# arjunchandra/paac

Measured on AMD Instinct MI355X. Metric: global env-steps/sec at 32 envs, t_max=5, Nature net; 1/2/4/8 MI355X, higher is better.
Workload: dtype f32; 1 GPU; breakout action set (A=4), NATURE net, 32 envs per GPU x 1 GPU, t_max=5, synthetic 84x84x4 u8 frames generated on device, sampler=numpy, hipGraph replay; envs_per_gpu=32, t_max=5, global_envs=32, parallelism=env-sharded dp1, no collective (one process)

## Files before the change

include/paac_hip.h:

```cpp
#ifndef PAAC_HIP_H
#define PAAC_HIP_H

#include <stdint.h>

#ifdef __cplusplus
extern "C" {
#endif

typedef struct paac_ctx paac_ctx;
typedef struct paac_graph paac_graph;
typedef void* paac_stream_t;

enum { PAAC_ARCH_NIPS = 0, PAAC_ARCH_NATURE = 1,
       PAAC_ARCH_USER = 2 };
enum { PAAC_CLIP_IGNORE = 0, PAAC_CLIP_GLOBAL = 1, PAAC_CLIP_LOCAL = 2 };

#define PAAC_MAX_TENSORS 12
#define PAAC_OBS_BYTES 28224
#define PAAC_RAW_H 210
#define PAAC_RAW_W 160

typedef struct {
  int32_t num_tensors;
  int64_t total;
  int64_t total_unpadded;
  int64_t offset[PAAC_MAX_TENSORS];
  int64_t size[PAAC_MAX_TENSORS];
  int32_t rank[PAAC_MAX_TENSORS];
  int32_t shape[PAAC_MAX_TENSORS][4];
  char name[PAAC_MAX_TENSORS][32];
} paac_layout;

typedef struct {
  int32_t device;
  int32_t arch;
  int32_t num_actions;
  int32_t max_batch;
} paac_cfg;

const char* paac_last_error(void);
int paac_version(void);

int paac_param_layout(int arch, int num_actions, paac_layout* out);

int paac_create(const paac_cfg* cfg, paac_ctx** out);
int paac_destroy(paac_ctx* ctx);

int paac_forward(paac_ctx* ctx, const float* params, const uint8_t* states, int batch,
                 float* logits, float* probs, float* values, paac_stream_t stream);

int paac_forward_sample(paac_ctx* ctx, const float* params, const uint8_t* states, int batch, float* probs,
                        float* values, uint64_t seed, const uint64_t* step_base_dev, uint64_t step_offset,
                        uint32_t env_offset, int32_t* actions, paac_stream_t stream);

int paac_forward_sample_synth_step(paac_ctx* ctx, const float* params, const uint8_t* states, int batch, float* probs,
                                   float* values, uint64_t seed, const uint64_t* step_base_dev, uint64_t step_offset,
                                   uint32_t env_offset, int32_t* actions, uint64_t env_seed, uint32_t terminal_threshold,
                                   uint8_t* stack_out, float* rewards_out, float* masks_out, float* ep_reward,
                                   int32_t* ep_len, void* finished, paac_stream_t stream);

int paac_train_forward(paac_ctx* ctx, const float* params, const uint8_t* states, int batch, float* values,
                       paac_stream_t stream);
int paac_train_forward_trunk(paac_ctx* ctx, const float* params, const uint8_t* states, int batch, paac_stream_t stream);

int paac_keep_next_forward(paac_ctx* ctx, int train_row);
int paac_bootstrap_forward_trunk(paac_ctx* ctx, const float* params, const uint8_t* states, int batch, int train_row,
                                 paac_stream_t stream);

#define PAAC_ACT_STEP_MAX_ENVS 64
#define PAAC_ACT_STEP_MAX_ENVS_LARGE 256
int paac_act_step_mt(paac_ctx* ctx, const float* params, const uint8_t* states, int batch, uint32_t* mt_state,
                     int32_t* actions, float* probs_out, float* values_out, uint64_t env_seed, uint32_t env_offset,
                     uint32_t terminal_threshold, const uint64_t* step_base_dev, uint64_t step_offset, uint8_t* stack_out,
                     uint8_t* stack_out2, float* rewards_out, float* masks_out, float* ep_reward, int32_t* ep_len,
                     void* finished, uint8_t* raw_scratch, void* walk_scratch, int64_t walk_scratch_bytes,
                     paac_stream_t stream);

int paac_pack_weights(paac_ctx* ctx, const float* params, paac_stream_t stream);
int paac_set_managed_weights(paac_ctx* ctx, int on);

int paac_loss_backward(paac_ctx* ctx, const float* params, const uint8_t* states, const int32_t* actions,
                       const float* y, const float* adv, int batch, float entropy_beta,
                       float* grad, float* loss_out, int forward_done, int phase, paac_stream_t stream);

enum { PAAC_RETURNS_NSTEP = 0, PAAC_RETURNS_GAE = 1 };

typedef struct {
  const float* v_boot;
  const float* rewards;
  const float* masks;
  const float* values;
  int32_t T, N;
  double gamma;
  float* y_out;
  float* adv_out;
  int64_t* global_step_dev;
  int64_t increment;
  double initial_lr;
  int64_t lr_annealing_steps;
  float* lr_out_dev;
  uint64_t* tick_dev;
  uint64_t tick_inc;
  int32_t estimator;
  double gae_lambda;
} paac_returns;
#define PAAC_RETURNS_TRUNCS 0x100
typedef struct {
  paac_returns ret;
  const float* truncs;
} paac_returns_truncs;
int paac_loss_backward_returns(paac_ctx* ctx, const float* params, const uint8_t* states, const int32_t* actions,
                               const paac_returns* ret, int batch, float entropy_beta, float* grad, float* loss_out,
                               int forward_done, int phase, paac_stream_t stream);

#define PAAC_PPO_EPOCHS_MAX 16
int paac_loss_backward_record(paac_ctx* ctx, const float* params, const uint8_t* states, const int32_t* actions,
                              const float* y, const float* adv, float* p_old_out, int batch, float entropy_beta,
                              float* grad, float* loss_out, int forward_done, int phase, paac_stream_t stream);
int paac_loss_backward_returns_record(paac_ctx* ctx, const float* params, const uint8_t* states, const int32_t* actions,
                                      const paac_returns* ret, float* p_old_out, int batch, float entropy_beta,
                                      float* grad, float* loss_out, int forward_done, int phase, paac_stream_t stream);
int paac_loss_backward_ppo(paac_ctx* ctx, const float* params, const uint8_t* states, const int32_t* actions,
                           const float* y, const float* adv, const float* p_old, float clip_eps, int batch,
                           float entropy_beta, float* grad, float* loss_out, float* ppo_stats_out, int forward_done,
                           int phase, paac_stream_t stream);

int paac_loss_backward_ppo_vclip(paac_ctx* ctx, const float* params, const uint8_t* states, const int32_t* actions,
                                 const float* y, const float* adv, const float* p_old, const float* v_old, float clip_eps,
                                 float vclip_eps, int batch, float entropy_beta, float* grad, float* loss_out,
// ... 186 lines not shown
```

paac_amd/_lib.py:

```python
import ctypes
import os
from ctypes import POINTER, c_char, c_char_p, c_double, c_float, c_int, c_int32, c_int64, c_uint32, c_uint64, c_void_p

HERE = os.path.dirname(os.path.abspath(__file__))
LIB_PATH = os.environ.get("PAAC_HIP_LIB") or os.path.join(HERE, "libpaac_hip.so")

MAX_TENSORS = 12
PROF_FAMILIES = 16
ARCH_NIPS, ARCH_NATURE, ARCH_USER = 0, 1, 2
CLIP_IGNORE, CLIP_GLOBAL, CLIP_LOCAL = 0, 1, 2
RETURNS_NSTEP, RETURNS_GAE = 0, 1
RETURNS_TRUNCS = 0x100
PPO_EPOCHS_MAX = 16
PPO_MINIBATCHES_MAX = 16
PPO_STEPS_MAX = 64
MINIBATCH_MAX_ROWS = 8192
EVAL_CATCH, EVAL_BRICKS, EVAL_RALLY = 0, 1, 2
EVAL_USER = 3


class Layout(ctypes.Structure):
    _fields_ = [("num_tensors", c_int32),
                ("total", c_int64),
                ("total_unpadded", c_int64),
# ... 59 lines not shown
                                          c_void_p, c_void_p, c_int, c_int, c_void_p]),
    "paac_loss_backward_ppo": (c_int, [c_void_p, c_void_p, c_void_p, c_void_p, c_void_p, c_void_p, c_void_p, c_float, c_int,
                                       c_float, c_void_p, c_void_p, c_void_p, c_int, c_int, c_void_p]),
    "paac_loss_backward_ppo_vclip": (c_int, [c_void_p, c_void_p, c_void_p, c_void_p, c_void_p, c_void_p, c_void_p, c_void_p,
                                             c_float, c_float, c_int, c_float, c_void_p, c_void_p, c_void_p, c_int, c_int,
                                             c_void_p]),
    "paac_minibatch_perms": (c_int, [c_int, c_int, c_uint64, c_void_p, c_uint64, c_void_p, c_void_p]),
    "paac_gather_minibatch": (c_int, [c_void_p, c_int, c_void_p, c_void_p, c_void_p, c_void_p, c_void_p, c_void_p, c_void_p,
                                      c_void_p, c_void_p, c_void_p, c_void_p, c_void_p, c_void_p]),
    "paac_record_policy": (c_int, [c_void_p, c_void_p, c_void_p, c_int, c_void_p, c_void_p, c_int, c_void_p]),
    "paac_adv_normalize": (c_int, [c_void_p, c_int, c_void_p, c_void_p, c_void_p]),
    "paac_returns_norm_tick": (c_int, [c_void_p, c_void_p, POINTER(Returns), c_void_p, c_void_p, c_void_p]),
    "paac_returns_scan": (c_int, [POINTER(Returns), c_void_p]),
    "paac_game_step": (c_int, [c_int, c_uint64, c_uint32, c_int] + [c_void_p] * 7 + [POINTER(EnvRecords), c_int, c_void_p]),
    "paac_grad_stats": (c_int, [c_void_p, c_void_p, c_void_p]),
    "paac_grad_tensor_stats": (c_int, [c_void_p, c_void_p, c_void_p]),
    "paac_clip_rmsprop": (c_int, [c_void_p, c_void_p, c_void_p, c_void_p, c_void_p, c_int64, c_void_p, c_float,
                                  c_float, c_float, c_float, c_int, c_float, c_void_p, c_void_p]),
    "paac_clip_adam": (c_int, [c_void_p, c_void_p, c_void_p, c_void_p, c_void_p, c_void_p, c_int64, c_void_p, c_float,
                               c_float, c_float, c_float, c_int, c_float, c_void_p, c_void_p]),
    "paac_clip_rmsprop_gated": (c_int, [c_void_p, c_void_p, c_void_p, c_void_p, c_void_p, c_int64, c_void_p, c_float,
                                        c_float, c_float, c_float, c_int, c_float, c_void_p, POINTER(KlGate), c_void_p]),
    "paac_clip_adam_gated": (c_int, [c_void_p, c_void_p, c_void_p, c_void_p, c_void_p, c_void_p, c_int64, c_void_p, c_float,
                                     c_float, c_float, c_float, c_int, c_float, c_void_p, POINTER(KlGate), c_void_p]),
    "paac_lr_step": (c_int, [c_void_p, c_int64, c_double, c_int64, c_void_p, c_void_p]),
    "paac_nstep_returns": (c_int, [c_void_p, c_void_p, c_void_p, c_void_p, c_int, c_int, c_double, c_void_p,
                                   c_void_p, c_void_p]),
    "paac_nstep_returns_tick": (c_int, [c_void_p, c_void_p, c_void_p, c_void_p, c_int, c_int, c_double, c_void_p,
                                        c_void_p, c_void_p, c_int64, c_double, c_int64, c_void_p, c_void_p, c_uint64,
                                        c_void_p]),
    "paac_gae_returns": (c_int, [c_void_p, c_void_p, c_void_p, c_void_p, c_int, c_int, c_double, c_double, c_void_p,
                                 c_void_p, c_void_p]),
    "paac_gae_returns_tick": (c_int, [c_void_p, c_void_p, c_void_p, c_void_p, c_int, c_int, c_double, c_double, c_void_p,
                                      c_void_p, c_void_p, c_int64, c_double, c_int64, c_void_p, c_void_p, c_uint64,
                                      c_void_p]),
    "paac_sample_mt_scratch_bytes": (c_int64, [c_int, c_int]),
    "paac_sample_mt": (c_int, [c_void_p, c_int, c_int, c_void_p, c_void_p, c_void_p, c_void_p]),
    "paac_sample_philox": (c_int, [c_void_p, c_int, c_int, c_uint64, c_void_p, c_uint64, c_uint32, c_void_p, c_void_p]),
    "paac_counter_add": (c_int, [c_void_p, c_uint64, c_void_p]),
    "paac_preprocess_stack": (c_int, [c_void_p, c_int, c_int, c_void_p, c_void_p, c_void_p, c_void_p, c_void_p]),
    "paac_synth_reset": (c_int, [c_uint64, c_uint32, c_int, c_void_p, c_void_p, c_void_p]),
    "paac_synth_step": (c_int, [c_uint64, c_uint32, c_int, c_void_p, c_uint32, c_void_p, c_uint64, c_void_p,
                                c_void_p, c_void_p, c_void_p, c_void_p, c_void_p, c_void_p, c_void_p, c_void_p,
                                c_void_p]),
    "paac_eval_step": (c_int, [c_int, c_void_p, c_int, c_int, c_int, c_uint64, c_int, c_void_p, c_uint64, c_uint64, c_uint32,
                               c_void_p, c_void_p, c_void_p, c_void_p, c_void_p, c_void_p, c_void_p, c_void_p, c_void_p,
                               c_void_p]),
    "paac_match_step": (c_int, [c_void_p, c_int, c_int, c_int, c_uint64, c_int, c_void_p, c_uint64, c_uint64, c_uint32,
                                c_void_p, c_void_p, c_void_p, c_void_p, c_void_p, c_void_p, c_void_p, c_void_p, c_void_p,
                                c_void_p]),
    "paac_act_step_mt": (c_int, [c_void_p, c_void_p, c_void_p, c_int, c_void_p, c_void_p, c_void_p, c_void_p, c_uint64,
                                 c_uint32, c_uint32, c_void_p, c_uint64, c_void_p, c_void_p, c_void_p, c_void_p, c_void_p,
                                 c_void_p, c_void_p, c_void_p, c_void_p, c_int64, c_void_p]),
    "paac_walk_scratch_bytes": (c_int64, [c_int, c_int]),
    "paac_debug_report_zero": (c_int, [c_int]),
    "paac_sample_mt_synth_step": (c_int, [c_void_p, c_int, c_void_p, c_void_p, c_uint64, c_uint32, c_int, c_uint32, c_void_p,
                                          c_uint64, c_void_p, c_void_p, c_void_p, c_void_p, c_void_p, c_void_p, c_void_p,
                                          c_void_p, c_void_p, c_int64, c_void_p, c_void_p]),
    "paac_forward_sample_synth_step": (c_int, [c_void_p, c_void_p, c_void_p, c_int, c_void_p, c_void_p, c_uint64, c_void_p,
                                               c_uint64, c_uint32, c_void_p, c_uint64, c_uint32, c_void_p, c_void_p,
                                               c_void_p, c_void_p, c_void_p, c_void_p, c_void_p]),
    "paac_graph_begin": (c_int, [c_void_p]),
    "paac_graph_end": (c_int, [c_void_p, POINTER(c_void_p)]),
    "paac_graph_launch": (c_int, [c_void_p, c_void_p]),
    "paac_graph_destroy": (c_int, [c_void_p]),
    "paac_debug_activation": (c_int64, [c_void_p, c_int, c_int, c_void_p, c_int64, c_void_p]),
    "paac_debug_activation_size": (c_int64, [c_int, c_int, c_int]),
    "paac_debug_set_tuning": (c_int, [c_void_p, c_int, c_int, c_int, c_int, c_int]),
    "paac_debug_get_tuning": (c_int, [c_void_p, c_int, c_int, POINTER(c_int), POINTER(c_int), POINTER(c_int)]),
    "paac_debug_cfg_known": (c_int, [c_int, c_int]),
    "paac_debug_cfg_body": (c_int, [c_int, c_int]),
    "paac_debug_clock": (c_int, [c_void_p, c_void_p]),
    "paac_prof_enable": (c_int, [c_void_p, c_int]),
    "paac_prof_read": (c_int, [c_void_p, POINTER(c_int32), POINTER(c_int32), POINTER(c_float), c_int]),
    "paac_prof_read_mix": (c_int, [c_void_p, POINTER(c_int32), c_int]),
    "paac_prof_name": (c_char_p, [c_int]),
    "paac_user_arch": (c_int, [POINTER(c_int32), POINTER(c_int32), POINTER(c_int32)]),
    "paac_user_arch_layers": (c_int, [POINTER(c_int32), POINTER(c_int32)]),
}

for _game in ("catch", "bricks", "rally"):
    _SIGNATURES["paac_%s_reset" % _game] = (c_int, [c_uint64, c_uint32, c_int, c_void_p, c_void_p, c_void_p])
    _SIGNATURES["paac_%s_step" % _game] = (c_int, [c_uint64, c_uint32, c_int] + [c_void_p] * 12 +
                                           ([c_int] if _game == "bricks" else []) + [c_void_p])
_SIGNATURES["paac_duel_reset"] = _SIGNATURES["paac_catch_reset"]
_SIGNATURES["paac_duel_step"] = (c_int, [c_uint64, c_uint32, c_int] + [c_void_p] * 7 + [POINTER(EnvRecords), c_void_p])
_SIGNATURES["paac_duel_ghost_reset"] = (c_int, [c_uint64, c_uint32, c_int, c_void_p, c_void_p, c_void_p, c_void_p])
_SIGNATURES["paac_duel_ghost_step"] = (c_int, [c_uint64, c_uint32, c_int, c_void_p, c_void_p, c_int, c_uint64, c_void_p, c_uint64] +
                                       [c_void_p] * 9 + [POINTER(EnvRecords), c_void_p, c_void_p])
_SIGNATURES["paac_user_game_info"] = (c_int, [POINTER(c_int), POINTER(c_int), POINTER(c_int)])
_SIGNATURES["paac_user_game_reset"] = _SIGNATURES["paac_catch_reset"]
_SIGNATURES["paac_user_game_step"] = (c_int, [c_uint64, c_uint32, c_int] + [c_void_p] * 7 + [POINTER(EnvRecords), c_int, c_void_p])

EXPORTED_SYMBOLS = tuple(sorted(_SIGNATURES))

_lib = None


def use_library(path):
    global LIB_PATH
    if _lib is not None and os.path.abspath(path) != os.path.abspath(LIB_PATH):
        raise PaacHipError("%s is already loaded: a process holds ONE geometry besides Nature -- choose the user "
                           "architecture before anything touches the library" % LIB_PATH)
    LIB_PATH = path


# ... 53 lines not shown
```

paac_amd/csrc/api.hip:

```cpp
#include <stdarg.h>
#include <stdlib.h>

#include <new>

#include "common.h"
#include "synth_dev.h"

namespace paac {

static thread_local char g_err[512] = "";
thread_local ProfEvents g_prof = {nullptr, nullptr, 0, 0};
paac_ctx* g_prof_ctx = nullptr;

void set_error(const char* fmt, ...) {
  va_list ap;
  va_start(ap, fmt);
  vsnprintf(g_err, sizeof(g_err), fmt, ap);
  va_end(ap);
}

ArchSpec arch_spec(int arch) {
  ArchSpec s;
  memset(&s, 0, sizeof(s));
  if (arch == PAAC_ARCH_NATURE) {
// ... 6 lines not shown
#ifdef PAAC_USER_ARCH
  } else if (arch == PAAC_ARCH_USER) {
#ifndef PAAC_USER_K1
#define PAAC_USER_K1 8
#define PAAC_USER_S1 4
#define PAAC_USER_K2 4
#define PAAC_USER_S2 2
#define PAAC_USER_K3 3
#define PAAC_USER_S3 1
#endif
    constexpr int o1 = (84 - PAAC_USER_K1) / PAAC_USER_S1 + 1, o2 = (o1 - PAAC_USER_K2) / PAAC_USER_S2 + 1;
    constexpr int o3 = PAAC_USER_NCONV == 3 ? (o2 - PAAC_USER_K3) / PAAC_USER_S3 + 1 : o2;
    s.nconv = PAAC_USER_NCONV;
    s.conv[0] = ConvSpec{84, 84, 4, o1, o1, PAAC_USER_C1, PAAC_USER_K1, PAAC_USER_S1};
    s.conv[1] = ConvSpec{o1, o1, PAAC_USER_C1, o2, o2, PAAC_USER_C2, PAAC_USER_K2, PAAC_USER_S2};
    if (PAAC_USER_NCONV == 3) s.conv[2] = ConvSpec{o2, o2, PAAC_USER_C2, o3, o3, PAAC_USER_C3, PAAC_USER_K3, PAAC_USER_S3};
    s.flat = PAAC_USER_NCONV == 3 ? o3 * o3 * PAAC_USER_C3 : o2 * o2 * PAAC_USER_C2;
    s.fc = PAAC_USER_H;
#endif
  } else {
    s.nconv = 2;
    s.conv[0] = ConvSpec{84, 84, 4, 20, 20, 16, 8, 4};
    s.conv[1] = ConvSpec{20, 20, 16, 9, 9, 32, 4, 2};
    s.flat = 2592;
    s.fc = 256;
  }
  return s;
}

bool arch_supported(int arch) {
#ifdef PAAC_USER_ARCH
  return arch == PAAC_ARCH_NATURE || arch == PAAC_ARCH_USER;
#else
  return arch == PAAC_ARCH_NATURE || arch == PAAC_ARCH_NIPS;
#endif
}

int64_t wslab_floats_needed(int arch);
size_t tower_pack_bytes();
void default_tuning(paac_ctx* c);
int cfg_body(int op, int cfg);
int fc_splits_max();

static const char* kFamilyNames[PAAC_PROF_FAMILIES] = {
    "conv1_fwd", "conv2_fwd", "conv3_fwd", "fc_fwd", "heads_fwd", "heads_bwd", "fc_wgrad", "fc_dgrad",
    "conv3_wgrad", "conv3_dgrad", "conv2_wgrad", "conv2_dgrad", "conv1_wgrad", "grad_finalize", "clip_rmsprop", "misc",
    "env_step", "sample_env_step", "sample_mt", "sample_philox", "nstep_returns", "preprocess_stack", "conv_tower",
    "fc_conv3_wgrad", "conv2_conv1_wgrad", "dgrad_tower"};

}

using namespace paac;

struct paac_graph {
  hipGraph_t graph;
  hipGraphExec_t exec;
};

extern "C" {

const char* paac_last_error(void) { return g_err; }
int paac_version(void) { return 100; }

int paac_param_layout(int arch, int num_actions, paac_layout* out) {
  PAAC_REQUIRE(out, "paac_param_layout: null out");
  PAAC_REQUIRE(arch_supported(arch), "paac_param_layout: arch %d is not compiled into this library (a library holds Nature "
               "and either the NIPS geometry or one user architecture, paac_user_arch)", arch);
  PAAC_REQUIRE(num_actions >= 2 && num_actions <= 32, "paac_param_layout: num_actions %d not in [2,32]", num_actions);
  memset(out, 0, sizeof(*out));
  const ArchSpec s = arch_spec(arch);
  int t = 0;
  int64_t off = 0, unp = 0;
  auto add = [&](const char* name, int rank, int d0, int d1, int d2, int d3) {
    int64_t size = (int64_t)d0 * (rank > 1 ? d1 : 1) * (rank > 2 ? d2 : 1) * (rank > 3 ? d3 : 1);
    snprintf(out->name[t], sizeof(out->name[t]), "%s", name);
    out->rank[t] = rank;
    out->shape[t][0] = d0; out->shape[t][1] = rank > 1 ? d1 : 0;
    out->shape[t][2] = rank > 2 ? d2 : 0; out->shape[t][3] = rank > 3 ? d3 : 0;
    out->offset[t] = off;
    out->size[t] = size;
    off += (size + 3) / 4 * 4;
    unp += size;
    ++t;
  };
  char nm[32];
  for (int i = 0; i < s.nconv; ++i) {
    snprintf(nm, sizeof(nm), "conv%d_weights", i + 1);
    add(nm, 4, s.conv[i].k, s.conv[i].k, s.conv[i].cin, s.conv[i].cout);
    snprintf(nm, sizeof(nm), "conv%d_biases", i + 1);
    add(nm, 1, s.conv[i].cout, 0, 0, 0);
  }
  snprintf(nm, sizeof(nm), "fc%d_weights", s.nconv + 1);
  add(nm, 2, s.flat, s.fc, 0, 0);
  snprintf(nm, sizeof(nm), "fc%d_biases", s.nconv + 1);
  add(nm, 1, s.fc, 0, 0, 0);
  add("actor_output_weights", 2, s.fc, num_actions, 0, 0);
  add("actor_output_biases", 1, num_actions, 0, 0, 0);
  add("critic_output_weights", 2, s.fc, 1, 0, 0);
  add("critic_output_biases", 1, 1, 0, 0, 0);
  out->num_tensors = t;
  out->total = off;
  out->total_unpadded = unp;
  return 0;
}

int paac_create(const paac_cfg* cfg, paac_ctx** out) {
// ... 37 lines not shown
        else if (op < 0 || op >= OP_COUNT || cls < 0 || cls > 2)
          set_error("paac_create: PAAC_TUNE_OVERRIDE entry \"%s\": op %d / class %d outside the table (ops 0..%d, classes 0..2)",
                    entry, op, cls, OP_COUNT - 1);
        else set_error("paac_create: PAAC_TUNE_OVERRIDE entry \"%s\": op %d has no configuration id %d", entry, op, cf);
        delete c;
        return -1;
      }
      c->tune[op][cls] = Tune{cf, ks, xc};
      ov += used;
      if (*ov == ',') ++ov;
    }
  }
  const int64_t B = cfg->max_batch;
  const int A = cfg->num_actions;
  c->fc_splits_max = fc_splits_max();
  for (int w = 0; w < 2; ++w) {
    Workspace& W = c->ws[w];
    for (int i = 0; i < c->spec.nconv; ++i) {
      const ConvSpec& cs = c->spec.conv[i];
      PAAC_CHECK_HIP(hipMalloc(&W.act[i], (size_t)((B + 15) / 16 * 16) * cs.oh * cs.ow * cs.cout * sizeof(float)));
    }
    PAAC_CHECK_HIP(hipMalloc(&W.fc_slab, (size_t)c->fc_splits_max * B * c->spec.fc * sizeof(float)));
    PAAC_CHECK_HIP(hipMalloc(&W.h, (size_t)B * c->spec.fc * sizeof(float)));
    PAAC_CHECK_HIP(hipMalloc(&W.probs, (size_t)B * A * sizeof(float)));
    PAAC_CHECK_HIP(hipMalloc(&W.logits, (size_t)B * A * sizeof(float)));
    PAAC_CHECK_HIP(hipMalloc(&W.values, (size_t)B * sizeof(float)));
  }
  for (int i = 0; i < c->spec.nconv; ++i) {
    const ConvSpec& cs = c->spec.conv[i];
    PAAC_CHECK_HIP(hipMalloc(&c->dact[i], (size_t)B * cs.oh * cs.ow * cs.cout * sizeof(float)));
  }
  PAAC_CHECK_HIP(hipMalloc(&c->dh, (size_t)B * c->spec.fc * sizeof(float)));
  if (paac::dh_planes_supported(c->spec.fc)) {
    PAAC_CHECK_HIP(hipMalloc(&c->dh_planes, paac::dh_planes_bytes((int)B, c->spec.fc)));
    PAAC_CHECK_HIP(hipMemset(c->dh_planes, 0, paac::dh_planes_bytes((int)B, c->spec.fc)));
  }
  { const char* v = getenv("PAAC_FC_DGRAD_ONCE"); c->fc_dgrad_once = !(v && *v && atoi(v) == 0); }
  PAAC_CHECK_HIP(hipMalloc(&c->dl_buf, (size_t)B * paac::kDlStride * sizeof(float)));
  PAAC_CHECK_HIP(hipMalloc(&c->ppo_rows, (size_t)B * 2 * sizeof(float)));
  PAAC_CHECK_HIP(hipMalloc(&c->vclip_rows, (size_t)B * sizeof(float)));
  c->wslab_floats = wslab_floats_needed(cfg->arch);
  PAAC_CHECK_HIP(hipMalloc(&c->wslab, (size_t)c->wslab_floats * sizeof(float)));
  PAAC_CHECK_HIP(hipMalloc(&c->partials, 8192 * sizeof(float)));
  PAAC_CHECK_HIP(hipMemset(c->partials, 0, 8192 * sizeof(float)));
  PAAC_CHECK_HIP(hipMalloc(&c->zeros, (size_t)(c->spec.fc > 1024 ? c->spec.fc : 1024) * sizeof(float)));
  PAAC_CHECK_HIP(hipMemset(c->zeros, 0, (size_t)(c->spec.fc > 1024 ? c->spec.fc : 1024) * sizeof(float)));
  c->keep_row = -1;
  c->keep_h_only = 0;
  c->heads_pending_h = 0;
  PAAC_CHECK_HIP(hipMalloc(&c->mt_ahead, mt_ahead_bytes()));
  PAAC_CHECK_HIP(hipMemset(c->mt_ahead, 0, mt_ahead_bytes()));
  c->ahead_state = nullptr;
  c->ahead_D = 0;
  {
    const char* v = getenv("PAAC_TOWER");
    c->tower_on = (cfg->arch == PAAC_ARCH_NATURE) && !(v && *v && atoi(v) == 0);
    { const char* q = getenv("PAAC_FC_QUARTER"); c->no_quarter_tiles = (q && *q && atoi(q) == 0) ? 1 : 0; }
    c->tower2_on = (cfg->arch == PAAC_ARCH_NIPS) && tower2_available() && !(v && *v && atoi(v) == 0);
    c->managed_weights = 0;
    c->tower_pack = nullptr;
    if (c->tower_on || c->tower2_on) PAAC_CHECK_HIP(hipMalloc(&c->tower_pack, tower_pack_bytes()));
    PAAC_CHECK_HIP(hipMalloc(&c->fc_pack, (size_t)c->spec.flat * c->spec.fc * sizeof(float)));
  }
  c->ev_start = new hipEvent_t[paac_ctx::PROF_MAX_EVENTS];
  c->ev_stop = new hipEvent_t[paac_ctx::PROF_MAX_EVENTS];
  c->ev_family = new int[paac_ctx::PROF_MAX_EVENTS];
  c->ev_batch = new int[paac_ctx::PROF_MAX_EVENTS];
  c->ev_mix = new int[paac_ctx::PROF_MAX_EVENTS];
  c->ev_count = 0;
  c->prof_on = 0;
  for (int i = 0; i < paac_ctx::PROF_MAX_EVENTS; ++i) {
    c->ev_start[i] = nullptr;
    c->ev_stop[i] = nullptr;
  }
  *out = c;
  return 0;
}

int paac_destroy(paac_ctx* c) {
  if (!c) return 0;
  for (int w = 0; w < 2; ++w) {
    Workspace& W = c->ws[w];
    for (int i = 0; i < 3; ++i)
      if (W.act[i]) (void)hipFree(W.act[i]);
    float* bufs[] = {W.fc_slab, W.h, W.probs, W.logits, W.values};
    for (float* b : bufs)
      if (b) (void)hipFree(b);
  }
  for (int i = 0; i < 3; ++i)
    if (c->dact[i]) (void)hipFree(c->dact[i]);
  float* bufs[] = {c->dh, c->wslab, c->partials, c->dl_buf, c->zeros, c->ppo_rows, c->vclip_rows};
  for (float* b : bufs)
    if (b) (void)hipFree(b);
  if (c->mt_ahead) (void)hipFree(c->mt_ahead);
  if (c->dh_planes) (void)hipFree(c->dh_planes);
  if (c->tower_pack) (void)hipFree(c->tower_pack);
  if (c->fc_pack) (void)hipFree(c->fc_pack);
  for (int i = 0; i < paac_ctx::PROF_MAX_EVENTS; ++i) {
    if (c->ev_start[i]) (void)hipEventDestroy(c->ev_start[i]);
    if (c->ev_stop[i]) (void)hipEventDestroy(c->ev_stop[i]);
  }
  delete[] c->ev_start;
  delete[] c->ev_stop;
  delete[] c->ev_family;
  delete[] c->ev_batch;
  delete[] c->ev_mix;
  delete c;
  return 0;
}

int paac_forward(paac_ctx* ctx, const float* params, const uint8_t* states, int batch, float* logits, float* probs,
                 float* values, paac_stream_t stream) {
  PAAC_REQUIRE(ctx && params && states, "paac_forward: null argument");
  PAAC_REQUIRE(batch > 0 && batch <= ctx->max_batch, "paac_forward: batch %d outside (0, max_batch=%d]", batch,
               ctx->max_batch);
  const int rc = launch_forward(ctx, 0, params, states, batch, logits, probs, values, (hipStream_t)stream);
  if (rc) return rc;
  PAAC_CHECK_HIP(hipGetLastError());
  return 0;
}

int paac_pack_weights(paac_ctx* ctx, const float* params, paac_stream_t stream) {
  PAAC_REQUIRE(ctx && params, "paac_pack_weights: null argument");
  const int rc = launch_pack_weights(ctx, params, (hipStream_t)stream);
  if (rc) return rc;
  PAAC_CHECK_HIP(hipGetLastError());
  return 0;
}

int paac_set_managed_weights(paac_ctx* ctx, int on) {
  PAAC_REQUIRE(ctx, "paac_set_managed_weights: null ctx");
  ctx->managed_weights = on ? 1 : 0;
  return 0;
}

int paac_train_forward(paac_ctx* ctx, const float* params, const uint8_t* states, int batch, float* values,
                       paac_stream_t stream) {
  PAAC_REQUIRE(ctx && params && states, "paac_train_forward: null argument");
  PAAC_REQUIRE(batch > 0 && batch <= ctx->max_batch, "paac_train_forward: batch %d outside (0, max_batch=%d]", batch,
               ctx->max_batch);
  const int rc = launch_forward(ctx, 1, params, states, batch, nullptr, nullptr, values, (hipStream_t)stream);
  if (rc) return rc;
  PAAC_CHECK_HIP(hipGetLastError());
  return 0;
}

int paac_train_forward_trunk(paac_ctx* ctx, const float* params, const uint8_t* states, int batch, paac_stream_t stream) {
  PAAC_REQUIRE(ctx && params && states, "paac_train_forward_trunk: null argument");
  PAAC_REQUIRE(batch > 0 && batch <= ctx->max_batch, "paac_train_forward_trunk: batch %d outside (0, max_batch=%d]", batch,
               ctx->max_batch);
  const int rc = launch_forward_trunk_train(ctx, params, states, batch, (hipStream_t)stream);
  if (rc) return rc;
  PAAC_CHECK_HIP(hipGetLastError());
  return 0;
}

int paac_keep_next_forward(paac_ctx* ctx, int train_row) {
  PAAC_REQUIRE(ctx, "paac_keep_next_forward: null ctx");
  PAAC_REQUIRE(train_row >= -1 && train_row < ctx->max_batch, "paac_keep_next_forward: row %d outside [-1, max_batch=%d)",
               train_row, ctx->max_batch);
  ctx->keep_row = train_row;
  return 0;
}

int paac_bootstrap_forward_trunk(paac_ctx* ctx, const float* params, const uint8_t* states, int batch, int train_row,
                                 paac_stream_t stream) {
  PAAC_REQUIRE(ctx && params && states, "paac_bootstrap_forward_trunk: null argument");
  PAAC_REQUIRE(batch > 0 && train_row >= 0 && train_row + batch <= ctx->max_batch,
               "paac_bootstrap_forward_trunk: rows [%d, %d) outside max_batch=%d", train_row, train_row + batch, ctx->max_batch);
  const int rc = launch_bootstrap_trunk(ctx, params, states, batch, train_row, (hipStream_t)stream);
  if (rc) return rc;
  PAAC_CHECK_HIP(hipGetLastError());
  return 0;
}

int paac_forward_sample(paac_ctx* ctx, const float* params, const uint8_t* states, int batch, float* probs,
                        float* values, uint64_t seed, const uint64_t* step_base_dev, uint64_t step_offset,
                        uint32_t env_offset, int32_t* actions, paac_stream_t stream) {
  PAAC_REQUIRE(ctx && params && states && actions, "paac_forward_sample: null argument");
  PAAC_REQUIRE(batch > 0 && batch <= ctx->max_batch, "paac_forward_sample: batch %d outside (0, max_batch=%d]", batch,
               ctx->max_batch);
  const int rc = launch_forward_sample(ctx, params, states, batch, probs, values, seed, step_base_dev, step_offset,
                                       env_offset, actions, nullptr, (hipStream_t)stream);
  if (rc) return rc;
  PAAC_CHECK_HIP(hipGetLastError());
  return 0;
}

int paac_forward_sample_synth_step(paac_ctx* ctx, const float* params, const uint8_t* states, int batch, float* probs,
                                   float* values, uint64_t seed, const uint64_t* step_base_dev, uint64_t step_offset,
                                   uint32_t env_offset, int32_t* actions, uint64_t env_seed, uint32_t terminal_threshold,
                                   uint8_t* stack_out, float* rewards_out, float* masks_out, float* ep_reward,
                                   int32_t* ep_len, void* finished, paac_stream_t stream) {
  PAAC_REQUIRE(ctx && params && states && actions, "paac_forward_sample_synth_step: null argument");
  SynthStep st;
  if (synth_step_of("paac_forward_sample_synth_step", "null argument", false, &st, env_seed, env_offset, batch, terminal_threshold,
                    step_base_dev, step_offset, states, stack_out, nullptr, rewards_out, masks_out, ep_reward, ep_len, finished,
                    nullptr))
    return -1;
  PAAC_REQUIRE(batch > 0 && batch <= ctx->max_batch, "paac_forward_sample_synth_step: batch %d outside (0, max_batch=%d]",
               batch, ctx->max_batch);
  const int rc = launch_forward_sample(ctx, params, states, batch, probs, values, seed, step_base_dev, step_offset, env_offset,
                                       actions, &st, (hipStream_t)stream);
  if (rc) return rc;
  PAAC_CHECK_HIP(hipGetLastError());
  return 0;
}

int paac_act_step_mt(paac_ctx* ctx, const float* params, const uint8_t* states, int batch, uint32_t* mt_state,
                     int32_t* actions, float* probs_out, float* values_out, uint64_t env_seed, uint32_t env_offset,
                     uint32_t terminal_threshold, const uint64_t* step_base_dev, uint64_t step_offset, uint8_t* stack_out,
                     uint8_t* stack_out2, float* rewards_out, float* masks_out, float* ep_reward, int32_t* ep_len,
                     void* finished, uint8_t* raw_scratch, void* walk_scratch, int64_t walk_scratch_bytes,
                     paac_stream_t stream) {
  PAAC_REQUIRE(ctx && params && states && mt_state && actions && probs_out && values_out, "paac_act_step_mt: null argument");
  HeadsPartials hp{nullptr, 0, nullptr, nullptr, values_out};
  if (stack_out == nullptr) {
    PAAC_REQUIRE(!stack_out2 && !raw_scratch, "paac_act_step_mt: no environment step (stack_out == NULL) takes no stack_out2 / "
                 "raw_scratch");
    PAAC_REQUIRE(batch > 0 && batch <= ctx->max_batch && batch <= PAAC_ACT_STEP_MAX_ENVS &&
                 (int64_t)batch * (ctx->cfg.num_actions - 1) <= 1024,
                 "paac_act_step_mt: sampling without an environment step covers up to %d environments and 1024 draws (use "
                 "paac_forward + paac_sample_mt); got %d x %d actions", PAAC_ACT_STEP_MAX_ENVS, batch, ctx->cfg.num_actions);
// ... 25 lines not shown
               "paac_act_step_mt: N*(A-1) = %ld exceeds %d (use paac_forward + paac_sample_mt + paac_synth_step)",
               (long)batch * (ctx->cfg.num_actions - 1), PAAC_FUSED_SAMPLE_MAX_DRAWS);
  if (!forward_has_fc_heads(ctx)) {
    int rc = launch_forward(ctx, 0, params, states, batch, nullptr, probs_out, values_out, (hipStream_t)stream);
    if (rc) return rc;
    rc = launch_sample_mt_synth_step(probs_out, ctx->cfg.num_actions, mt_state, actions, st, walk_scratch, walk_scratch_bytes,
                                     nullptr, (hipStream_t)stream);
    if (rc) return rc;
    PAAC_CHECK_HIP(hipGetLastError());
    return 0;
  }
  if (batch > PAAC_ACT_STEP_MAX_ENVS || (int64_t)batch * (ctx->cfg.num_actions - 1) > 1024) {
    const bool tail = (ctx->tower_on || ctx->tower2_on) && ctx->managed_weights && batch <= PAAC_ACT_STEP_MAX_ENVS_LARGE;
    if (tail) {
      ctx->ahead_state = mt_state;
      ctx->ahead_D = batch * (ctx->cfg.num_actions - 1);
    }
    static const int fold_knob = [] {
      const char* v = getenv("PAAC_HEADS_IN_SAMPLER");
      return (v && *v) ? (atoi(v) != 0 ? 1 : 0) : -1;
    }();
    const bool fold = fold_knob >= 0 ? fold_knob == 1 : ctx->cfg.num_actions <= 8;
    int rc;
    if (tail && fold && sampler_folds_heads(batch, ctx->cfg.num_actions, walk_scratch))
      rc = launch_forward_trunk(ctx, params, states, batch, &hp, (hipStream_t)stream);
    else
      rc = launch_forward(ctx, 0, params, states, batch, nullptr, probs_out, values_out, (hipStream_t)stream);
    ctx->ahead_state = nullptr;
    if (rc) return rc;
    rc = launch_sample_mt_synth_step(probs_out, ctx->cfg.num_actions, mt_state, actions, st, walk_scratch, walk_scratch_bytes,
                                     tail ? ctx->mt_ahead : nullptr, (hipStream_t)stream, hp.partial ? &hp : nullptr);
    if (rc) return rc;
    PAAC_CHECK_HIP(hipGetLastError());
    return 0;
  }
  static const bool ahead_on = [] {
    const char* v = getenv("PAAC_MT_AHEAD_SMALL");
    return v && *v && atoi(v) != 0;
  }();
  if (ahead_on) {
    ctx->ahead_state = mt_state;
    ctx->ahead_D = batch * (ctx->cfg.num_actions - 1);
  }
  int rc = launch_forward_trunk(ctx, params, states, batch, &hp, (hipStream_t)stream);
  ctx->ahead_state = nullptr;
  if (rc) return rc;
  rc = launch_sample_env_step_heads(hp, probs_out, ctx->cfg.num_actions, mt_state, actions, st, ahead_on ? ctx->mt_ahead : nullptr,
                                    (hipStream_t)stream);
  if (rc) return rc;
  PAAC_CHECK_HIP(hipGetLastError());
  return 0;
}

static int check_returns(const char* fn, const paac_returns* ret) {
  PAAC_REQUIRE(ret->rewards && ret->masks && ret->values && ret->y_out && ret->adv_out, "%s: null rollout record", fn);
  PAAC_REQUIRE(returns_estimator(ret) == PAAC_RETURNS_NSTEP || returns_estimator(ret) == PAAC_RETURNS_GAE,
               "%s: estimator %d (PAAC_RETURNS_NSTEP = 0, PAAC_RETURNS_GAE = 1)", fn, returns_estimator(ret));
  PAAC_REQUIRE(ret->gae_lambda >= 0.0 && ret->gae_lambda <= 1.0, "%s: gae_lambda %g outside [0, 1]", fn, ret->gae_lambda);
  PAAC_REQUIRE(!ret->global_step_dev || (ret->lr_out_dev && ret->lr_annealing_steps > 0),
               "%s: schedule bookkeeping needs lr_out_dev and lr_annealing_steps", fn);
  return 0;
}

static int loss_backward_entry(const char* fn, paac_ctx* ctx, const float* params, const uint8_t* states, const int32_t* actions,
                               int batch, float entropy_beta, float* grad, float* loss_out, const BackwardCall& call,
                               int forward_done, int phase, paac_stream_t stream) {
  PAAC_REQUIRE(ctx && params && states && actions && grad && (call.ret || (call.y && call.adv)), "%s: null argument", fn);
  PAAC_REQUIRE(batch > 0 && batch <= ctx->max_batch, "%s: batch %d outside (0, max_batch=%d]", fn, batch, ctx->max_batch);
  PAAC_REQUIRE(phase >= 0 && phase <= 3, "%s: phase %d", fn, phase);
  if (const paac_returns* ret = call.ret) {
    PAAC_REQUIRE(ret->T > 0 && ret->N > 0 && ret->T * ret->N == batch, "%s: T*N = %d*%d != batch %d", fn, ret->T, ret->N, batch);
    if (const int rc = check_returns(fn, ret)) return rc;
    PAAC_REQUIRE(ret->v_boot || (forward_done && batch + ret->N <= ctx->max_batch),
                 "%s: v_boot == NULL takes the bootstrap values from rows [batch, batch + N) of a training forward that has "
                 "already run over batch + N rows", fn);
  }
  int rc = 0;
  if (!forward_done && phase != 2) {
    rc = launch_forward(ctx, 1, params, states, batch, nullptr, nullptr, nullptr, (hipStream_t)stream);
    if (rc) return rc;
  }
  ctx->last_ws = 1;
  rc = launch_backward(ctx, params, states, actions, batch, entropy_beta, grad, loss_out, phase, call, (hipStream_t)stream);
  if (rc) return rc;
  PAAC_CHECK_HIP(hipGetLastError());
  return 0;
}

int paac_loss_backward(paac_ctx* ctx, const float* params, const uint8_t* states, const int32_t* actions, const float* y,
                       const float* adv, int batch, float entropy_beta, float* grad, float* loss_out,
                       int forward_done, int phase, paac_stream_t stream) {
  const BackwardCall call{.y = y, .adv = adv, .loss = kLossA3c};
  return loss_backward_entry("paac_loss_backward", ctx, params, states, actions, batch, entropy_beta, grad, loss_out, call,
                             forward_done, phase, stream);
}

int paac_loss_backward_returns(paac_ctx* ctx, const float* params, const uint8_t* states, const int32_t* actions,
                               const paac_returns* ret, int batch, float entropy_beta, float* grad, float* loss_out,
                               int forward_done, int phase, paac_stream_t stream) {
  PAAC_REQUIRE(ret, "paac_loss_backward_returns: null argument");
  const BackwardCall call{.ret = ret, .loss = kLossA3c};
  return loss_backward_entry("paac_loss_backward_returns", ctx, params, states, actions, batch, entropy_beta, grad, loss_out,
                             call, forward_done, phase, stream);
}

int paac_loss_backward_returns_record(paac_ctx* ctx, const float* params, const uint8_t* states, const int32_t* actions,
                                      const paac_returns* ret, float* p_old_out, int batch, float entropy_beta, float* grad,
                                      float* loss_out, int forward_done, int phase, paac_stream_t stream) {
  PAAC_REQUIRE(ret, "paac_loss_backward_returns_record: null argument");
  PAAC_REQUIRE(p_old_out, "paac_loss_backward_returns_record: null p_old_out");
  const BackwardCall call{.ret = ret, .loss = kLossA3cRecord, .p_old_out = p_old_out};
  return loss_backward_entry("paac_loss_backward_returns_record", ctx, params, states, actions, batch, entropy_beta, grad,
                             loss_out, call, forward_done, phase, stream);
}

int paac_loss_backward_record(paac_ctx* ctx, const float* params, const uint8_t* states, const int32_t* actions,
                              const float* y, const float* adv, float* p_old_out, int batch, float entropy_beta, float* grad,
                              float* loss_out, int forward_done, int phase, paac_stream_t stream) {
  PAAC_REQUIRE(p_old_out, "paac_loss_backward_record: null p_old_out");
  const BackwardCall call{.y = y, .adv = adv, .loss = kLossA3cRecord, .p_old_out = p_old_out};
  return loss_backward_entry("paac_loss_backward_record", ctx, params, states, actions, batch, entropy_beta, grad, loss_out,
                             call, forward_done, phase, stream);
}

int paac_loss_backward_ppo(paac_ctx* ctx, const float* params, const uint8_t* states, const int32_t* actions, const float* y,
                           const float* adv, const float* p_old, float clip_eps, int batch, float entropy_beta, float* grad,
                           float* loss_out, float* ppo_stats_out, int forward_done, int phase, paac_stream_t stream) {
  PAAC_REQUIRE(p_old, "paac_loss_backward_ppo: null p_old");
  PAAC_REQUIRE(clip_eps > 0.f && clip_eps < 1.f, "paac_loss_backward_ppo: clip_eps %g outside (0, 1)", (double)clip_eps);
  const BackwardCall call{.y = y, .adv = adv, .loss = kLossPpo, .p_old = p_old, .clip_eps = clip_eps,
                          .ppo_stats_out = ppo_stats_out};
  return loss_backward_entry("paac_loss_backward_ppo", ctx, params, states, actions, batch, entropy_beta, grad, loss_out, call,
                             forward_done, phase, stream);
}

static int64_t debug_activation_elems(const ArchSpec& spec, int what, int batch) {
  if (what == 25) return batch;
  if (what >= 21 && what <= 24) what -= 20;
  if (what >= 11 && what <= 10 + spec.nconv) what -= 10;
  if (what >= 1 && what <= spec.nconv) {
    const ConvSpec& cs = spec.conv[what - 1];
    return (int64_t)batch * cs.oh * cs.ow * cs.cout;
  }
  if (what == 4 || what == 14) return (int64_t)batch * spec.fc;
  return -1;
}

int paac_returns_norm_tick(paac_ctx* ctx, const float* params, const paac_returns* ret, float* adv_n_out, double* stats_out,
                           paac_stream_t stream) {
  PAAC_REQUIRE(ret && adv_n_out, "paac_returns_norm_tick: null argument");
  PAAC_REQUIRE(ret->T > 0 && ret->N > 0, "paac_returns_norm_tick: T=%d N=%d", ret->T, ret->N);
  if (const int rc = check_returns("paac_returns_norm_tick", ret)) return rc;
  const float* v_boot = ret->v_boot;
  if (!v_boot) {
    const int64_t batch = (int64_t)ret->T * ret->N;
    PAAC_REQUIRE(ctx && params && batch + ret->N <= ctx->max_batch,
                 "paac_returns_norm_tick: v_boot == NULL takes the bootstrap values from rows [T*N, T*N + N) of a training "
                 "forward that has already run over T*N + N rows of this ctx");
    const int rc = launch_bootstrap_heads(ctx, params, (int)batch, ret->N, (hipStream_t)stream);
    if (rc) return rc;
    v_boot = ctx->ws[1].values + batch;
  }
  const int rc = launch_returns_norm(ret, v_boot, adv_n_out, stats_out, (hipStream_t)stream);
  if (rc) return rc;
  PAAC_CHECK_HIP(hipGetLastError());
  return 0;
}

int paac_record_policy(paac_ctx* ctx, const float* params, const int32_t* actions, int batch, float* p_old_out, float* v_out,
                       int value_rows, paac_stream_t stream) {
  PAAC_REQUIRE(ctx && params, "paac_record_policy: null argument");
  PAAC_REQUIRE(p_old_out || v_out, "paac_record_policy: nothing to record (p_old_out and v_out are both NULL)");
  PAAC_REQUIRE(!p_old_out || actions, "paac_record_policy: p_old_out needs the actions");
  if (!p_old_out) batch = 0;
  if (!v_out) value_rows = 0;
  const int rows = batch > value_rows ? batch : value_rows;
  PAAC_REQUIRE(batch >= 0 && value_rows >= 0 && rows > 0 && rows <= ctx->max_batch,
               "paac_record_policy: batch %d / value_rows %d outside (0, max_batch=%d]", batch, value_rows, ctx->max_batch);
  if (ctx->heads_pending_rows > 0) {
    PAAC_REQUIRE(rows <= ctx->heads_pending_rows, "paac_record_policy: the pending training forward covers %d rows, %d are asked "
                 "for", ctx->heads_pending_rows, rows);
    const int rc = launch_deferred_heads(ctx, params, (hipStream_t)stream);
    if (rc) return rc;
  }
  const int rc = launch_record_policy(ctx, actions, batch, value_rows, p_old_out, v_out, (hipStream_t)stream);
  if (rc) return rc;
  PAAC_CHECK_HIP(hipGetLastError());
  return 0;
}

int paac_loss_backward_ppo_vclip(paac_ctx* ctx, const float* params, const uint8_t* states, const int32_t* actions,
                                 const float* y, const float* adv, const float* p_old, const float* v_old, float clip_eps,
                                 float vclip_eps, int batch, float entropy_beta, float* grad, float* loss_out,
                                 float* ppo_stats_out, int forward_done, int phase, paac_stream_t stream) {
  PAAC_REQUIRE(p_old, "paac_loss_backward_ppo_vclip: null p_old");
  PAAC_REQUIRE(v_old, "paac_loss_backward_ppo_vclip: null v_old");
  PAAC_REQUIRE(clip_eps > 0.f && clip_eps < 1.f, "paac_loss_backward_ppo_vclip: clip_eps %g outside (0, 1)", (double)clip_eps);
  PAAC_REQUIRE(vclip_eps > 0.f, "paac_loss_backward_ppo_vclip: vclip_eps %g is not positive (0 = off: paac_loss_backward_ppo)",
               (double)vclip_eps);
  const BackwardCall call{.y = y, .adv = adv, .loss = kLossPpoVclip, .p_old = p_old, .clip_eps = clip_eps,
                          .ppo_stats_out = ppo_stats_out, .v_old = v_old, .vclip_eps = vclip_eps};
  return loss_backward_entry("paac_loss_backward_ppo_vclip", ctx, params, states, actions, batch, entropy_beta, grad, loss_out,
                             call, forward_done, phase, stream);
}

int64_t paac_debug_activation_size(int arch, int what, int batch) {
  PAAC_REQUIRE(batch > 0, "paac_debug_activation_size: batch %d", batch);
  const int64_t n = debug_activation_elems(arch_spec(arch), what, batch);
  if (n < 0) {
    set_error("paac_debug_activation_size: what=%d", what);
    return -1;
  }
  return n;
}

int64_t paac_debug_activation(paac_ctx* ctx, int what, int batch, float* out, int64_t out_capacity, paac_stream_t stream) {
  PAAC_REQUIRE(ctx && out && batch > 0 && batch <= ctx->max_batch, "paac_debug_activation: bad arguments");
  if (what == 26) {
    const int64_t np = (int64_t)batch * ctx->cfg.num_actions;
    PAAC_REQUIRE(np <= out_capacity, "paac_debug_activation: what=26 needs %ld floats, out holds %ld", (long)np, (long)out_capacity);
    PAAC_CHECK_HIP(hipMemcpyAsync(out, ctx->ws[1].probs, (size_t)np * sizeof(float), hipMemcpyDeviceToDevice, (hipStream_t)stream));
    return np;
  }
  const int64_t n = debug_activation_elems(ctx->spec, what, batch);
  if (n < 0) {
    set_error("paac_debug_activation: what=%d", what);
// ... 160 lines not shown
```

paac_amd/csrc/common.h:

```cpp
#pragma once
#include <hip/hip_runtime.h>
#include <hip/hip_ext.h>
#include <stdint.h>
#include <stdio.h>
#include <string.h>

#include "../../include/paac_hip.h"

namespace paac {

void set_error(const char* fmt, ...);

inline int returns_estimator(const paac_returns* ret) { return ret->estimator & ~PAAC_RETURNS_TRUNCS; }
inline const float* returns_truncs(const paac_returns* ret) {
  return (ret->estimator & PAAC_RETURNS_TRUNCS) ? reinterpret_cast<const paac_returns_truncs*>(ret)->truncs : nullptr;
}

#define PAAC_CHECK_HIP(expr)                                                              \
  do {                                                                                    \
    hipError_t _e = (expr);                                                               \
    if (_e != hipSuccess) {                                                               \
      paac::set_error("%s:%d: %s -> %s", __FILE__, __LINE__, #expr, hipGetErrorString(_e)); \
      return -2;                                                                          \
    }                                                                                     \
// ... 20 lines not shown
  int fc;
};
ArchSpec arch_spec(int arch);

enum Family {
  F_CONV1_FWD = 0, F_CONV2_FWD, F_CONV3_FWD, F_FC_FWD, F_HEADS_FWD,
  F_HEADS_BWD, F_FC_WGRAD, F_FC_DGRAD, F_CONV3_WGRAD, F_CONV3_DGRAD, F_CONV2_WGRAD, F_CONV2_DGRAD, F_CONV1_WGRAD,
  F_GRAD_FINALIZE, F_CLIP_RMSPROP, F_MISC,
  F_ENV_STEP, F_SAMPLE_ENV_STEP, F_SAMPLE_MT, F_SAMPLE_PHILOX, F_NSTEP_RETURNS, F_PREPROCESS_STACK, F_CONV_TOWER,
  F_FC_CONV3_WGRAD, F_CONV2_CONV1_WGRAD, F_DGRAD_TOWER
};
static_assert(F_DGRAD_TOWER + 1 == PAAC_PROF_FAMILIES, "family count");

}

namespace paac {
struct Workspace {
  float* act[3];
  float* fc_slab;
  float* h;
  float* probs;
  float* values;
  float* logits;
};
}

namespace paac {
enum Op { OP_CONV1_FWD = 0, OP_CONV2_FWD, OP_CONV3_FWD, OP_FC_FWD, OP_FC_WGRAD, OP_FC_DGRAD, OP_CONV3_WGRAD,
          OP_CONV3_DGRAD, OP_CONV2_WGRAD, OP_CONV2_DGRAD, OP_CONV1_WGRAD, OP_CONV_TOWER, OP_COUNT };
struct Tune {
  int cfg;
  int ksplit;
  int xcd;
};
inline int batch_class(int batch) { return batch > 512 ? 2 : batch > 64 ? 1 : 0; }

constexpr int kDlStride = 36;

constexpr bool dh_planes_supported(int H) { return (H % 32) == 0 && H <= 1024; }
inline size_t dh_planes_bytes(int max_batch, int H) { return (size_t)((max_batch + 15) / 16 * 16) * H * 6; }

struct FinalizeSeg {
  const float* src;
  float* dst;
  int count;
  int splits;
  long stride;
};
struct FinalizeArgs {
  FinalizeSeg seg[8];
  int nseg;
};

}

struct paac_ctx {
  paac_cfg cfg;
  paac::Tune tune[paac::OP_COUNT][3];
  paac::ArchSpec spec;
  paac_layout layout;
  int max_batch;
  paac::Workspace ws[2];
  int last_ws;
  float* dact[3];
  float* dh;
  void* dh_planes;
  int dh_planes_rows;
  int fc_dgrad_once;
  float* wslab;
  int64_t wslab_floats;
  float* partials;
  int last_clip_local;
  paac::FinalizeArgs pending_fin;
  const float* pending_fin_grad;
  int heads_pending_rows, heads_pending_splits;
  int keep_row;
  int keep_h_only;
  int heads_pending_h;
  float* zeros;
  void* mt_ahead;
  const uint32_t* ahead_state;
  int ahead_D;
  float* dl_buf;
  float* ppo_rows;
  float* vclip_rows;
  int fc_splits_max;
  void* tower_pack;
  void* fc_pack;
  int tower_on;
  int heads_ntiles;
  int no_quarter_tiles;
  int tower2_on;
  int managed_weights;
  int prof_on;
  static constexpr int PROF_MAX_EVENTS = 8192;
  hipEvent_t* ev_start;
  hipEvent_t* ev_stop;
  int* ev_family;
  int* ev_batch;
  int* ev_mix;
  int ev_count;
};

namespace paac {

struct ProfEvents {
  hipEvent_t start, stop;
  int mix, nmix;
};
extern thread_local ProfEvents g_prof;
extern paac_ctx* g_prof_ctx;

struct ProfScope {
  paac_ctx* ctx;
  int idx;
  ProfScope(paac_ctx* c, int family, int batch, hipStream_t) : ctx(c), idx(-1) {
    if (c && c->prof_on && c->ev_count < paac_ctx::PROF_MAX_EVENTS) {
      idx = c->ev_count++;
      c->ev_family[idx] = family;
      c->ev_batch[idx] = batch;
      g_prof.start = c->ev_start[idx];
      g_prof.stop = c->ev_stop[idx];
    }
  }
  ~ProfScope() {
    if (idx >= 0) ctx->ev_mix[idx] = g_prof.mix;
    g_prof.start = nullptr;
    g_prof.stop = nullptr;
    g_prof.mix = 0;
    g_prof.nmix = 0;
  }
};

inline void prof_mix(int products) {
  if (g_prof.start && g_prof.nmix < 4) g_prof.mix |= (products & 255) << (8 * g_prof.nmix++);
}

enum { PROF_WHOLE = 0, PROF_FIRST = 1, PROF_LAST = 2, PROF_NONE = 3 };
template <class K, class... Args>
inline void launch_k(K kernel, dim3 grid, dim3 block, hipStream_t s, int part, Args... args) {
  hipEvent_t st = (part == PROF_WHOLE || part == PROF_FIRST) ? g_prof.start : nullptr;
  hipEvent_t sp = (part == PROF_WHOLE || part == PROF_LAST) ? g_prof.stop : nullptr;
  if (st || sp)
    hipExtLaunchKernelGGL(kernel, grid, block, 0, s, st, sp, 0, args...);
  else
    hipLaunchKernelGGL(kernel, grid, block, 0, s, args...);
}

int launch_forward_trunk_train(paac_ctx* ctx, const float* params, const uint8_t* states, int batch, hipStream_t s);
int launch_deferred_heads(paac_ctx* ctx, const float* params, hipStream_t s);
int launch_bootstrap_heads(paac_ctx* ctx, const float* params, int batch, int N, hipStream_t s);
int launch_returns_norm(const paac_returns* ret, const float* v_boot, float* adv_n, double* stats, hipStream_t s);
int launch_record_policy(paac_ctx* ctx, const int32_t* actions, int batch, int vrows, float* p_old, float* v_out, hipStream_t s);
int launch_forward(paac_ctx* ctx, int ws, const float* params, const uint8_t* states, int batch, float* logits,
                   float* probs, float* values, hipStream_t s);
struct SynthStep;
int launch_forward_sample(paac_ctx* ctx, const float* params, const uint8_t* states, int batch, float* probs,
                          float* values, uint64_t seed, const uint64_t* step_base, uint64_t step_off,
                          uint32_t env_offset, int32_t* actions, const SynthStep* step, hipStream_t s);
int launch_pack_weights(paac_ctx* ctx, const float* params, hipStream_t s);
int launch_pack_dgrad(paac_ctx* ctx, const float* params, hipStream_t s);
struct HeadsPartials {
  const float* partial;
  int ntiles;
  const float *ba, *bc;
  float* values_out;
};
size_t mt_ahead_bytes();
bool sampler_folds_heads(int N, int A, const void* walk_scratch);
bool tower2_available();
int synth_step_of(const char* fn, const char* what, bool in_place_ok, SynthStep* st, uint64_t seed, uint32_t env_offset, int N,
                  uint32_t thresh, const uint64_t* step_base, uint64_t step_off, const uint8_t* stack_in, uint8_t* stack_out,
                  uint8_t* stack_out2, float* rewards, float* masks, float* ep_reward, int32_t* ep_len, void* finished,
                  uint8_t* raw_scratch);
int launch_sample_mt_synth_step(const float* probs, int A, uint32_t* mt_state, int32_t* actions, const SynthStep& st,
                                void* walk_scratch, int64_t walk_scratch_bytes, const void* mt_ahead, hipStream_t stream,
                                const HeadsPartials* heads = nullptr);
int launch_sample_mt_probs(const float* probs, int A, uint32_t* mt_state, int32_t* actions, int N, hipStream_t stream);
bool forward_has_fc_heads(const paac_ctx* ctx);
__device__ __forceinline__ void gae_step(const double gamma, const double gl, const float rw, const float mk, const double V,
                                         const double Vn, double& A) {
  const double delta = __dsub_rn(__dadd_rn((double)rw, __dmul_rn(__dmul_rn(gamma, Vn), (double)mk)), V);
  A = __dadd_rn(delta, __dmul_rn(__dmul_rn(gl, A), (double)mk));
}
__device__ __forceinline__ void nstep_step(const double gamma, const bool first, const float vb, const float rw, const float mk,
                                           double& R) {
  const double prod = first ? (double)__fmul_rn((float)gamma, vb) : __dmul_rn(gamma, R);
  R = __dadd_rn((double)rw, __dmul_rn(prod, (double)mk));
}
__device__ __forceinline__ void nstep_step_tr(const double gamma, const bool first, const float vb, const float rw, const float mk,
                                              const float tr, const double V, double& R) {
  if (tr != 0.f) R = __dadd_rn((double)rw, __dmul_rn(gamma, V));
  else nstep_step(gamma, first, vb, rw, mk, R);
}
__device__ __forceinline__ void gae_step_tr(const double gamma, const double gl, const float rw, const float mk, const float tr,
                                            const double V, const double Vn, double& A) {
  if (tr != 0.f) A = __dsub_rn(__dadd_rn((double)rw, __dmul_rn(gamma, V)), V);
  else gae_step(gamma, gl, rw, mk, V, Vn, A);
}

struct CycleTick {
  int64_t* global_step;
  int64_t step_inc;
  double lr0;
  int64_t anneal;
  float* lr_out;
  uint64_t* tick;
  uint64_t tick_inc;
};
__device__ __forceinline__ void cycle_tick(const CycleTick& ct) {
  if (ct.global_step) {
    const int64_t step = *ct.global_step + ct.step_inc;
    *ct.global_step = step;
    double lr = 0.0;
    if (step <= ct.anneal) lr = ct.lr0 - ((double)step * ct.lr0 / (double)ct.anneal);
    *ct.lr_out = (float)lr;
  }
  if (ct.tick) *ct.tick += ct.tick_inc;
}

// ... 38 lines not shown
```

paac_amd/csrc/fc_heads.h:

```cpp
#pragma once
#include "dmm.h"
#include "mt_ahead.h"

namespace paac {

constexpr int fc_heads_waves(const int flat) {
  const int g = flat / 16;
  for (const int w : {7, 9, 8, 6, 5, 10, 4, 12, 3})
    if (flat % 16 == 0 && g % w == 0 && g / w > 8) return w;
  return 0;
}

constexpr int kFcHeadsMaxRows = 64;
constexpr int kFcHeadsMidRows = 256;

template <int K, int H>
__global__ __launch_bounds__(256) void pack_fc_kernel(const float* __restrict__ Wf, f32x4* __restrict__ out) {
  constexpr int G = K / 16;
  const int i = blockIdx.x * 256 + threadIdx.x;
  if (i >= (H / 16) * G * 64) return;
  const int lane = i & 63, unit = i >> 6;
  const int g = unit % G, nt = unit / G;
  const int li = lane & 15, kq = lane >> 4;
  f32x4 v;
#pragma unroll
  for (int s = 0; s < 4; ++s) v[s] = Wf[(size_t)(16 * g + 4 * kq + s) * H + 16 * nt + li];
  out[i] = v;
}

template <int K, int H, int NW, bool A_PACKED>
__global__ __launch_bounds__(64 * NW) void fc_heads_kernel(const float* __restrict__ act, const f32x4* __restrict__ wfp,
                                                           const float* __restrict__ bf, const float* __restrict__ Wa,
                                                           const float* __restrict__ Wc, const int A, const int B,
                                                           float* __restrict__ partial, float* __restrict__ h_out,
                                                           const MtAheadArgs ahead) {
  constexpr int NTILES = H / 16, G = K / 16, GPW = G / NW, PF = 8;
  static_assert(K % 16 == 0 && H % 16 == 0 && G % NW == 0 && GPW > PF, "fc geometry");
  if (ahead.out != nullptr && blockIdx.x == gridDim.x - 1) {
    __shared__ uint32_t ahead_blocks[MT_AHEAD_BLK * 624];
    mt_produce_ahead<64 * NW>(ahead, ahead_blocks);
    return;
  }
  __shared__ f32x4 red[NW * 64];
  const int tid = threadIdx.x, lane = tid & 63;
  const int wave = __builtin_amdgcn_readfirstlane(tid >> 6);
  const int li = lane & 15, kq = lane >> 4;
  const int nt = blockIdx.x % NTILES, mt = blockIdx.x / NTILES;
  const int row_a = mt * 16 + li;
  const bool row_ok = row_a < B;
  const int col = nt * 16 + li;
  constexpr int A_STEP = A_PACKED ? 256 : 16;
  const float* ap = A_PACKED ? act + (((size_t)mt * G + (size_t)wave * GPW) * 64 + lane) * 4
                             : act + (size_t)(row_ok ? row_a : 0) * K + 4 * kq + (size_t)wave * (GPW * 16);
  const f32x4* bp = wfp + ((size_t)nt * G + (size_t)wave * GPW) * 64 + lane;

  constexpr int RING = PF + 1;
  f32x4 fa[RING], fb[RING];
  constexpr int NO = (33 + NW - 1) / NW;
  float wh[NO];
#pragma unroll
  for (int q = 0; q < NO; ++q) {
    const int o = wave + NW * q;
    wh[q] = (o < A) ? Wa[(size_t)col * A + o] : (o == A ? Wc[col] : 0.f);
  }
  const float bias = bf[col];
#pragma unroll
  for (int i = 0; i < PF; ++i) {
    fa[i] = *reinterpret_cast<const f32x4*>(ap + A_STEP * i);
    fb[i] = bp[(size_t)i * 64];
  }
  __builtin_amdgcn_sched_barrier(0);
  f32x4 acc = (f32x4){0.f, 0.f, 0.f, 0.f};
#pragma unroll
  for (int i = 0; i < GPW; ++i) {
    if (i + PF < GPW) {
      fa[(i + PF) % RING] = *reinterpret_cast<const f32x4*>(ap + A_STEP * (i + PF));
      fb[(i + PF) % RING] = bp[(size_t)(i + PF) * 64];
    }
    __builtin_amdgcn_sched_barrier(0);
#pragma unroll
    for (int e = 0; e < 4; ++e)
      acc = __builtin_amdgcn_mfma_f32_16x16x4f32(row_ok ? fa[i % RING][e] : 0.f, fb[i % RING][e], acc, 0, 0, 0);
    __builtin_amdgcn_sched_barrier(0);
  }
  red[wave * 64 + lane] = acc;
  __syncthreads();
  f32x4 h = red[lane];
#pragma unroll
  for (int w = 1; w < NW; ++w) h += red[w * 64 + lane];
#pragma unroll
  for (int r = 0; r < 4; ++r) h[r] = fmaxf(h[r] + bias, 0.f);
  if (h_out != nullptr && wave == 0) {
#pragma unroll
    for (int r = 0; r < 4; ++r) {
      const int row = mt * 16 + 4 * kq + r;
      if (row < B) h_out[(size_t)row * H + col] = h[r];
    }
  }
#pragma unroll
  for (int q = 0; q < NO; ++q) {
    const int o = wave + NW * q;
    if (o > A) break;
    float v[4];
#pragma unroll
    for (int r = 0; r < 4; ++r) {
      float t = h[r] * wh[q];
      t += __shfl_xor(t, 1, 64);
      t += __shfl_xor(t, 2, 64);
      t += __shfl_xor(t, 4, 64);
      t += __shfl_xor(t, 8, 64);
      v[r] = t;
    }
    if (li == 0) {
#pragma unroll
      for (int r = 0; r < 4; ++r) {
        const int row = mt * 16 + 4 * kq + r;
        if (row < B) partial[((size_t)nt * B + row) * (A + 1) + o] = v[r];
      }
    }
  }
}

template <int K, int H, int NW, bool A_PACKED>
__global__ __launch_bounds__(64 * NW) void fc_heads_q_kernel(const float* __restrict__ act, const f32x4* __restrict__ wfp,
                                                             const float* __restrict__ bf, const float* __restrict__ Wa,
                                                             const float* __restrict__ Wc, const int A, const int B,
                                                             float* __restrict__ partial, float* __restrict__ h_out) {
  constexpr int NTILES = H / 8, G = K / 16, GPW = G / NW, NS = GPW / 2, PF = 6;
  static_assert(K % 16 == 0 && H % 16 == 0 && G % NW == 0 && GPW % 2 == 0 && NS > PF, "fc geometry");
  __shared__ f32x4 red[NW * 64];
  const int tid = threadIdx.x, lane = tid & 63;
  const int wave = __builtin_amdgcn_readfirstlane(tid >> 6);
  const int li = lane & 15, kq = lane >> 4;
  const int l8 = li & 7, odd = li >> 3;
  const int nt = blockIdx.x % NTILES, mt = blockIdx.x / NTILES;
  const int row_a = mt * 8 + l8;
  const bool row_ok = row_a < B;
  const int col = nt * 8 + l8;
  constexpr int A_STEP = A_PACKED ? 512 : 32;
  const int g0 = wave * GPW + odd;
  const float* ap = A_PACKED ? act + ((((size_t)(mt >> 1) * G + g0) * 64) + kq * 16 + (mt & 1) * 8 + l8) * 4
                             : act + (size_t)(row_ok ? row_a : 0) * K + 4 * kq + (size_t)g0 * 16;
  const f32x4* bp = wfp + ((size_t)(nt >> 1) * G + g0) * 64 + kq * 16 + (nt & 1) * 8 + l8;

  constexpr int RING = PF + 1;
  f32x4 fa[RING], fb[RING];
  constexpr int NO = (33 + NW - 1) / NW;
  float wh[NO];
#pragma unroll
  for (int q = 0; q < NO; ++q) {
    const int o = wave + NW * q;
    wh[q] = (o < A) ? Wa[(size_t)col * A + o] : (o == A ? Wc[col] : 0.f);
  }
  const float bias = bf[col];
#pragma unroll
  for (int i = 0; i < PF; ++i) {
    fa[i] = *reinterpret_cast<const f32x4*>(ap + A_STEP * i);
    fb[i] = bp[(size_t)i * 128];
  }
  __builtin_amdgcn_sched_barrier(0);
  f32x4 acc = (f32x4){0.f, 0.f, 0.f, 0.f};
#pragma unroll
  for (int i = 0; i < NS; ++i) {
    if (i + PF < NS) {
      fa[(i + PF) % RING] = *reinterpret_cast<const f32x4*>(ap + A_STEP * (i + PF));
      fb[(i + PF) % RING] = bp[(size_t)(i + PF) * 128];
    }
    __builtin_amdgcn_sched_barrier(0);
#pragma unroll
    for (int e = 0; e < 4; ++e)
      acc = __builtin_amdgcn_mfma_f32_16x16x4f32(row_ok ? fa[i % RING][e] : 0.f, fb[i % RING][e], acc, 0, 0, 0);
    __builtin_amdgcn_sched_barrier(0);
  }
  red[wave * 64 + lane] = acc;
  __syncthreads();
  const bool own = li < 8 && kq < 2;
  const int src = own ? lane : 0;
  f32x4 h = red[src] + red[src + 40];
#pragma unroll
  for (int w = 1; w < NW; ++w) h += red[w * 64 + src] + red[w * 64 + src + 40];
#pragma unroll
  for (int r = 0; r < 4; ++r) h[r] = own ? fmaxf(h[r] + bias, 0.f) : 0.f;
  if (h_out != nullptr && wave == 0 && own) {
#pragma unroll
    for (int r = 0; r < 4; ++r) {
      const int row = mt * 8 + 4 * kq + r;
      if (row < B) h_out[(size_t)row * H + col] = h[r];
    }
  }
#pragma unroll
  for (int q = 0; q < NO; ++q) {
    const int o = wave + NW * q;
    if (o > A) break;
    float v[4];
#pragma unroll
    for (int r = 0; r < 4; ++r) {
      float t = h[r] * wh[q];
      t += __shfl_xor(t, 1, 64);
      t += __shfl_xor(t, 2, 64);
      t += __shfl_xor(t, 4, 64);
      v[r] = t;
    }
    if (li == 0 && kq < 2) {
#pragma unroll
      for (int r = 0; r < 4; ++r) {
        const int row = mt * 8 + 4 * kq + r;
        if (row < B) partial[((size_t)nt * B + row) * (A + 1) + o] = v[r];
      }
    }
  }
}
constexpr bool fc_heads_quarter_ok(const int flat) {
  const int w = fc_heads_waves(flat);
  return w > 0 && (flat / 16 / w) % 2 == 0 && (flat / 16 / w) / 2 > 6;
}

__device__ __forceinline__ void heads_softmax_store(const int B, const int A, const float* lg_s, float* probs_lds,
                                                    float* __restrict__ logits_out, float* __restrict__ probs_out,
                                                    float* __restrict__ values_out, float* __restrict__ logits_out2,
                                                    float* __restrict__ probs_out2, float* __restrict__ values_out2) {
  const int tid = threadIdx.x;
  for (int idx = tid; idx < B * A; idx += 256) {
    const int row = idx / A, a = idx - row * A;
    const float* lg = lg_s + row * (A + 1);
    float m = lg[0];
    for (int j = 1; j < A; ++j) m = fmaxf(m, lg[j]);
// ... 83 lines not shown
```

paac_amd/csrc/misc.hip:

```cpp
#include "common.h"
#include "synth_dev.h"
#include "fc_heads.h"
#include "heads.h"

namespace paac {

#ifdef PAAC_DMM_STAMPS
__device__ unsigned long long* g_misc_stamps = nullptr;
#define MISC_STAMP(i)                                                                       \
  do {                                                                                      \
    __builtin_amdgcn_sched_barrier(0);                                                      \
    if (g_misc_stamps && threadIdx.x == 0) g_misc_stamps[(i)] = (unsigned long long)wall_clock64(); \
    __builtin_amdgcn_sched_barrier(0);                                                      \
  } while (0)
#else
#define MISC_STAMP(i)
#endif

struct NoPlane {};
template <int EST, class PLANE = NoPlane>
__global__ void returns_scan_kernel(const float* __restrict__ v_boot, const float* __restrict__ rewards,
                                    const float* __restrict__ masks, const float* __restrict__ values, int T, int N,
                                    double gamma, double gl, float* __restrict__ y, float* __restrict__ adv,
                                    const CycleTick ct, const PLANE truncs) {
  constexpr bool TR = !std::is_same<PLANE, NoPlane>::value;
  const int e = blockIdx.x * 64 + (threadIdx.x & 63);
  if (threadIdx.x >= 64) {
    if (blockIdx.x == 0 && threadIdx.x == 64) cycle_tick(ct);
    return;
  }
  if (e >= N) return;
  constexpr int CH = 8;
  const float vb = v_boot[e];
  double S = 0.0, Vn = (double)vb;
  for (int t0 = T - 1; t0 >= 0; t0 -= CH) {
    float r[CH], m[CH], v[CH], tr[CH];
#pragma unroll
    for (int u = 0; u < CH; ++u) {
      const int t = t0 - u;
      const long i = (long)(t >= 0 ? t : 0) * N + e;
      r[u] = rewards[i];
      m[u] = masks[i];
      v[u] = values[i];
      if constexpr (TR) tr[u] = truncs[i];
    }
#pragma unroll
    for (int u = 0; u < CH; ++u) {
      const int t = t0 - u;
      if (t >= 0) {
        const long i = (long)t * N + e;
        const double V = (double)v[u];
        if constexpr (EST == kEstGae) {
          if constexpr (TR) gae_step_tr(gamma, gl, r[u], m[u], tr[u], V, Vn, S);
          else gae_step(gamma, gl, r[u], m[u], V, Vn, S);
// ... 512 lines not shown
    heads_softmax_store(hi - lo, A, scratch, dst + (size_t)lo * A, nullptr, probs_out + (size_t)lo * A, values_out + lo, nullptr,
                        nullptr, nullptr);
  }
};
template <class H> struct HookOwnRows { static constexpr bool value = false; };
template <> struct HookOwnRows<RowsHeadsHook> { static constexpr bool value = true; };
struct FusedHeadsHook {
  const float (&pv)[64];
  float bias;
  int ntiles, N, A;
  float* probs_lds;
  float* probs_out;
  float* values_out;
  __device__ __forceinline__ void operator()(double* pj_buf, double* thr_s, int* any_zero) const {
    const int tid = threadIdx.x, lane = tid & 63;
    const int row = tid >> 3, a = tid & 7, J = A - 1;
    const bool rv = row < N;
    float acc = bias;
#pragma unroll
    for (int t = 0; t < 64; ++t) acc += (t < ntiles) ? pv[t] : 0.f;
    float lg[8];
#pragma unroll
    for (int j = 0; j < 8; ++j) lg[j] = __shfl(acc, (lane & ~7) | j, 64);
    float m = lg[0];
#pragma unroll
    for (int j = 1; j < 7; ++j)
      if (j < A) m = fmaxf(m, lg[j]);
    float sum = 0.f;
#pragma unroll
    for (int j = 0; j < 7; ++j)
      if (j < A) sum += expf(lg[j] - m);
    const float pa = expf(acc - m) / sum;
    if (rv && a < A) {
      probs_lds[row * A + a] = pa;
      probs_out[row * A + a] = pa;
    }
    if (rv && a == A) values_out[row] = acc;
    float pr[8];
#pragma unroll
    for (int j = 0; j < 8; ++j) pr[j] = __shfl(pa, (lane & ~7) | j, 64);
    if (rv && a < J) {
      double remaining = 1.0;
#pragma unroll
      for (int i = 0; i < 6; ++i)
        if (i < a) remaining -= (double)(pr[i] - 5.9604644775390625e-08f);
      const double p = (double)(pa - 5.9604644775390625e-08f);
      const double cond = p / remaining;
      pj_buf[row * J + a] = cond;
      if (cond == 0.0) *any_zero = 1;
      if (thr_s) thr_s[row * J + a] = mt_pack_threshold(cond);
    }
  }
};
template <class H> struct HookFused { static constexpr bool value = false; };
template <> struct HookFused<FusedHeadsHook> { static constexpr bool value = true; };
template <int LDSC, class HOOK = NoProbsHook>
__device__ __forceinline__ bool sample_mt_body(const float* __restrict__ probs, int N, int A,
                                               uint32_t* __restrict__ mt_state, double* __restrict__ pj_g,
                                               double* __restrict__ u_g, uint32_t* __restrict__ blocks_g,
                                               int32_t* __restrict__ actions, int16_t* act_lds,
                                               const float* probs_lds = nullptr, const uint32_t* stw_pre = nullptr,
                                               const HOOK probs_hook = HOOK(), const MultiWalk mw = MultiWalk{nullptr, nullptr, nullptr, 0},
                                               const MtAhead* __restrict__ ahead = nullptr) {
  constexpr bool HOOKED = !__is_same(HOOK, NoProbsHook);
  constexpr bool OWNROWS = HookOwnRows<HOOK>::value;
  constexpr bool FUSED = HookFused<HOOK>::value;
  MISC_STAMP(0);
  constexpr bool LDSPATH = LDSC > 0;
  constexpr int PRW = LDSC == 2 ? 18 : 8;
  __shared__ double pj_s[mt_lds_d(LDSC)];
  __shared__ double u_s[mt_lds_d(LDSC)];
  __shared__ uint32_t blocks_s[mt_lds_blk(LDSC) * 624];
  double* pj_buf = LDSPATH ? pj_s : pj_g;
  double* u_buf = LDSPATH ? u_s : u_g;
  uint32_t* blocks = LDSPATH ? blocks_s : blocks_g;
  const int tid = threadIdx.x;
  const int J = A - 1;
  const int D = N * J;
  __shared__ float probs_s[LDSPATH ? 2 * mt_lds_d(LDSC) : 1];
  __shared__ uint32_t pos_s;
  __shared__ int any_zero;
  uint32_t pos;
  constexpr int AHW = LDSC == 2 ? (MT_LDS_D2 + 255) / 256 : (LDSC == 1 ? MT_LDS_D / 256 : 1);
  double ahu[AHW];
  uint32_t ahk[5] = {0u, 0u, 0u, 0u, 0u};
  bool pre_ok = false;
  if (tid == 0) any_zero = 0;
  if constexpr (LDSPATH) {
    uint32_t stw[3];
    float prw[PRW];
    if (ahead) {
#pragma unroll
      for (int k = 0; k < 5; ++k) ahk[k] = ahead->hdr[k];
#pragma unroll
      for (int k = 0; k < AHW; ++k) ahu[k] = ahead->u[min(tid + k * 256, MT_LDS_D2 - 1)];
    }
#pragma unroll
    for (int k = 0; k < 3; ++k) stw[k] = stw_pre ? stw_pre[k] : mt_state[min(tid + k * 256, 624)];
    if (!probs_lds && !OWNROWS) {
#pragma unroll
      for (int k = 0; k < PRW; ++k) prw[k] = probs[min(tid + k * 256, N * A - 1)];
    }
#pragma unroll
    for (int k = 0; k < 3; ++k) {
      const int idx = tid + k * 256;
      if (idx < 624) blocks[idx] = stw[k];
      if (idx == 624) pos_s = stw[k];
    }
    if (!probs_lds && !OWNROWS) {
#pragma unroll
      for (int k = 0; k < PRW; ++k)
        if (tid + k * 256 < N * A) probs_s[tid + k * 256] = prw[k];
    }
    __syncthreads();
    pos = pos_s;
    if (ahead) {
      pre_ok = ahk[0] == pos && ahk[1] == blocks[0] && ahk[2] == blocks[1] && ahk[3] == blocks[623] && (int)ahk[4] >= N * J;
      if (pre_ok) {
#pragma unroll
        for (int k = 0; k < AHW; ++k)
          if (tid + k * 256 < N * J) u_buf[tid + k * 256] = ahu[k];
      }
    }
  } else {
    pos = mt_state[624];
  }
  MISC_STAMP(1);
  const float* pr = LDSPATH ? (probs_lds ? probs_lds : probs_s) : probs;
  const int nblk = (int)((pos + 2u * (uint32_t)D) / 624u) + 1;
  __shared__ __attribute__((aligned(16))) unsigned char jh_tab[mt_tab_max(LDSC)];
  const bool multi = LDSC == 2 && mw.W > 0;
  const bool walk_ok = (LDSC == 1 && N <= 32 && 4 + 48 * (J - 1) <= 256) || multi;
  double* thr_s = reinterpret_cast<double*>(jh_tab);
  unsigned char* inv_s = jh_tab + (LDSC == 0 ? 0 : 8 * mt_lds_d(LDSC));
  static_assert(LDSC == 0 || mt_tab_max(LDSC) >= 9 * mt_lds_d(LDSC), "threshold arrays reuse the table's LDS");
  auto phase1 = [&](const int e_lo, const int e_hi) {
    for (int d = e_lo * J + tid; d < e_hi * J; d += 256) {
      const int e = d / J, j = d - e * J;
      double remaining = 1.0;
      double p;
      if (LDSPATH && J <= 4) mt_row_inputs<4>(pr + (long)e * A, j, remaining, p);
      else if (LDSPATH && J <= 17) mt_row_inputs<17>(pr + (long)e * A, j, remaining, p);
      else {
        for (int i = 0; i < j; ++i)
          remaining -= (double)(pr[(long)e * A + i] - 5.9604644775390625e-08f);
        p = (double)(pr[(long)e * A + j] - 5.9604644775390625e-08f);
      }
      const double cond = p / remaining;
      pj_buf[d] = cond;
      if (LDSPATH && cond == 0.0) any_zero = 1;
      if (walk_ok) thr_s[d] = mt_pack_threshold(cond);
    }
  };
  int p1_lo = 0, p1_hi = N;
  if (multi) {
    if constexpr (!OWNROWS) {
      float pz[PRW];
#pragma unroll
      for (int k = 0; k < PRW; ++k) pz[k] = pr[min(tid + k * 256, N * A - 1)];
      bool z = false;
#pragma unroll
      for (int k = 0; k < PRW; ++k) z = z || ((pz[k] - 5.9604644775390625e-08f) == 0.0f);
      if (z) any_zero = 1;
    }
    const int NGm = (N + MW_G - 1) / MW_G;
    const long nwk = mw_first_walk(NGm, J - 1);
    const long w0 = (long)blockIdx.x * 256, w1 = w0 + 255 < nwk - 1 ? w0 + 255 : nwk - 1;
    if (w0 < nwk) {
      p1_lo = mw_group_of(w0, J - 1, NGm) * MW_G;
      p1_hi = (mw_group_of(w1, J - 1, NGm) + 1) * MW_G;
      p1_hi = p1_hi < N ? p1_hi : N;
    } else {
      p1_hi = 0;
    }
  }
  MISC_STAMP(13);
  if constexpr (!HOOKED) phase1(p1_lo, p1_hi);
  MISC_STAMP(2);
  if constexpr (!LDSPATH) {
    for (int i = tid; i < 624; i += 256) blocks[i] = mt_state[i];
  }
  __syncthreads();
  for (int b = 1; b < (pre_ok ? 1 : nblk); ++b) {
    const uint32_t* o = blocks + (long)(b - 1) * 624;
    uint32_t* nw = blocks + (long)b * 624;
    for (int k = tid; k < 227; k += 256) nw[k] = o[k + 397] ^ mt_mix(o[k], o[k + 1]);
    __syncthreads();
    for (int k = 227 + tid; k < 454; k += 256) nw[k] = nw[k - 227] ^ mt_mix(o[k], o[k + 1]);
    __syncthreads();
    for (int k = 454 + tid; k < 623; k += 256) nw[k] = nw[k - 227] ^ mt_mix(o[k], o[k + 1]);
    if (tid == 255) nw[623] = nw[396] ^ mt_mix(o[623], nw[0]);
    __syncthreads();
  }
  MISC_STAMP(3);
  for (int d = tid; d < (pre_ok ? 0 : D); d += 256) {
    const uint32_t q = pos + 2u * (uint32_t)d;
    const uint32_t a = mt_temper(blocks[q]) >> 5;
    const uint32_t b = mt_temper(blocks[q + 1]) >> 6;
    u_buf[d] = ((double)a * 67108864.0 + (double)b) * 1.1102230246251565404e-16;
  }
  __syncthreads();
  if constexpr (HOOKED) {
    if constexpr (OWNROWS) {
      probs_hook(probs_s, reinterpret_cast<float*>(jh_tab), p1_lo, p1_hi);
      for (int i = p1_lo * A + tid; i < p1_hi * A; i += 256)
        if ((pr[i] - 5.9604644775390625e-08f) == 0.0f) any_zero = 1;
    } else if constexpr (FUSED) {
      probs_hook(pj_buf, walk_ok ? thr_s : nullptr, &any_zero);
    } else {
      probs_hook();
    }
    if constexpr (!FUSED) phase1(p1_lo, p1_hi);
    __syncthreads();
  }
  MISC_STAMP(4);
  __shared__ unsigned short skip_tab[mt_skip_max(LDSC)];
  __shared__ int entry_s[33];
  bool chased = false;
  if constexpr (LDSPATH) {
    const long tab_entries = (long)N + (long)(J - 1) * N * (N - 1) / 2;
    bool walked = false;
    if constexpr (LDSC == 2) {
      if (multi) {
        if (!OWNROWS && any_zero) {
          if (blockIdx.x != 0) return false;
          phase1(0, N);
          __syncthreads();
        } else {
          unsigned short* exits_lds = reinterpret_cast<unsigned short*>(jh_tab + 9 * mt_lds_d(2));
          static_assert(mt_tab_max(2) >= 9 * MT_LDS_D2 + 2 * 16384, "exit offsets of up to 16 k walks next to the thresholds");
          int owner;
          const bool lz = OWNROWS && (any_zero != 0 || (int)blockIdx.x == g_dbg_zero_wg);
          switch (J) {
            case 1: owner = mt_multi_walks<1>(mw, thr_s, inv_s, u_buf, exits_lds, entry_s, &any_zero, N, J, D, actions, act_lds, OWNROWS, lz); break;
            case 2: owner = mt_multi_walks<2>(mw, thr_s, inv_s, u_buf, exits_lds, entry_s, &any_zero, N, J, D, actions, act_lds, OWNROWS, lz); break;
            case 3: owner = mt_multi_walks<3>(mw, thr_s, inv_s, u_buf, exits_lds, entry_s, &any_zero, N, J, D, actions, act_lds, OWNROWS, lz); break;
            case 5: owner = mt_multi_walks<5>(mw, thr_s, inv_s, u_buf, exits_lds, entry_s, &any_zero, N, J, D, actions, act_lds, OWNROWS, lz); break;
            case 8: owner = mt_multi_walks<8>(mw, thr_s, inv_s, u_buf, exits_lds, entry_s, &any_zero, N, J, D, actions, act_lds, OWNROWS, lz); break;
            case 17: owner = mt_multi_walks<17>(mw, thr_s, inv_s, u_buf, exits_lds, entry_s, &any_zero, N, J, D, actions, act_lds, OWNROWS, lz); break;
            default: owner = mt_multi_walks<0>(mw, thr_s, inv_s, u_buf, exits_lds, entry_s, &any_zero, N, J, D, actions, act_lds, OWNROWS, lz); break;
          }
          if (!owner) return false;
          if (owner == 2) {
            if constexpr (OWNROWS) probs_hook(probs_s, reinterpret_cast<float*>(jh_tab), 0, N);
            phase1(0, N);
            __syncthreads();
          } else {
            walked = true;
            chased = true;
          }
        }
      }
    }
    if constexpr (LDSC == 1) {
      if (!any_zero && walk_ok) {
        static_assert(mt_skip_max(1) >= 1024 + 256, "walk scratch");
        switch (J) {
#define PAAC_WALK_CASE(JJ) \
  case JJ: mt_group_walks<JJ, (mt_walks(4, JJ - 1) <= 256 ? 4 : 8)>(thr_s, u_buf, inv_s, skip_tab, entry_s, &any_zero, N, D, actions, act_lds); break;
          PAAC_WALK_CASE(1) PAAC_WALK_CASE(2) PAAC_WALK_CASE(3) PAAC_WALK_CASE(4) PAAC_WALK_CASE(5)
          default: mt_group_walks<6, 8>(thr_s, u_buf, inv_s, skip_tab, entry_s, &any_zero, N, D, actions, act_lds); break;
#undef PAAC_WALK_CASE
        }
        __syncthreads();
        walked = true;
        chased = true;
      }
    }
    if (!walked && tab_entries <= mt_tab_max(LDSC) && N <= 256) {
      if (!any_zero) {
// ... 250 lines not shown
    synth_bookkeep(synth_key(st.seed, st.env_offset + (uint32_t)e, id), e, actions, st.thresh, st.rec);
  synth_shift_band(st.seed, st.env_offset, id, st.thresh, e * PRE_BANDS + band, st.stack_in, st.stack_out, st.stack_out2,
                   force_reset != 0);
}

__device__ __forceinline__ void step_unit(const SynthStep& st, uint64_t id, int unit) {
  if (st.raw) synth_raw_unit(st.seed, st.env_offset, id, unit, st.raw);
  else synth_shift_band(st.seed, st.env_offset, id, st.thresh, unit, st.stack_in, st.stack_out, st.stack_out2);
}

template <int LDSC, bool FOLD = false>
__global__ __launch_bounds__(256) void synth_step_a_mt_kernel(const float* __restrict__ probs, int A,
                                                              uint32_t* __restrict__ mt_state,
                                                              int32_t* __restrict__ actions, const SynthStep st,
                                                              const MultiWalk mw, const MtAhead* __restrict__ ahead,
                                                              const RowsHeadsHook hs) {
  const int N = st.N;
  const uint64_t id = st.id();
  const int samplers = mw.W > 0 ? mw.W : 1;
  if ((int)blockIdx.x < samplers) {
    __shared__ int16_t act_s[mt_lds_d(LDSC)];
    const int e0 = threadIdx.x < N ? threadIdx.x : 0;
    const float ep_reward0 = st.active() ? st.rec.ep_reward[e0] : 0.f;
    const int32_t ep_len0 = st.active() ? st.rec.ep_len[e0] : 0;
    bool go_on;
    if constexpr (FOLD)
      go_on = sample_mt_body<LDSC, RowsHeadsHook>(nullptr, N, A, mt_state, nullptr, nullptr, nullptr, actions, act_s, nullptr, nullptr,
                                                  hs, mw, ahead);
    else
      go_on = sample_mt_body<LDSC>(probs, N, A, mt_state, nullptr, nullptr, nullptr, actions, act_s, nullptr, nullptr,
                                   NoProbsHook(), mw, ahead);
    if (!go_on || !st.active()) return;
    MISC_STAMP(7);
    for (int e = threadIdx.x; e < N; e += 256) {
      const uint32_t key = synth_key(st.seed, st.env_offset + (uint32_t)e, id);
      if (e < 256)
        synth_bookkeep_with(key, e, act_s[e], st.thresh, ep_reward0, ep_len0, st.rec);
      else
        synth_bookkeep_with(key, e, act_s[e], st.thresh, st.rec.ep_reward[e], st.rec.ep_len[e], st.rec);
    }
    MISC_STAMP(8);
    return;
  }
  if constexpr (LDSC == 2) {
    const int nshift = (int)gridDim.x - samplers;
    for (int u = (int)blockIdx.x - samplers; u < N * PRE_BANDS; u += nshift) {
      step_unit(st, id, u);
    }
  } else {
    step_unit(st, id, (int)blockIdx.x - samplers);
  }
}

__global__ __launch_bounds__(256) void synth_step_a_mth_kernel(const float* __restrict__ partial, int ntiles,
                                                               const float* __restrict__ ba, const float* __restrict__ bc,
                                                               float* __restrict__ probs_out, float* __restrict__ values_out,
                                                               int A, uint32_t* __restrict__ mt_state,
                                                               int32_t* __restrict__ actions, uint64_t seed,
                                                               uint32_t env_offset, int N, uint32_t thresh,
                                                               const uint64_t* __restrict__ step_base, uint64_t step_off,
                                                               const uint32_t* __restrict__ stack_in,
                                                               uint32_t* __restrict__ stack_out,
                                                               uint32_t* __restrict__ stack_out2, float* rewards_out,
                                                               float* masks_out, float* ep_reward, int32_t* ep_len,
                                                               FinishedRing* fin, uint32_t* __restrict__ raw,
                                                               const MtAhead* __restrict__ ahead) {
  const uint64_t id = (step_base ? *step_base : 0ull) + step_off + 1ull;
  if (blockIdx.x == 0) {
    __shared__ int16_t act_s[kFcHeadsMaxRows];
    __shared__ float lg_s[kFcHeadsMaxRows * 33];
    __shared__ float probs_sh[kFcHeadsMaxRows * 32];
    uint32_t stw[3];
#pragma unroll
    for (int k = 0; k < 3; ++k) stw[k] = mt_state[min((int)threadIdx.x + k * 256, 624)];
    const int e0 = threadIdx.x < N ? threadIdx.x : 0;
    const bool env_step = rewards_out != nullptr;
    const float ep_reward0 = env_step ? ep_reward[e0] : 0.f;
    const int32_t ep_len0 = env_step ? ep_len[e0] : 0;
    const uint32_t key0 = synth_key(seed, env_offset + (uint32_t)e0, id);
    const uint32_t hr5 = synth_reward_slot(key0);
    const bool term0 = synth_terminal(key0, thresh);
    if (N <= 32 && A <= 7 && ntiles <= 64) {
      float pv[64];
      const int row = (int)threadIdx.x >> 3, a = (int)threadIdx.x & 7;
      const int n = N * (A + 1);
      const int idx = (row < N && a <= A) ? row * (A + 1) + a : 0;
      const float bias = (a < A) ? ba[a] : bc[0];
#pragma unroll
      for (int t = 0; t < 64; ++t) pv[t] = partial[(size_t)(t < ntiles ? t : 0) * n + idx];
      sample_mt_body<1>(nullptr, N, A, mt_state, nullptr, nullptr, nullptr, actions, act_s, probs_sh, stw,
                        FusedHeadsHook{pv, bias, ntiles, N, A, probs_sh, probs_out, values_out},
                        MultiWalk{nullptr, nullptr, nullptr, 0}, ahead);
    } else {
      heads_from_partials(partial, ntiles, N, A, ba, bc, lg_s, probs_sh, nullptr, probs_out, values_out, nullptr, nullptr,
                          nullptr);
      sample_mt_body<1>(nullptr, N, A, mt_state, nullptr, nullptr, nullptr, actions, act_s, probs_sh, stw, NoProbsHook(),
                        MultiWalk{nullptr, nullptr, nullptr, 0}, ahead);
    }
    if (env_step && (int)threadIdx.x < N)
      synth_bookkeep_hashed(hr5, term0, e0, act_s[e0], ep_reward0, ep_len0, StepRecords{rewards_out, masks_out, ep_reward, ep_len, fin});
    return;
  }
  if (raw) synth_raw_unit(seed, env_offset, id, (int)blockIdx.x - 1, raw);
  else synth_shift_band(seed, env_offset, id, thresh, (int)blockIdx.x - 1, stack_in, stack_out, stack_out2);
}

__global__ __launch_bounds__(256) void synth_raw_kernel(const SynthStep st, const int32_t* __restrict__ actions,
                                                        int force_reset) {
  const int e = blockIdx.x;
  const uint64_t id = force_reset ? 0ull : st.id();
  const uint32_t key = synth_key(st.seed, st.env_offset + (uint32_t)e, id);
  if (!force_reset && blockIdx.y == 0 && threadIdx.x == 0) synth_bookkeep(key, e, actions, st.thresh, st.rec);
  uint32_t* __restrict__ raw = st.raw;
  const uint32_t rkey = key ^ 0x5bd1e995u;
  constexpr int WORDS = 2 * PAAC_RAW_H * PAAC_RAW_W / 4;
  uint4* out = reinterpret_cast<uint4*>(raw + (long)e * WORDS);
  for (int q = blockIdx.y * 256 + threadIdx.x; q < WORDS / 4; q += 256 * gridDim.y)
    out[q] = make_uint4(synth_word(rkey, (uint32_t)(4 * q)), synth_word(rkey, (uint32_t)(4 * q + 1)),
                        synth_word(rkey, (uint32_t)(4 * q + 2)), synth_word(rkey, (uint32_t)(4 * q + 3)));
}

static void launch_preprocess_after_step(const SynthStep& st, hipStream_t s) {
  ProfScope ps(g_prof_ctx, F_PREPROCESS_STACK, st.N, s);
  launch_k(preprocess_stack_kernel<false>, dim3(st.N, PRE_BANDS), dim3(256), s, PROF_WHOLE, (const uint8_t*)st.raw, st.N,
           st.stack_in, st.stack_out, st.stack_out2, (const uint8_t*)nullptr, (const uint8_t*)nullptr,
           (const float*)st.rec.masks);
}

int synth_step_of(const char* fn, const char* what, bool in_place_ok, SynthStep* st, uint64_t seed, uint32_t env_offset, int N,
                  uint32_t thresh, const uint64_t* step_base, uint64_t step_off, const uint8_t* stack_in, uint8_t* stack_out,
                  uint8_t* stack_out2, float* rewards, float* masks, float* ep_reward, int32_t* ep_len, void* finished,
                  uint8_t* raw_scratch) {
  PAAC_REQUIRE(stack_in && stack_out && rewards && masks && ep_reward && ep_len, "%s: %s", fn, what);
  PAAC_REQUIRE(in_place_ok || (stack_in != stack_out && stack_in != stack_out2), "%s: the step cannot shift the stacks in place",
               fn);
  *st = SynthStep{seed, env_offset, N, thresh, step_base, step_off, (const uint32_t*)stack_in, (uint32_t*)stack_out,
                  (uint32_t*)stack_out2, StepRecords{rewards, masks, ep_reward, ep_len, (FinishedRing*)finished},
                  (uint32_t*)raw_scratch};
  return 0;
}

int launch_sample_env_step_heads(const HeadsPartials& hp, float* probs_out, int A, uint32_t* mt_state, int32_t* actions,
                                 const SynthStep& st, const void* mt_ahead, hipStream_t s) {
  {
    ProfScope ps(g_prof_ctx, F_SAMPLE_ENV_STEP, st.N, s);
    launch_k(synth_step_a_mth_kernel, dim3(st.active() ? 1 + st.N * PRE_BANDS : 1), dim3(256), s, PROF_WHOLE, hp.partial,
             hp.ntiles, hp.ba, hp.bc, probs_out, hp.values_out, A, mt_state, actions, st.seed, st.env_offset, st.N, st.thresh,
             st.step_base, st.step_off, st.stack_in, st.stack_out, st.stack_out2, st.rec.rewards, st.rec.masks, st.rec.ep_reward,
             st.rec.ep_len, st.rec.fin, st.raw, reinterpret_cast<const MtAhead*>(mt_ahead));
  }
  if (st.raw) launch_preprocess_after_step(st, s);
  return 0;
}

int launch_returns_norm(const paac_returns* ret, const float* v_boot, float* adv_n, double* stats, hipStream_t s) {
  const TruncArgs rt = returns_args(ret, v_boot);
  if (rt.truncs) {
    launch_k(returns_norm_kernel<TruncArgs>, dim3(1), dim3(kNormThreads), s, PROF_WHOLE, rt, adv_n, stats);
  } else if (rt.gae) {
    const GaeArgs& rg = rt;
    launch_k(returns_norm_kernel<GaeArgs>, dim3(1), dim3(kNormThreads), s, PROF_WHOLE, rg, adv_n, stats);
  } else {
    const ReturnsArgs& rn = rt;
    launch_k(returns_norm_kernel<ReturnsArgs>, dim3(1), dim3(kNormThreads), s, PROF_WHOLE, rn, adv_n, stats);
  }
  return 0;
}

static int launch_returns_scan(const char* name, int estimator, const float* v_boot, const float* rewards, const float* masks,
                               const float* values, int T, int N, double gamma, double gae_lambda, float* y, float* adv,
                               const CycleTick& ct, paac_stream_t stream, const float* truncs = nullptr) {
  PAAC_REQUIRE(T > 0 && N > 0, "%s: T=%d N=%d", name, T, N);
  hipStream_t s = (hipStream_t)stream;
  ProfScope ps(g_prof_ctx, F_NSTEP_RETURNS, N * T, s);
  if (truncs) {
    auto* kernel = estimator == kEstGae ? returns_scan_kernel<kEstGae, const float*> : returns_scan_kernel<kEstNstep, const float*>;
    launch_k(kernel, dim3((N + 63) / 64), dim3(128), s, PROF_WHOLE, v_boot, rewards, masks, values, T, N, gamma,
             gamma * gae_lambda, y, adv, ct, truncs);
    PAAC_CHECK_HIP(hipGetLastError());
    return 0;
  }
  auto* kernel = estimator == kEstGae ? returns_scan_kernel<kEstGae> : returns_scan_kernel<kEstNstep>;
  launch_k(kernel, dim3((N + 63) / 64), dim3(128), s, PROF_WHOLE, v_boot, rewards, masks, values, T, N, gamma,
           gamma * gae_lambda, y, adv, ct, NoPlane{});
  PAAC_CHECK_HIP(hipGetLastError());
  return 0;
}

}

using namespace paac;

extern "C" {

#ifdef PAAC_DMM_STAMPS
void paac_debug_set_misc_stamps(unsigned long long* p) { (void)hipMemcpyToSymbol(HIP_SYMBOL(g_misc_stamps), &p, sizeof(p)); }
#endif

int paac_nstep_returns(const float* v_boot, const float* rewards, const float* masks, const float* values, int T, int N,
                       double gamma, float* y, float* adv, paac_stream_t stream) {
  return launch_returns_scan("paac_nstep_returns", kEstNstep, v_boot, rewards, masks, values, T, N, gamma, 0.0, y, adv,
                             CycleTick{}, stream);
}

int paac_nstep_returns_tick(const float* v_boot, const float* rewards, const float* masks, const float* values, int T,
// ... 317 lines not shown
```

paac_amd/csrc/net_fwd.hip:

```cpp
#include "net_common.h"
#include "tower.h"
#include "tower2.h"
#include "fc_heads.h"
#include "gemm3.h"

namespace paac {

#ifdef PAAC_DMM_STAMPS
unsigned long long* g_tower_stamps = nullptr;
extern "C" void paac_debug_set_tower_stamps(unsigned long long* p) { g_tower_stamps = p; }
unsigned long long* g_stamps = nullptr;
int g_stamp_which = -1, g_stamp_calls = 0;
extern "C" void paac_debug_set_stamps(unsigned long long* p, int which) {
  g_stamps = p;
  g_stamp_which = which;
  g_stamp_calls = 0;
}
#endif

template <class G, bool U8, int NDIM, int EPI>
static int launch_fwd(const GemmArgs& g, Tune t, hipStream_t s) {
  constexpr int VN = (NDIM % 64 == 0) ? 4 : (NDIM % 32 == 0) ? 2 : 1;
  int cfg = t.cfg, ksplit = 1, xcd = t.xcd;
  if constexpr (EPI == EPI_SLAB) {
// ... 167 lines not shown
  } else {
    if (keep) launch_tower_variant<TowerGeom<7, 7>, true>(a, s);
    else launch_tower_variant<TowerGeom<7, 7>, false>(a, s);
  }
}

template <class G, bool KEEP>
static void launch_tower2_variant(const Tower2Args& a, hipStream_t s) {
  launch_k(tower2_kernel<G, KEEP>, dim3((unsigned)(a.batch * G::NR)), dim3(512), s, PROF_WHOLE, a);
}

static void launch_tower2(paac_ctx* ctx, Workspace& W, const float* params, const uint8_t* states, int batch, bool keep,
                          bool packed2, hipStream_t s, Workspace* keepW = nullptr, int keep_row = 0) {
  const paac_layout& L = ctx->layout;
  Tower2Args a;
  a.states = states;
  const bf16x8* pk = reinterpret_cast<const bf16x8*>(ctx->tower_pack);
  a.w1p = pk;
  a.w2p = pk + kT2W1Vecs;
  a.b1 = params + L.offset[1];
  a.b2 = params + L.offset[3];
  a.act1 = W.act[0];
  a.act2 = W.act[1];
  a.batch = batch;
  a.act2_packed = packed2 ? 1 : 0;
  a.act2_rows = nullptr;
  if (keepW) {
    keep = true;
    a.act1 = keepW->act[0] + (size_t)keep_row * 400 * 16;
    if (packed2) a.act2_rows = keepW->act[1] + (size_t)keep_row * kT2Flat;
    else a.act2 = keepW->act[1] + (size_t)keep_row * kT2Flat;
  }
  const int force = ctx->tune[OP_CONV_TOWER][batch_class(batch)].cfg;
  int regions = (9 * batch <= 256) ? 9 : (4 * batch <= 256) ? 4 : 1;
  if (force == 1 || force == 4 || force == 9) regions = force;
  if (regions == 9) {
    if (keep) launch_tower2_variant<Tower2Geom<3, 3>, true>(a, s);
    else launch_tower2_variant<Tower2Geom<3, 3>, false>(a, s);
  } else if (regions == 4) {
    if (keep) launch_tower2_variant<Tower2Geom<5, 5>, true>(a, s);
    else launch_tower2_variant<Tower2Geom<5, 5>, false>(a, s);
  } else {
    if (keep) launch_tower2_variant<Tower2Geom<9, 9>, true>(a, s);
    else launch_tower2_variant<Tower2Geom<9, 9>, false>(a, s);
  }
}

template <class NT>
static int forward_impl(paac_ctx* ctx, int wsi, const float* params, const uint8_t* states, int batch, float* logits,
                        float* probs, float* values, const PhiloxArgs& ph, const SynthStep& st, hipStream_t s,
                        bool defer_heads = false, bool trunk_only = false) {
  const paac_layout& L = ctx->layout;
  Workspace& W = ctx->ws[wsi];
  ctx->last_ws = wsi;
  const int cls = batch_class(batch);
  const int A = ctx->cfg.num_actions;
  int t = 0;
  const float* w1 = params + L.offset[t++];
  const float* b1 = params + L.offset[t++];
  const float* w2 = params + L.offset[t++];
  const float* b2 = params + L.offset[t++];
  const float* w3 = nullptr;
  const float* b3 = nullptr;
  if constexpr (NT::NCONV == 3) {
    w3 = params + L.offset[t++];
    b3 = params + L.offset[t++];
  }
  const float* wf = params + L.offset[t++];
  const float* bf = params + L.offset[t++];
  const float* wa = params + L.offset[t++];
  const float* ba = params + L.offset[t++];
  const float* wc = params + L.offset[t++];
  const float* bc = params + L.offset[t++];

  bool tower = false;
  if constexpr (NT::NCONV == 3) tower = ctx->tower_on != 0;
  bool tower2 = false;
  if constexpr (NT::NCONV == 2 && kTower2) tower2 = ctx->tower2_on != 0;
  int keep_row = -1;
  bool keep_h_only = false;
  if (wsi == 0) {
    keep_row = ctx->keep_row;
    keep_h_only = ctx->keep_h_only != 0;
    ctx->keep_row = -1;
    ctx->keep_h_only = 0;
  }
  const bool keep_acts = wsi == 1 || !ctx->managed_weights;
  constexpr int NW = fc_heads_waves(NT::FLAT);
  const bool small_tail = NW > 0 && batch <= kFcHeadsMaxRows && !ph.enabled && !st.active();
  const bool mid_tail = !small_tail && (tower || tower2) && !keep_acts && wsi == 0 && batch <= kFcHeadsMidRows && !ph.enabled &&
                        !st.active() && !trunk_only;
  Workspace* keepW = nullptr;
  if (keep_row >= 0) {
    const bool generic_ok = !small_tail && !mid_tail && (ph.enabled || st.active()) && !defer_heads && !trunk_only;
    if (!((tower || tower2) && !keep_acts && (small_tail || mid_tail || generic_ok) && keep_row + batch <= ctx->max_batch)) {
      set_error("paac_keep_next_forward: rows [%d, %d) cannot be kept -- needs a stock trunk's conv tower, managed weights, an "
                "acting forward of at most %d rows (any size with the counter-based sampler) and keep_row + batch <= max_batch "
                "(%d)", keep_row, keep_row + batch, kFcHeadsMidRows, ctx->max_batch);
      return -1;
    }
    keepW = &ctx->ws[1];
  }
  const bool packed3 = (tower || tower2) && (small_tail || mid_tail) && !keep_acts;
  if (!ctx->managed_weights && (tower || tower2 || batch <= kFcHeadsMaxRows)) launch_pack_weights(ctx, params, s);
  if (tower) {
    ProfScope ps(ctx, F_CONV_TOWER, batch, s);
    prof_mix(3);
    prof_mix(6);
    launch_tower(ctx, W, params, states, batch, keep_acts, packed3, s, keep_h_only ? nullptr : keepW, keep_row < 0 ? 0 : keep_row);
  }
  if (tower2) {
    ProfScope ps(ctx, F_CONV_TOWER, batch, s);
    prof_mix(3);
    prof_mix(6);
    launch_tower2(ctx, W, params, states, batch, keep_acts, packed3, s, keep_h_only ? nullptr : keepW, keep_row < 0 ? 0 : keep_row);
  }
  if (!tower && !tower2) {
    ProfScope ps(ctx, F_CONV1_FWD, batch, s);
    constexpr int P1 = NT::G1::OPIX, F1 = NT::G1::FEATS;
    GemmArgs g = make_args(states, (size_t)batch * 28224, w1, (size_t)F1 * NT::C1 * 4, W.act[0], b1, batch * P1, NT::C1, F1, NT::C1, NT::C1);
    if (launch_fwd<typename NT::G1, true, NT::C1, EPI_BIAS_RELU>(g, ctx->tune[OP_CONV1_FWD][cls], s) < 0) return -1;
  }
  if (!tower && !tower2) {
    ProfScope ps(ctx, F_CONV2_FWD, batch, s);
    constexpr int P1 = NT::G1::OPIX, P2 = NT::G2::OPIX, F2 = NT::G2::FEATS;
    GemmArgs g = make_args(W.act[0], (size_t)batch * P1 * NT::C1 * 4, w2, (size_t)F2 * NT::C2 * 4, W.act[1], b2, batch * P2, NT::C2, F2, NT::C2, NT::C2);
    if (launch_fwd<typename NT::G2, false, NT::C2, EPI_BIAS_RELU>(g, ctx->tune[OP_CONV2_FWD][cls], s) < 0) return -1;
  }
  const float* last = W.act[1];
  if constexpr (NT::NCONV == 3) {
    last = W.act[2];
  }
  if (keepW && !keep_h_only && !packed3)
    last = keepW->act[NT::NCONV - 1] + (size_t)keep_row * NT::FLAT;
  if constexpr (NT::NCONV == 3) if (!tower) {
    ProfScope ps(ctx, F_CONV3_FWD, batch, s);
    constexpr int P2 = NT::G2::OPIX, P3 = NT::G3::OPIX, F3 = NT::G3::FEATS;
    GemmArgs g = make_args(W.act[1], (size_t)batch * P2 * NT::C2 * 4, w3, (size_t)F3 * NT::C3 * 4, W.act[2], b3, batch * P3, NT::C3, F3, NT::C3, NT::C3);
    if (launch_fwd<typename NT::G3, false, NT::C3, EPI_BIAS_RELU>(g, ctx->tune[OP_CONV3_FWD][cls], s) < 0) return -1;
    last = W.act[2];
  }
  if constexpr (NW > 0) if (small_tail || mid_tail) {
    if (wsi == 1) ctx->heads_pending_rows = 0;
    const bool quarter = fc_heads_quarter_ok(NT::FLAT) && ((batch + 7) / 8) * (NT::H / 8) <= 256 && !ctx->no_quarter_tiles &&
                         ctx->ahead_state == nullptr;
    const int NTILES = quarter ? NT::H / 8 : NT::H / 16;
    ctx->heads_ntiles = NTILES;
    float* partial = W.fc_slab;
    const bool keep_h = keep_acts;
    float* h_keep = keepW ? keepW->fc_slab + (size_t)keep_row * NT::H : nullptr;
    {
      ProfScope ps(ctx, F_FC_FWD, batch, s);
      prof_mix(1);
      MtAheadArgs ah{ctx->ahead_state, ctx->ahead_state ? reinterpret_cast<MtAhead*>(ctx->mt_ahead) : nullptr, ctx->ahead_D};
      ctx->ahead_state = nullptr;
      const unsigned grid = NTILES * ((batch + 15) / 16) + (ah.out ? 1 : 0);
      if constexpr (fc_heads_quarter_ok(NT::FLAT)) if (quarter) {
        if (packed3)
          launch_k(fc_heads_q_kernel<NT::FLAT, NT::H, NW, true>, dim3(NTILES * ((batch + 7) / 8)), dim3(64 * NW), s, PROF_WHOLE,
                   last, reinterpret_cast<const f32x4*>(ctx->fc_pack), bf, wa, wc, A, batch, partial, h_keep);
        else
          launch_k(fc_heads_q_kernel<NT::FLAT, NT::H, NW, false>, dim3(NTILES * ((batch + 7) / 8)), dim3(64 * NW), s, PROF_WHOLE,
                   last, reinterpret_cast<const f32x4*>(ctx->fc_pack), bf, wa, wc, A, batch, partial,
                   keep_h ? W.h : (float*)nullptr);
      }
      if (quarter) {
      } else if (packed3)
        launch_k(fc_heads_kernel<NT::FLAT, NT::H, NW, true>, dim3(grid), dim3(64 * NW), s, PROF_WHOLE,
                 last, reinterpret_cast<const f32x4*>(ctx->fc_pack), bf, wa, wc, A, batch, partial, h_keep, ah);
      else
        launch_k(fc_heads_kernel<NT::FLAT, NT::H, NW, false>, dim3(grid), dim3(64 * NW), s, PROF_WHOLE,
                 last, reinterpret_cast<const f32x4*>(ctx->fc_pack), bf, wa, wc, A, batch, partial,
                 keep_h ? W.h : (float*)nullptr, ah);
    }
    if (defer_heads) return 0;
    if (mid_tail) {
      ProfScope ps(ctx, F_HEADS_FWD, batch, s);
      const int rpw = 256 / (A + 1);
      launch_k(heads_finish_rows_kernel, dim3((batch + rpw - 1) / rpw), dim3(256), s, PROF_WHOLE, (const float*)partial, NTILES,
               batch, A, rpw, ba, bc, W.logits, W.probs, W.values, logits, probs, values);
    } else {
      ProfScope ps(ctx, F_HEADS_FWD, batch, s);
      launch_k(heads_finish_kernel, dim3(1), dim3(256), s, PROF_WHOLE, (const float*)partial, NTILES, batch, A, ba, bc,
               W.logits, W.probs, W.values, logits, probs, values);
    }
    return 0;
  }
  if (defer_heads) {
    set_error("forward: deferred heads need batch <= %d", kFcHeadsMaxRows);
    return -1;
  }
  int splits = 1;
  {
    ProfScope ps(ctx, F_FC_FWD, batch, s);
    GemmArgs g = make_args(last, (size_t)batch * NT::FLAT * 4, wf, (size_t)NT::FLAT * NT::H * 4, W.fc_slab, nullptr, batch, NT::H, NT::FLAT, NT::H, NT::H);
    g.slab_rows = batch;
    splits = launch_fc_gemm3(last, wf, W.fc_slab, batch, NT::FLAT, NT::H, s);
    if (splits == 0) splits = launch_fwd<typename NT::GFC, false, NT::H, EPI_SLAB>(g, ctx->tune[OP_FC_FWD][cls], s);
    if (splits < 0) return -1;
  }
  if (wsi == 1) ctx->heads_pending_rows = 0;
  if (trunk_only && wsi == 1) {
    ctx->heads_pending_rows = batch;
    ctx->heads_pending_splits = splits;
    ctx->heads_pending_h = 0;
    return 0;
  }
  {
    ProfScope ps(ctx, F_HEADS_FWD, batch, s);
    launch_heads_fwd<NT::H>(A, dim3(st.active() ? batch + batch * PRE_BANDS : batch), s, (const float*)W.fc_slab, splits,
                            (long)batch * NT::H, bf, wa, ba, wc, bc, A, keepW ? keepW->fc_slab + (size_t)keep_row * NT::H : W.h,
                            W.logits, W.probs, W.values, logits, probs, values, ph, batch, st);
  }
  return 0;
}

int launch_forward(paac_ctx* ctx, int ws, const float* params, const uint8_t* states, int batch, float* logits,
                   float* probs, float* values, hipStream_t s) {
  PhiloxArgs ph;
  memset(&ph, 0, sizeof(ph));
  const SynthStep st{};
  if (ctx->cfg.arch == PAAC_ARCH_NATURE)
    return forward_impl<NatureNet>(ctx, ws, params, states, batch, logits, probs, values, ph, st, s);
  return forward_impl<OtherNet>(ctx, ws, params, states, batch, logits, probs, values, ph, st, s);
}

// ... 23 lines not shown
  ProfScope ps(ctx, F_HEADS_FWD, rows, s);
  if (ctx->cfg.arch == PAAC_ARCH_NATURE)
    launch_heads_fwd<NatureNet::H>(A, dim3(rows), s, (const float*)W.fc_slab, ctx->heads_pending_splits, (long)rows * H, bf, wa,
                                   ba, wc, bc, A, W.h, W.logits, W.probs, W.values, (float*)nullptr, (float*)nullptr,
                                   (float*)nullptr, ph, rows, st);
  else
    launch_heads_fwd<OtherNet::H>(A, dim3(rows), s, (const float*)W.fc_slab, ctx->heads_pending_splits, (long)rows * H, bf, wa,
                                  ba, wc, bc, A, W.h, W.logits, W.probs, W.values, (float*)nullptr, (float*)nullptr,
                                  (float*)nullptr, ph, rows, st);
  return 0;
}

int launch_bootstrap_heads(paac_ctx* ctx, const float* params, int batch, int N, hipStream_t s) {
  const int rows = ctx->heads_pending_rows;
  if (rows <= 0) return 0;
  if (rows < batch + N) {
    set_error("paac_returns_norm_tick: the pending training forward covers %d rows, the bootstrap rows end at %d", rows, batch + N);
    return -1;
  }
  const paac_layout& L = ctx->layout;
  const int nt = L.num_tensors;
  Workspace& W = ctx->ws[1];
  PhiloxArgs ph;
  memset(&ph, 0, sizeof(ph));
  const SynthStep st{};
  const int A = ctx->cfg.num_actions, H = ctx->spec.fc;
  const float *bf = ctx->heads_pending_h ? ctx->zeros : params + L.offset[nt - 5], *wa = params + L.offset[nt - 4],
              *ba = params + L.offset[nt - 3], *wc = params + L.offset[nt - 2], *bc = params + L.offset[nt - 1];
  const size_t r0 = (size_t)batch;
  ProfScope ps(ctx, F_HEADS_FWD, N, s);
  if (ctx->cfg.arch == PAAC_ARCH_NATURE)
    launch_heads_fwd<NatureNet::H>(A, dim3(N), s, (const float*)W.fc_slab + r0 * H, ctx->heads_pending_splits, (long)rows * H, bf,
                                   wa, ba, wc, bc, A, W.h + r0 * H, W.logits + r0 * A, W.probs + r0 * A, W.values + r0,
                                   (float*)nullptr, (float*)nullptr, (float*)nullptr, ph, N, st);
  else
    launch_heads_fwd<OtherNet::H>(A, dim3(N), s, (const float*)W.fc_slab + r0 * H, ctx->heads_pending_splits, (long)rows * H, bf,
                                  wa, ba, wc, bc, A, W.h + r0 * H, W.logits + r0 * A, W.probs + r0 * A, W.values + r0,
                                  (float*)nullptr, (float*)nullptr, (float*)nullptr, ph, N, st);
  return 0;
}

bool forward_has_fc_heads(const paac_ctx* ctx) {
  return fc_heads_waves(ctx->cfg.arch == PAAC_ARCH_NATURE ? NatureNet::FLAT : OtherNet::FLAT) > 0;
}

int launch_forward_trunk(paac_ctx* ctx, const float* params, const uint8_t* states, int batch, HeadsPartials* hp, hipStream_t s) {
  PhiloxArgs ph;
  memset(&ph, 0, sizeof(ph));
  const SynthStep st{};
  const paac_layout& L = ctx->layout;
  const int nt = L.num_tensors;
  hp->ba = params + L.offset[nt - 3];
  hp->bc = params + L.offset[nt - 1];
  hp->partial = ctx->ws[0].fc_slab;
  const int rc = (ctx->cfg.arch == PAAC_ARCH_NATURE)
                     ? forward_impl<NatureNet>(ctx, 0, params, states, batch, nullptr, nullptr, nullptr, ph, st, s, true)
                     : forward_impl<OtherNet>(ctx, 0, params, states, batch, nullptr, nullptr, nullptr, ph, st, s, true);
  hp->ntiles = ctx->heads_ntiles;
  return rc;
}

int launch_bootstrap_trunk(paac_ctx* ctx, const float* params, const uint8_t* states, int batch, int train_row, hipStream_t s) {
  PhiloxArgs ph;
  memset(&ph, 0, sizeof(ph));
  const SynthStep st{};
  ctx->keep_row = train_row;
  ctx->keep_h_only = 1;
  int rc;
  if (ctx->cfg.arch == PAAC_ARCH_NATURE)
    rc = forward_impl<NatureNet>(ctx, 0, params, states, batch, nullptr, nullptr, nullptr, ph, st, s, true);
  else
    rc = forward_impl<OtherNet>(ctx, 0, params, states, batch, nullptr, nullptr, nullptr, ph, st, s, true);
  ctx->keep_row = -1;
  ctx->keep_h_only = 0;
  if (rc) return rc;
  ctx->heads_pending_rows = train_row + batch;
  ctx->heads_pending_splits = 1;
  ctx->heads_pending_h = 1;
  return 0;
}

int launch_forward_sample(paac_ctx* ctx, const float* params, const uint8_t* states, int batch, float* probs,
                          float* values, uint64_t seed, const uint64_t* step_base, uint64_t step_off,
                          uint32_t env_offset, int32_t* actions, const SynthStep* step, hipStream_t s) {
  const SynthStep st = step ? *step : SynthStep{};
  PhiloxArgs ph;
  ph.enabled = 1;
  ph.seed = seed;
  ph.step_base = step_base;
  ph.step_off = step_off;
  ph.env_offset = env_offset;
  ph.actions = actions;
  if (ctx->cfg.arch == PAAC_ARCH_NATURE)
    return forward_impl<NatureNet>(ctx, 0, params, states, batch, nullptr, probs, values, ph, st, s);
  return forward_impl<OtherNet>(ctx, 0, params, states, batch, nullptr, probs, values, ph, st, s);
}

#ifdef PAAC_DMM_STAMPS
extern "C" void paac_debug_set_heads_stamps(unsigned long long* p) {
  (void)hipMemcpyToSymbol(HIP_SYMBOL(g_stamps_dev), &p, sizeof(p));
}
#endif

int fc_splits_max() { return FC_SPLITS_MAX; }

}
```

paac_amd/csrc/synth_dev.h:

```cpp
#pragma once
#include "common.h"

namespace paac {

constexpr int PRE_BANDS = 7;

__device__ __forceinline__ uint32_t lowbias32(uint32_t x) {
  x ^= x >> 16; x *= 0x7feb352du; x ^= x >> 15; x *= 0x846ca68bu; x ^= x >> 16;
  return x;
}
__device__ __forceinline__ uint32_t synth_key(uint64_t seed, uint32_t env, uint64_t id) {
  uint32_t k = lowbias32((uint32_t)seed ^ lowbias32(env + 0x9E3779B9u));
  k = lowbias32(k ^ (uint32_t)(seed >> 32) ^ lowbias32((uint32_t)id * 0x85EBCA6Bu + (uint32_t)(id >> 32) + 0x7F4A7C15u));
  return k;
}
__device__ __forceinline__ uint32_t synth_word(uint32_t key, uint32_t w) { return lowbias32(key + w * 0x9E3779B9u + 0x165667B1u); }

struct FinishedRing {
  int32_t count;
  int32_t pad;
  float reward[4096];
  int32_t len[4096];
};

// ... 6 lines not shown
  float* truncs;
};

struct SynthStep {
  uint64_t seed;
  uint32_t env_offset;
  int N;
  uint32_t thresh;
  const uint64_t* step_base;
  uint64_t step_off;
  const uint32_t* stack_in;
  uint32_t *stack_out, *stack_out2;
  StepRecords rec;
  uint32_t* raw;
  __host__ __device__ bool active() const { return rec.rewards != nullptr; }
  __device__ uint64_t id() const { return (step_base ? *step_base : 0ull) + step_off + 1ull; }
};

__device__ __forceinline__ uint32_t synth_reward_slot(uint32_t key) { return lowbias32(key ^ 0xA511E9B3u) % 5u; }
__device__ __forceinline__ bool synth_terminal(uint32_t key, uint32_t thresh) { return lowbias32(key ^ 0x3C6EF372u) < thresh; }
__device__ __forceinline__ bool env_bookkeep(float r, bool term, int e, float ep_reward0, int32_t ep_len0, const StepRecords& rec) {
  rec.rewards[e] = fminf(fmaxf(r, -1.f), 1.f);
  rec.masks[e] = term ? 0.f : 1.f;
  const float tot = ep_reward0 + r;
  const int len = ep_len0 + 1;
  if (term) {
    if (rec.fin) {
      const int slot = atomicAdd(&rec.fin->count, 1) & 4095;
      rec.fin->reward[slot] = tot;
      rec.fin->len[slot] = len;
    }
    rec.ep_reward[e] = 0.f;
    rec.ep_len[e] = 0;
  } else {
    rec.ep_reward[e] = tot;
    rec.ep_len[e] = len;
  }
  return term;
}
__device__ __forceinline__ bool synth_bookkeep_hashed(uint32_t hr5, bool term, int e, int act, float ep_reward0,
                                                      int32_t ep_len0, const StepRecords& rec) {
  const float table[5] = {-2.f, 0.f, 0.f, 1.f, 3.f};
  return env_bookkeep(table[(hr5 + (uint32_t)act) % 5u], term, e, ep_reward0, ep_len0, rec);
}
__device__ __forceinline__ bool synth_bookkeep_with(uint32_t key, int e, int act, uint32_t thresh, float ep_reward0,
                                                    int32_t ep_len0, const StepRecords& rec) {
  return synth_bookkeep_hashed(synth_reward_slot(key), synth_terminal(key, thresh), e, act, ep_reward0, ep_len0, rec);
}
__device__ __forceinline__ bool synth_bookkeep(uint32_t key, int e, const int32_t* actions, uint32_t thresh,
                                               const StepRecords& rec) {
  return synth_bookkeep_with(key, e, actions ? actions[e] : 0, thresh, rec.ep_reward[e], rec.ep_len[e], rec);
}

__device__ __forceinline__ void synth_shift_band(uint64_t seed, uint32_t env_offset, uint64_t id, uint32_t thresh, int unit,
                                                 const uint32_t* __restrict__ stack_in, uint32_t* __restrict__ stack_out,
                                                 uint32_t* __restrict__ stack_out2 = nullptr,
                                                 const bool force_reset = false) {
  const int e = unit / PRE_BANDS;
  const int band = unit % PRE_BANDS;
  constexpr int QUADS_PER_BAND = OBS_PIX / PRE_BANDS / 4;
  const int i = threadIdx.x;
  if (i >= QUADS_PER_BAND) return;
  const int q = band * QUADS_PER_BAND + i;
  const long quad = (long)e * (OBS_PIX / 4) + q;
  uint4 old = force_reset ? make_uint4(0u, 0u, 0u, 0u) : reinterpret_cast<const uint4*>(stack_in)[quad];
  const uint32_t key = synth_key(seed, env_offset + (uint32_t)e, id);
  const bool reset = force_reset || lowbias32(key ^ 0x3C6EF372u) < thresh;
  if (reset) old = make_uint4(0u, 0u, 0u, 0u);
  const uint32_t w = synth_word(key, (uint32_t)q);
  const uint4 outv = make_uint4((old.x >> 8) | ((w & 255u) << 24), (old.y >> 8) | (((w >> 8) & 255u) << 24),
                                (old.z >> 8) | (((w >> 16) & 255u) << 24), (old.w >> 8) | ((w >> 24) << 24));
  reinterpret_cast<uint4*>(stack_out)[quad] = outv;
  if (stack_out2) reinterpret_cast<uint4*>(stack_out2)[quad] = outv;
}

__device__ __forceinline__ void synth_raw_unit(uint64_t seed, uint32_t env_offset, uint64_t id, int unit,
                                               uint32_t* __restrict__ raw) {
  const int e = unit / PRE_BANDS;
  const int part = unit % PRE_BANDS;
  const uint32_t rkey = synth_key(seed, env_offset + (uint32_t)e, id) ^ 0x5bd1e995u;
  constexpr int WORDS = 2 * PAAC_RAW_H * PAAC_RAW_W / 4;
  constexpr int PER = WORDS / 4 / PRE_BANDS;
  uint4* out = reinterpret_cast<uint4*>(raw + (long)e * WORDS);
  for (int q = part * PER + (int)threadIdx.x; q < (part + 1) * PER; q += 256)
    out[q] = make_uint4(synth_word(rkey, (uint32_t)(4 * q)), synth_word(rkey, (uint32_t)(4 * q + 1)),
                        synth_word(rkey, (uint32_t)(4 * q + 2)), synth_word(rkey, (uint32_t)(4 * q + 3)));
}

}
```

paac_amd/hip_ops.py:

```python
import ctypes
import functools
import gc

import numpy as np
import torch

from . import _lib

OBS_SHAPE = (84, 84, 4)
RAW_H, RAW_W = 210, 160
FINISHED_RING_BYTES = 8 + 4096 * 4 + 4096 * 4


def _stream():
    return ctypes.c_void_p(torch.cuda.current_stream().cuda_stream)


def _ptr(t, dtype, numel=None, name="tensor", optional=False):
    if t is None:
        if optional:
            return ctypes.c_void_p(0)
        raise ValueError("%s is required" % name)
    if not isinstance(t, torch.Tensor) or not t.is_cuda:
        raise ValueError("%s must be a CUDA/HIP torch tensor" % name)
# ... 273 lines not shown
            _ptr(gnorm_out, torch.float32, 1, "gnorm_out", True), *tail, _stream()), entry)

    def clip_rmsprop(self, params, grad, ms, mom, lr_dev, decay, momentum, eps, clip_norm, clip_mode, grad_scale=1.0,
                     gnorm_out=None):
        self._clip_step("paac_clip_rmsprop", params, grad, (("ms", ms), ("mom", mom)), (), lr_dev, (decay, momentum, eps),
                        clip_norm, clip_mode, grad_scale, gnorm_out)

    def clip_adam(self, params, grad, m, v, beta_powers, lr_dev, beta1, beta2, eps, clip_norm, clip_mode, grad_scale=1.0,
                  gnorm_out=None):
        self._clip_step("paac_clip_adam", params, grad, (("m", m), ("v", v)),
                        (_ptr(beta_powers, torch.float32, 2, "beta_powers"),), lr_dev, (beta1, beta2, eps), clip_norm,
                        clip_mode, grad_scale, gnorm_out)

    @staticmethod
    def _kl_gate(kl, scale, thr, first, stop, applied, checked):
        return _lib.KlGate(_ptr(kl, torch.float32, 1, "gate kl", True), float(scale), float(thr), 1 if first else 0,
                           _ptr(stop, torch.int32, 1, "gate stop", True), _ptr(applied, torch.int32, 1, "gate applied", True),
                           _ptr(checked, torch.float32, 1, "gate checked", True))

    def clip_rmsprop_gated(self, params, grad, ms, mom, lr_dev, decay, momentum, eps, clip_norm, clip_mode, grad_scale=1.0,
                           gnorm_out=None, *, kl, thr, first, stop, applied=None, checked=None, kl_scale=1.0):
        self._clip_step("paac_clip_rmsprop_gated", params, grad, (("ms", ms), ("mom", mom)), (), lr_dev,
                        (decay, momentum, eps), clip_norm, clip_mode, grad_scale, gnorm_out,
                        self._kl_gate(kl, kl_scale, thr, first, stop, applied, checked))

    def clip_adam_gated(self, params, grad, m, v, beta_powers, lr_dev, beta1, beta2, eps, clip_norm, clip_mode, grad_scale=1.0,
                        gnorm_out=None, *, kl, thr, first, stop, applied=None, checked=None, kl_scale=1.0):
        self._clip_step("paac_clip_adam_gated", params, grad, (("m", m), ("v", v)),
                        (_ptr(beta_powers, torch.float32, 2, "beta_powers"),), lr_dev, (beta1, beta2, eps), clip_norm,
                        clip_mode, grad_scale, gnorm_out,
                        self._kl_gate(kl, kl_scale, thr, first, stop, applied, checked))

    def keep_next_forward(self, train_row):
        _lib.check(self.lib.paac_keep_next_forward(self.handle, int(train_row)), "paac_keep_next_forward")

    def bootstrap_forward_trunk(self, params, states, train_row):
        B = self._check_states(states)
        _lib.check(self.lib.paac_bootstrap_forward_trunk(self.handle, _ptr(params, torch.float32, self.layout["total"], "params"),
                                                         _ptr(states, torch.uint8, B * 28224, "states"), B, int(train_row), _stream()),
                   "paac_bootstrap_forward_trunk")

    def act_step_mt(self, params, states, mt_state, actions, probs_out, values_out, env_seed, env_offset,
                    terminal_threshold, step_base_dev, step_offset, stack_out, rewards_out, masks_out, ep_reward, ep_len,
                    finished=None, stack_out2=None, raw_scratch=None, walk_scratch=None):
        N, A = self._check_states(states), self.num_actions
        if N > ACT_STEP_MAX_ENVS_LARGE or N * (A - 1) > FUSED_SAMPLE_MAX_DRAWS:
            raise ValueError("act_step_mt supports N <= %d and N*(A-1) <= %d" % (ACT_STEP_MAX_ENVS_LARGE, FUSED_SAMPLE_MAX_DRAWS))
        if stack_out is None:
            raise ValueError("stack_out is required")
        step = _step_ptrs(N, stack_out, rewards_out, masks_out, ep_reward, ep_len, finished, stack_out2, states=states)
        self._act(N, params, states, mt_state, actions, probs_out, values_out, step, env_seed, env_offset, terminal_threshold,
                  step_base_dev, step_offset, raw_scratch, walk_scratch)

    def act_mt(self, params, states, mt_state, actions, probs_out, values_out):
        N = self._check_states(states)
        self._act(N, params, states, mt_state, actions, probs_out, values_out, _step_ptrs(N))

    def _act(self, N, params, states, mt_state, actions, probs_out, values_out, step, env_seed=0, env_offset=0,
             terminal_threshold=0, step_base_dev=None, step_offset=0, raw_scratch=None, walk_scratch=None):
        A = self.num_actions
        _lib.check(self.lib.paac_act_step_mt(
            self.handle, _ptr(params, torch.float32, self.layout["total"], "params"),
            _ptr(states, torch.uint8, N * 28224, "states"), N, _ptr(mt_state, torch.int32, 625, "mt_state"),
            _ptr(actions, torch.int32, N, "actions"), _ptr(probs_out, torch.float32, N * A, "probs_out"),
            _ptr(values_out, torch.float32, N, "values_out"), int(env_seed), int(env_offset), int(terminal_threshold),
            _ptr(step_base_dev, torch.int64, 1, "step_base", True), int(step_offset), *step,
            _ptr(raw_scratch, torch.uint8, N * 2 * RAW_H * RAW_W, "raw_scratch", True),
            *_lent(walk_scratch), _stream()), "paac_act_step_mt")

    def pack_weights(self, params):
        _lib.check(self.lib.paac_pack_weights(self.handle, _ptr(params, torch.float32, self.layout["total"], "params"),
                                              _stream()), "paac_pack_weights")

    def set_managed_weights(self, on=True):
        _lib.check(self.lib.paac_set_managed_weights(self.handle, 1 if on else 0), "paac_set_managed_weights")

    def grad_stats(self, clip_norm, clip_mode):
        out = torch.zeros(8, dtype=torch.float32, device=self.device)
        _lib.check(self.lib.paac_grad_stats(self.handle, ctypes.c_void_p(out.data_ptr()), _stream()), "paac_grad_stats")
        s, ss, mx, mn = [float(v) for v in out.cpu().numpy()[:4].astype(np.float64)]
        n = float(self.layout["total_unpadded"])
        mean = s / n
        std = max(ss / n - mean * mean, 0.0) ** 0.5
        gn = ss ** 0.5
        raw = {"mean": mean, "stddev": std, "max": mx, "min": mn}
        if clip_mode == _lib.CLIP_LOCAL:
            ts = self.grad_tensor_stats()
            f = ts[:, 5]
            cs, css = float(np.sum(f * ts[:, 0])), float(np.sum(f * f * ts[:, 1]))
            cmean = cs / n
            return {"global_norm": css ** 0.5, "raw_gradients": raw,
                    "clipped_gradients": {"mean": cmean, "stddev": max(css / n - cmean * cmean, 0.0) ** 0.5,
                                          "max": float(np.max(f * ts[:, 2])), "min": float(np.min(f * ts[:, 3]))},
                    "tensors": {t["name"]: {"norm": float(ts[i, 1]) ** 0.5, "factor": float(f[i])}
                                for i, t in enumerate(self.layout["tensors"])}}
        f = 1.0
        if clip_mode == _lib.CLIP_GLOBAL and gn > 0.0:
            f = clip_norm * min(1.0 / gn, 1.0 / clip_norm)
        return {"global_norm": gn,
                "raw_gradients": raw,
                "clipped_gradients": {"mean": mean * f, "stddev": std * f, "max": mx * f, "min": mn * f}}

    def grad_tensor_stats(self):
        out = torch.zeros(_lib.MAX_TENSORS * 8, dtype=torch.float32, device=self.device)
        _lib.check(self.lib.paac_grad_tensor_stats(self.handle, ctypes.c_void_p(out.data_ptr()), _stream()),
                   "paac_grad_tensor_stats")
        return out.cpu().numpy().astype(np.float64).reshape(_lib.MAX_TENSORS, 8)[:len(self.layout["tensors"])]

    def debug_activation(self, what, batch):
        convs, fc = arch_geometry(self.arch)
        cap = int(batch) * self.num_actions if int(what) == 26 else activation_size(convs, fc, what, batch)
        if cap is None:
            raise ValueError("debug_activation: what=%d is not an activation of this geometry" % what)
        out = torch.empty(cap, dtype=torch.float32, device=self.device)
        n = self.lib.paac_debug_activation(self.handle, int(what), int(batch), ctypes.c_void_p(out.data_ptr()), cap, _stream())
        _lib.check(n, "paac_debug_activation")
        return out[:n].clone()

    def prof_enable(self, on=True):
        _lib.check(self.lib.paac_prof_enable(self.handle, 1 if on else 0), "paac_prof_enable")

# ... 376 lines not shown
    N, buffers, records = _game_step_ptrs(DUEL_STATE_WORDS, actions, state_in, state_out, state_out2, stack_in, stack_out,
                                          stack_out2, rewards_out, masks_out, ep_reward, ep_len, finished)
    ghost_stacks = _stack_ptrs(N, ("ghost_stack_out2",), ghost_stack_in=ghost_stack_in, ghost_stack_out=ghost_stack_out,
                               ghost_stack_out2=ghost_stack_out2)
    if ghost_probs.dim() != 2 or ghost_probs.shape[0] != N:
        raise ValueError("ghost_probs must be [%d, A], got %s" % (N, tuple(ghost_probs.shape)))
    A = ghost_probs.shape[1]
    env_offset = _env_offset("duel_ghost_step", env_offset, N)
    rec = _env_records(N, records, truncs_out)
    _lib.check(_lib.load().paac_duel_ghost_step(
        int(seed), env_offset, N, buffers[0], _ptr(ghost_probs, torch.float32, N * A, "ghost_probs"), A,
        int(sampler_seed) & 0xFFFFFFFFFFFFFFFF, _ptr(step_base_dev, torch.int64, 1, "step_base", True), int(step_offset),
        *buffers[1:], *ghost_stacks, ctypes.byref(rec), _ptr(ghost_actions_out, torch.int32, N, "ghost_actions_out"), _stream()),
        "paac_duel_ghost_step")


def _scored_step_args(fn, words, probs, greedy, eval_seed, noops, step_base_dev, step_offset, env_seed, env_offset, state_in,
                      state_out, stack_in, stack_out, actions_out, score, length, done, alive):
    if probs.dim() != 2:
        raise ValueError("probs must be [N, A], got %s" % (tuple(probs.shape),))
    N, A = probs.shape
    stacks = _stack_ptrs(N, stack_in=stack_in, stack_out=stack_out)
    states = _state_ptrs(N, words, state_in=state_in, state_out=state_out)
    env_offset = _env_offset(fn, env_offset, N)
    return [_ptr(probs, torch.float32, N * A, "probs"), N, A, 1 if greedy else 0, int(eval_seed) & 0xFFFFFFFFFFFFFFFF, int(noops),
            _ptr(step_base_dev, torch.int64, 1, "step_base", True), int(step_offset), int(env_seed) & 0xFFFFFFFFFFFFFFFF,
            env_offset, *states, *stacks, _ptr(actions_out, torch.int32, N, "actions_out"),
            _ptr(score, torch.float32, N, "score"), _ptr(length, torch.int32, N, "length"), _ptr(done, torch.int32, N, "done"),
            _ptr(alive, torch.int32, 1, "alive")]


def eval_step(game, probs, greedy, eval_seed, noops, step_base_dev, step_offset, env_seed, env_offset, state_in, state_out,
              stack_in, stack_out, actions_out, score, length, done, alive):
    if game not in EVAL_GAMES and game not in USER_GAMES:
        raise ValueError("eval_step: game %r has no device evaluation (--emulator catch|bricks|rally)" % (game,))
    game_id, words = EVAL_GAMES[game] if game in EVAL_GAMES else (USER_GAMES[game]["eval_id"], USER_GAMES[game]["words"])
    _lib.check(_lib.load().paac_eval_step(game_id, *_scored_step_args("eval_step", words, probs, greedy, eval_seed, noops, step_base_dev,
                                                                      step_offset, env_seed, env_offset, state_in, state_out,
                                                                      stack_in, stack_out, actions_out, score, length, done, alive),
                                          _stream()), "paac_eval_step")


def match_step(probs, greedy, eval_seed, noops, step_base_dev, step_offset, env_seed, env_offset, state_in, state_out,
               stack_in, stack_out, actions_out, score, length, done, alive):
    _lib.check(_lib.load().paac_match_step(*_scored_step_args("match_step", DUEL_STATE_WORDS, probs, greedy, eval_seed, noops,
                                                              step_base_dev, step_offset, env_seed, env_offset, state_in, state_out,
                                                              stack_in, stack_out, actions_out, score, length, done, alive),
                                           _stream()), "paac_match_step")


FUSED_SAMPLE_MAX_DRAWS = 2304
ACT_STEP_MAX_DRAWS = 1024
ACT_STEP_MAX_ENVS = 64
ACT_STEP_MAX_ENVS_LARGE = 256
KEEP_FORWARD_MAX_ROWS = 256


def walk_scratch(N, A, device):
    return torch.zeros(int(_lib.load().paac_walk_scratch_bytes(int(N), int(A))), dtype=torch.uint8, device=device)


def sample_mt_synth_step(probs, mt_state, actions, seed, env_offset, terminal_threshold, step_base_dev, step_offset,
                         stack_in, stack_out, rewards_out, masks_out, ep_reward, ep_len, finished=None, stack_out2=None,
                         walk_scratch=None, raw_scratch=None):
    N, A = probs.shape
    if N * (A - 1) > FUSED_SAMPLE_MAX_DRAWS:
        raise ValueError("fused sampler+env step supports N*(A-1) <= %d" % FUSED_SAMPLE_MAX_DRAWS)
    step = _step_ptrs(N, stack_out, rewards_out, masks_out, ep_reward, ep_len, finished, stack_out2, stack_in=stack_in)
    _lib.check(_lib.load().paac_sample_mt_synth_step(
        _ptr(probs, torch.float32, N * A, "probs"), A, _ptr(mt_state, torch.int32, 625, "mt_state"),
        _ptr(actions, torch.int32, N, "actions"), int(seed), int(env_offset), N, int(terminal_threshold),
        _ptr(step_base_dev, torch.int64, 1, "step_base", True), int(step_offset),
        _ptr(stack_in, torch.uint8, N * 28224, "stack_in"), *step,
        *_lent(walk_scratch), _ptr(raw_scratch, torch.uint8, N * 2 * RAW_H * RAW_W, "raw_scratch", True), _stream()),
        "paac_sample_mt_synth_step")


def pin_host_array(t):
    try:
        rc = torch.cuda.cudart().cudaHostRegister(t.data_ptr(), t.numel() * t.element_size(), 0)
        return int(rc) == 0
    except Exception:
        return False


def unpin_host_array(t):
    torch.cuda.cudart().cudaHostUnregister(t.data_ptr())


class Graph(object):

    def __init__(self):
        self.lib = _lib.load()
        self.handle = None

    def begin(self):
        gc.collect()
        self._gc_was_enabled = gc.isenabled()
        gc.disable()
        try:
            _lib.check(self.lib.paac_graph_begin(_stream()), "paac_graph_begin")
        except Exception:
            self._restore_gc()
            raise

    def _restore_gc(self):
# ... 28 lines not shown
```

paac_amd/paac.py:

```python
import functools
import logging
import os
import time

import numpy as np
import torch

from . import hip_ops, logger_utils, parallel
from .actor_learner import ActorLearner
from .runners import TRUNCATED_ATTRIBUTE, EmulatorRunner, RawEmulatorRunner, Runners


def _stateful_kind(kind, spec_kwargs, max_episode_steps, truncates):
    return dict(words=hip_ops.DEVICE_GAMES[kind]["words"], reset=functools.partial(hip_ops.game_reset, kind),
                step=functools.partial(hip_ops.game_step, kind), spec_kwargs=spec_kwargs, max_episode_steps=max_episode_steps,
                truncates=truncates)


STATEFUL_KINDS = {
    "catch": _stateful_kind("catch", (), 13, False),
    "bricks": _stateful_kind("bricks", ("single_life",), 500, True),
    "rally": _stateful_kind("rally", (), 1000, True),
}

PAIRED_KINDS = {
    "duel": dict(words=hip_ops.PAIRED_GAMES["duel"]["words"], reset=hip_ops.duel_reset, step=hip_ops.duel_step, spec_kwargs=(),
                 max_episode_steps=1000, truncates=True, eval_kind="rally"),
}


USER_KINDS = {}


def register_user_kind(spec_kwargs, max_episode_steps, truncates):
    USER_KINDS["user"] = dict(words=hip_ops.USER_GAMES["user"]["words"], reset=hip_ops.user_game_reset, step=hip_ops.user_game_step,
                              spec_kwargs=tuple(spec_kwargs), max_episode_steps=int(max_episode_steps), truncates=bool(truncates))
    return USER_KINDS["user"]


def stateful_kind(kind):
    return STATEFUL_KINDS.get(kind) or USER_KINDS.get(kind)


def device_kind(env_spec):
    kind = (env_spec or {}).get("kind", "synthetic")
    return STATEFUL_KINDS.get(kind) or PAIRED_KINDS.get(kind) or USER_KINDS.get(kind)


def eval_env_spec(env_spec, **changes):
    kind = None if env_spec is None else env_spec.get("kind", "synthetic")
    if kind in PAIRED_KINDS:
        return dict(kind=PAIRED_KINDS[kind]["eval_kind"], seed=changes.get("seed", env_spec["seed"]))
    return dict(env_spec, **changes) if env_spec is not None else None


class DeviceRollout(object):
    truncs = None
    pool = None

    def __init__(self, learner, env_spec, sampler="philox", sampler_seed=42, env_offset=0, use_graph=True,
                 total_envs=None):
        L = learner
        self.L = L
        dev = L.torch_device
        N, T, A = L.emulator_counts, L.max_local_steps, L.num_actions
        self.N, self.T, self.A = N, T, A
        self.total_envs = total_envs if total_envs is not None else N * L._world()
        self.env_spec = env_spec
        self.env_offset = int(env_offset)
        self.sampler = sampler
        self.sampler_seed = int(sampler_seed)
        self.use_graph = use_graph
        self.states = torch.zeros((2 * T + 1, N, 84, 84, 4), dtype=torch.uint8, device=dev)
        self.parity = 0
        self.actions = torch.zeros((T, N), dtype=torch.int32, device=dev)
        self.values = torch.zeros((T, N), dtype=torch.float32, device=dev)
        self.rewards = torch.zeros((T, N), dtype=torch.float32, device=dev)
        self.masks = torch.zeros((T, N), dtype=torch.float32, device=dev)
        self.probs = torch.zeros((N, A), dtype=torch.float32, device=dev)
        self.y = torch.zeros((T * N,), dtype=torch.float32, device=dev)
        self.adv = torch.zeros((T * N,), dtype=torch.float32, device=dev)
        self.ep_reward = torch.zeros((N,), dtype=torch.float32, device=dev)
        self.ep_len = torch.zeros((N,), dtype=torch.int32, device=dev)
        self.finished = torch.zeros((hip_ops.FINISHED_RING_BYTES // 4,), dtype=torch.int32, device=dev)
        self.tick = torch.zeros((1,), dtype=torch.int64, device=dev)
        self.global_step_dev = torch.full((1,), int(L.global_step), dtype=torch.int64, device=dev)
        self.cycle_tick = dict(global_step_dev=self.global_step_dev, increment=self.total_envs * T, initial_lr=L.initial_lr,
                               lr_annealing_steps=L.lr_annealing_steps, lr_out_dev=L.lr_dev, tick_dev=self.tick, tick_inc=T)
        self.raw = None
        self.stateful = device_kind(env_spec)
        if env_spec.get("kind") in PAIRED_KINDS and N % 2:
            raise ValueError("-ec / --emulator_counts %d: --emulator %s plays two rows per board and needs an even number of "
                             "environments per rank" % (N, env_spec["kind"]))
        self.catch = env_spec.get("kind", "synthetic") == "catch"
        self.env_state = None
        if self.stateful:
            self.env_state = torch.zeros((2 * T + 1, N, self.stateful["words"]), dtype=torch.int32, device=dev)
            self.env_step_kwargs = {k: env_spec[k] for k in self.stateful["spec_kwargs"]}
        if getattr(L, "bootstrap_truncated", False) and self.stateful and self.stateful["truncates"]:
            self.truncs = torch.zeros((T, N), dtype=torch.float32, device=dev)
        if env_spec.get("kind") == "duel" and int(env_spec.get("pool", 0) or 0) > 0:
            from . import duel_pool
            largs = getattr(L, "args", None)
            self.ghost_states = torch.zeros((2 * T + 1, N, 84, 84, 4), dtype=torch.uint8, device=dev)
            self.ghost_probs = torch.zeros((N, A), dtype=torch.float32, device=dev)
            self.ghost_actions = torch.zeros((T, N), dtype=torch.int32, device=dev)
            self.pool = duel_pool.DevicePool(L.network.params, L.network.arch_id, A, N, int(env_spec["pool"]),
                                             int(getattr(largs, "duel_pool_every", 102400)),
                                             float(getattr(largs, "duel_pool_latest_p", 0.5)),
                                             int(getattr(largs, "random_seed", env_spec["seed"])), int(L.global_step),
                                             device_index=dev.index or 0)
        self.walk_scratch = hip_ops.walk_scratch(N, A, dev) if N * (A - 1) <= hip_ops.FUSED_SAMPLE_MAX_DRAWS else None
        if env_spec.get("raw_frames"):
            self.raw = torch.zeros((N, 2, hip_ops.RAW_H, hip_ops.RAW_W), dtype=torch.uint8, device=dev)
        if sampler == "numpy":
            self.mt_state = hip_ops.mt_state_from_numpy(np.random.get_state(), dev)
            self.mt_scratch = hip_ops.sample_mt_scratch(N, A, dev)
        self.stream = torch.cuda.Stream(device=dev)
        self.graph_a = [None, None]
        self.graph_conv = [None, None]
        self.graph_b = None
        self.graph_multi = [None, None]
        self.graph_multi_long = [None, None]
        self.graph_ua = [None, None]
        self.pending_update = False
        self.phased = parallel.collectives_active()
        mode = os.environ.get("PAAC_ALLREDUCE", "graph")
        self.single_exchange = mode != "split"
        self.graph_exchange = self.phased and mode == "graph" and use_graph and parallel.backend() == "nccl"
        self.side_group = parallel.side_group() if (self.phased and not self.single_exchange) else None
        self.exchange_mode = "none" if not self.phased else ("split" if not self.single_exchange else "single")
        self.exchange_fallback = None
        self.K = L.ppo_steps
        if self.K > 1 and self.phased and not self.single_exchange:
            raise ValueError("--ppo_epochs above 1%s is not built for PAAC_ALLREDUCE=split (the two-piece exchange): use graph "
                             "or single" % (" with --ppo_minibatches above 1" if L.minibatch_on else ""))
        self.graph_epoch = [[], []]
        self.actor_adv = L.adv_n if L.adv_norm else self.adv
        self.short_first = os.environ.get("PAAC_SHORT_GRAPH_FIRST", "1") != "0"
        self.spin_sync = os.environ.get("PAAC_SPIN_SYNC", "1") != "0"
        self.verify_exchange = os.environ.get("PAAC_VERIFY_EXCHANGE", "1") != "0"
        self.tail_offset = [t["offset"] for t in L.network.layout["tensors"] if t["name"].startswith("fc")][0]
        towered = getattr(L.network, "ARCH", None) in ("NATURE", "NIPS") and os.environ.get("PAAC_TOWER", "1") != "0"
        self.act_step_large = os.environ.get("PAAC_MT_AHEAD", "1") != "0" and N <= hip_ops.ACT_STEP_MAX_ENVS_LARGE and towered
        self.reuse_acting = os.environ.get("PAAC_REUSE_ACTING", "1") != "0" and towered and N <= hip_ops.KEEP_FORWARD_MAX_ROWS
        self.route = self._route()
        self.records = [(self.rewards[t], self.masks[t], self.ep_reward, self.ep_len, self.finished) for t in range(T)]
        if self.pool is not None:
            hip_ops.duel_ghost_reset(env_spec["seed"], self.env_offset, self.env_state[0], self.states[0], self.ghost_states[0])
        elif self.stateful:
            self.stateful["reset"](env_spec["seed"], self.env_offset, self.env_state[0], self.states[0])
        else:
            hip_ops.synth_reset(env_spec["seed"], self.env_offset, self.states[0], self.raw)
        torch.cuda.synchronize(dev)

    def _slot(self, parity, t):
        return parity * self.T + t

    def rollout_states(self, parity=None):
        parity = (self.parity ^ 1) if parity is None else parity
        T, N = self.T, self.N
        return self.states[parity * T:(parity + 1) * T].view(T * N, 84, 84, 4)

    def _route(self):
        N, draws = self.N, self.N * (self.A - 1)
        if self.stateful:
            return "stateful"
        if self.sampler != "numpy":
            return "heads_step" if self.raw is None else "separate"
        if draws > hip_ops.FUSED_SAMPLE_MAX_DRAWS:
            return "separate"
        small = N <= hip_ops.ACT_STEP_MAX_ENVS and draws <= hip_ops.ACT_STEP_MAX_DRAWS
        return "act_step" if (self.act_step_large or small) else "fused"

    def _act_step(self, parity, t):
        L, route = self.L, self.route
        params, slot, records = L.network.params, self._slot(parity, t), self.records[t]
        obs, nxt = self.states[slot], self.states[slot + 1]
        wrap = self.states[0] if (parity == 1 and t == self.T - 1) else None
        seed = self.env_spec["seed"]
        if self.reuse_acting:
            L.ctx.keep_next_forward(t * self.N)
        if route == "act_step":
            L.ctx.act_step_mt(params, obs, self.mt_state, self.actions[t], self.probs, self.values[t], seed, self.env_offset,
                              self.env_spec["terminal_threshold"], self.tick, t, nxt, *records, stack_out2=wrap,
                              raw_scratch=self.raw, walk_scratch=self.walk_scratch)
        elif route == "heads_step":
            L.ctx.forward_sample_synth_step(params, obs, self.sampler_seed, self.tick, t, self.env_offset, self.actions[t], seed,
                                            self.env_spec["terminal_threshold"], nxt, *records, probs=self.probs,
                                            values=self.values[t])
            if wrap is not None:
                wrap.copy_(nxt)
        else:
            if self.sampler != "numpy":
                L.ctx.forward_sample(params, obs, self.sampler_seed, self.tick, t, self.env_offset, self.actions[t],
                                     probs=self.probs, values=self.values[t])
            else:
                L.ctx.forward(params, obs, probs=self.probs, values=self.values[t])
                if route != "fused":
                    hip_ops.sample_mt(self.probs, self.mt_state, self.mt_scratch, self.actions[t])
            if self.pool is not None:
                second = wrap is not None
                self.pool.ctx.forward(self.pool.opponent, self.ghost_states[slot], probs=self.ghost_probs)
                hip_ops.duel_ghost_step(seed, self.env_offset, self.actions[t], self.ghost_probs, self.sampler_seed, self.tick, t,
                                        self.env_state[slot], self.env_state[slot + 1], obs, nxt, self.ghost_states[slot],
                                        self.ghost_states[slot + 1], self.ghost_actions[t], *records, stack_out2=wrap,
                                        state_out2=self.env_state[0] if second else None,
                                        ghost_stack_out2=self.ghost_states[0] if second else None,
                                        truncs_out=self.truncs[t] if self.truncs is not None else None)
            elif route == "stateful":
                self.stateful["step"](seed, self.env_offset, self.actions[t], self.env_state[slot], self.env_state[slot + 1], obs,
                                      nxt, *records, stack_out2=wrap, state_out2=self.env_state[0] if wrap is not None else None,
                                      **(dict(truncs_out=self.truncs[t]) if self.truncs is not None else {}),
                                      **self.env_step_kwargs)
            elif route == "fused":
                hip_ops.sample_mt_synth_step(self.probs, self.mt_state, self.actions[t], seed, self.env_offset,
                                             self.env_spec["terminal_threshold"], self.tick, t, obs, nxt, *records,
                                             stack_out2=wrap, walk_scratch=self.walk_scratch, raw_scratch=self.raw)
            else:
                hip_ops.synth_step(seed, self.env_offset, self.actions[t], self.env_spec["terminal_threshold"], self.tick, t, obs,
                                   nxt, *records, stack_out2=wrap, raw_scratch=self.raw)

    def _rollout_and_backward(self, parity):
        L, T, N = self.L, self.T, self.N
        params = L.network.params
        keep = self.reuse_acting
        for t in range(T):
            self._act_step(parity, t)
        if keep:
            L.ctx.bootstrap_forward_trunk(params, self.states[self._slot(parity, T)], T * N)
        else:
            L.ctx.train_forward_trunk(params, self.states[parity * T:(parity + 1) * T + 1].view((T + 1) * N, 84, 84, 4))
        phase = ((0 if self.single_exchange else 1) if self.phased else 3)
        if L.minibatch_on:
            self._record_and_first_minibatch(parity, phase)
            return
# ... 768 lines not shown
```

Measured before the change: 750,800 env-steps/s.

## Pipeline acting step: defer sampling into next step's fc-heads kernel

Adds an act_step_pipe path in which each step's action sampling and bookkeeping is carried by the next forward's fc-heads kernel, or by the bootstrap forward, as a 'rider'. The env frame shift is also split into a load and a store around the fc MFMA loop. This removes separate sample and env-step launches from the critical path at small batch and overlaps them with the fc compute. It adds owed-state tracking with guards on the other entry points, and costs extra LDS and code complexity in the fc kernels. It is enabled by default for the act_step route with N<=64.

```diff
diff --git a/include/paac_hip.h b/include/paac_hip.h
--- a/include/paac_hip.h
+++ b/include/paac_hip.h
@@ -75,6 +75,15 @@
                      uint8_t* stack_out2, float* rewards_out, float* masks_out, float* ep_reward, int32_t* ep_len,
                      void* finished, uint8_t* raw_scratch, void* walk_scratch, int64_t walk_scratch_bytes,
                      paac_stream_t stream);
+
+int paac_act_step_pipe(paac_ctx* ctx, const float* params, const uint8_t* states, int batch, uint32_t* mt_state,
+                       int32_t* actions, float* probs_out, float* values_out, uint64_t env_seed, uint32_t env_offset,
+                       uint32_t terminal_threshold, const uint64_t* step_base_dev, uint64_t step_offset, uint8_t* stack_out,
+                       uint8_t* stack_out2, float* rewards_out, float* masks_out, float* ep_reward, int32_t* ep_len,
+                       void* finished, uint8_t* raw_scratch, void* walk_scratch, int64_t walk_scratch_bytes,
+                       paac_stream_t stream);
+int paac_act_step_flush(paac_ctx* ctx, paac_stream_t stream);
+int paac_act_step_pending(const paac_ctx* ctx);
 
 int paac_pack_weights(paac_ctx* ctx, const float* params, paac_stream_t stream);
 int paac_set_managed_weights(paac_ctx* ctx, int on);
diff --git a/paac_amd/_lib.py b/paac_amd/_lib.py
--- a/paac_amd/_lib.py
+++ b/paac_amd/_lib.py
@@ -135,6 +135,11 @@
     "paac_act_step_mt": (c_int, [c_void_p, c_void_p, c_void_p, c_int, c_void_p, c_void_p, c_void_p, c_void_p, c_uint64,
                                  c_uint32, c_uint32, c_void_p, c_uint64, c_void_p, c_void_p, c_void_p, c_void_p, c_void_p,
                                  c_void_p, c_void_p, c_void_p, c_void_p, c_int64, c_void_p]),
+    "paac_act_step_pipe": (c_int, [c_void_p, c_void_p, c_void_p, c_int, c_void_p, c_void_p, c_void_p, c_void_p, c_uint64,
+                                   c_uint32, c_uint32, c_void_p, c_uint64, c_void_p, c_void_p, c_void_p, c_void_p, c_void_p,
+                                   c_void_p, c_void_p, c_void_p, c_void_p, c_int64, c_void_p]),
+    "paac_act_step_flush": (c_int, [c_void_p, c_void_p]),
+    "paac_act_step_pending": (c_int, [c_void_p]),
     "paac_walk_scratch_bytes": (c_int64, [c_int, c_int]),
     "paac_debug_report_zero": (c_int, [c_int]),
     "paac_sample_mt_synth_step": (c_int, [c_void_p, c_int, c_void_p, c_void_p, c_uint64, c_uint32, c_int, c_uint32, c_void_p,
diff --git a/paac_amd/csrc/api.hip b/paac_amd/csrc/api.hip
--- a/paac_amd/csrc/api.hip
+++ b/paac_amd/csrc/api.hip
@@ -82,6 +82,11 @@
 
 using namespace paac;
 
+#define PAAC_NO_PENDING_SAMPLE(ctx, fn)                                                                                  \
+  PAAC_REQUIRE(!(ctx)->act_owed->partial, "%s: the last paac_act_step_pipe's sample is still pending (that step's actions, "  \
+               "values and records are not written yet): pay it with paac_bootstrap_forward_trunk, another "                \
+               "paac_act_step_pipe or paac_act_step_flush first", fn)
+
 struct paac_graph {
   hipGraph_t graph;
   hipGraphExec_t exec;
@@ -225,6 +230,10 @@
   PAAC_CHECK_HIP(hipMemset(c->mt_ahead, 0, mt_ahead_bytes()));
   c->ahead_state = nullptr;
   c->ahead_D = 0;
+  c->act_owed = new (std::nothrow) ActSample{};
+  PAAC_REQUIRE(c->act_owed, "paac_create: out of host memory");
+  c->fc_rider = nullptr;
+  c->act_region = 0;
   {
     const char* v = getenv("PAAC_TOWER");
     c->tower_on = (cfg->arch == PAAC_ARCH_NATURE) && !(v && *v && atoi(v) == 0);
@@ -278,6 +287,7 @@
   delete[] c->ev_family;
   delete[] c->ev_batch;
   delete[] c->ev_mix;
+  delete c->act_owed;
   delete c;
   return 0;
 }
@@ -341,7 +351,19 @@
   PAAC_REQUIRE(ctx && params && states, "paac_bootstrap_forward_trunk: null argument");
   PAAC_REQUIRE(batch > 0 && train_row >= 0 && train_row + batch <= ctx->max_batch,
                "paac_bootstrap_forward_trunk: rows [%d, %d) outside max_batch=%d", train_row, train_row + batch, ctx->max_batch);
+  ActRider rider{};
+  rider.owed = *ctx->act_owed;
+  if (rider.owed.partial) {
+    PAAC_REQUIRE(batch <= PAAC_ACT_STEP_MAX_ENVS && forward_has_fc_heads(ctx) &&
+                 (size_t)(ctx->spec.fc / 8) * batch * (ctx->cfg.num_actions + 1) <= act_region_floats(ctx),
+                 "paac_bootstrap_forward_trunk: a forward of %d rows cannot carry the pending sample of paac_act_step_pipe "
+                 "(paac_act_step_flush pays it)", batch);
+    ctx->fc_rider = &rider;
+  }
   const int rc = launch_bootstrap_trunk(ctx, params, states, batch, train_row, (hipStream_t)stream);
+  const bool carried = rider.owed.partial && ctx->fc_rider == nullptr;
+  ctx->fc_rider = nullptr;
+  if (carried) ctx->act_owed->partial = nullptr;
   if (rc) return rc;
   PAAC_CHECK_HIP(hipGetLastError());
   return 0;
@@ -473,6 +495,58 @@
   return 0;
 }
 
+int paac_act_step_pipe(paac_ctx* ctx, const float* params, const uint8_t* states, int batch, uint32_t* mt_state,
+                       int32_t* actions, float* probs_out, float* values_out, uint64_t env_seed, uint32_t env_offset,
+                       uint32_t terminal_threshold, const uint64_t* step_base_dev, uint64_t step_offset, uint8_t* stack_out,
+                       uint8_t* stack_out2, float* rewards_out, float* masks_out, float* ep_reward, int32_t* ep_len,
+                       void* finished, uint8_t* raw_scratch, void* walk_scratch, int64_t walk_scratch_bytes,
+                       paac_stream_t stream) {
+  (void)walk_scratch;
+  (void)walk_scratch_bytes;
+  PAAC_REQUIRE(ctx && params && states && mt_state && actions && probs_out && values_out, "paac_act_step_pipe: null argument");
+  PAAC_REQUIRE(!raw_scratch, "paac_act_step_pipe: path B (raw_scratch) keeps paac_act_step_mt's route -- its preprocess launch "
+               "follows the step");
+  SynthStep st;
+  if (synth_step_of("paac_act_step_pipe", "null argument (the pipelined step always steps the environments)", false, &st, env_seed,
+                    env_offset, batch, terminal_threshold, step_base_dev, step_offset, states, stack_out, stack_out2, rewards_out,
+                    masks_out, ep_reward, ep_len, finished, nullptr))
+    return -1;
+  const int A = ctx->cfg.num_actions;
+  PAAC_REQUIRE(batch > 0 && batch <= ctx->max_batch && batch <= PAAC_ACT_STEP_MAX_ENVS && (int64_t)batch * (A - 1) <= 1024 &&
+               forward_has_fc_heads(ctx),
+               "paac_act_step_pipe: up to min(max_batch=%d, %d) environments and 1024 draws on a geometry with the fc + head "
+               "partials kernel (use paac_act_step_mt); got %d x %d actions", ctx->max_batch, PAAC_ACT_STEP_MAX_ENVS, batch, A);
+  PAAC_REQUIRE((size_t)(ctx->spec.fc / 8) * batch * (A + 1) <= act_region_floats(ctx),
+               "paac_act_step_pipe: two regions of head partials for %d x %d actions do not fit the fc slab buffer of "
+               "max_batch=%d (use paac_act_step_mt)", batch, A, ctx->max_batch);
+  ActRider rider{};
+  rider.owed = *ctx->act_owed;
+  rider.shift = st;
+  HeadsPartials hp{nullptr, 0, nullptr, nullptr, values_out};
+  ctx->fc_rider = &rider;
+  const int rc = launch_forward_trunk(ctx, params, states, batch, &hp, (hipStream_t)stream);
+  const bool launched = ctx->fc_rider == nullptr;
+  ctx->fc_rider = nullptr;
+  if (launched)
+    *ctx->act_owed = ActSample{hp.partial, hp.ntiles, hp.ba, hp.bc, probs_out, values_out, A, mt_state, actions, env_seed,
+                               env_offset, batch, terminal_threshold, step_base_dev, step_offset, st.rec};
+  if (rc) return rc;
+  PAAC_CHECK_HIP(hipGetLastError());
+  return 0;
+}
+
+int paac_act_step_flush(paac_ctx* ctx, paac_stream_t stream) {
+  PAAC_REQUIRE(ctx, "paac_act_step_flush: null ctx");
+  if (!ctx->act_owed->partial) return 0;
+  const int rc = launch_act_sample_flush(*ctx->act_owed, (hipStream_t)stream);
+  if (rc) return rc;
+  ctx->act_owed->partial = nullptr;
+  PAAC_CHECK_HIP(hipGetLastError());
+  return 0;
+}
+
+int paac_act_step_pending(const paac_ctx* ctx) { return (ctx && ctx->act_owed->partial) ? 1 : 0; }
+
 static int check_returns(const char* fn, const paac_returns* ret) {
   PAAC_REQUIRE(ret->rewards && ret->masks && ret->values && ret->y_out && ret->adv_out, "%s: null rollout record", fn);
   PAAC_REQUIRE(returns_estimator(ret) == PAAC_RETURNS_NSTEP || returns_estimator(ret) == PAAC_RETURNS_GAE,
@@ -489,6 +563,7 @@
   PAAC_REQUIRE(ctx && params && states && actions && grad && (call.ret || (call.y && call.adv)), "%s: null argument", fn);
   PAAC_REQUIRE(batch > 0 && batch <= ctx->max_batch, "%s: batch %d outside (0, max_batch=%d]", fn, batch, ctx->max_batch);
   PAAC_REQUIRE(phase >= 0 && phase <= 3, "%s: phase %d", fn, phase);
+  PAAC_NO_PENDING_SAMPLE(ctx, fn);
   if (const paac_returns* ret = call.ret) {
     PAAC_REQUIRE(ret->T > 0 && ret->N > 0 && ret->T * ret->N == batch, "%s: T*N = %d*%d != batch %d", fn, ret->T, ret->N, batch);
     if (const int rc = check_returns(fn, ret)) return rc;
@@ -572,6 +647,7 @@
   PAAC_REQUIRE(ret && adv_n_out, "paac_returns_norm_tick: null argument");
   PAAC_REQUIRE(ret->T > 0 && ret->N > 0, "paac_returns_norm_tick: T=%d N=%d", ret->T, ret->N);
   if (const int rc = check_returns("paac_returns_norm_tick", ret)) return rc;
+  if (ctx) PAAC_NO_PENDING_SAMPLE(ctx, "paac_returns_norm_tick");
   const float* v_boot = ret->v_boot;
   if (!v_boot) {
     const int64_t batch = (int64_t)ret->T * ret->N;
@@ -593,6 +669,7 @@
   PAAC_REQUIRE(ctx && params, "paac_record_policy: null argument");
   PAAC_REQUIRE(p_old_out || v_out, "paac_record_policy: nothing to record (p_old_out and v_out are both NULL)");
   PAAC_REQUIRE(!p_old_out || actions, "paac_record_policy: p_old_out needs the actions");
+  PAAC_NO_PENDING_SAMPLE(ctx, "paac_record_policy");
   if (!p_old_out) batch = 0;
   if (!v_out) value_rows = 0;
   const int rows = batch > value_rows ? batch : value_rows;
diff --git a/paac_amd/csrc/common.h b/paac_amd/csrc/common.h
--- a/paac_amd/csrc/common.h
+++ b/paac_amd/csrc/common.h
@@ -96,6 +96,11 @@
   int nseg;
 };
 
+}
+
+namespace paac {
+struct ActSample;
+struct ActRider;
 }
 
 struct paac_ctx {
@@ -125,6 +130,9 @@
   void* mt_ahead;
   const uint32_t* ahead_state;
   int ahead_D;
+  paac::ActSample* act_owed;
+  const paac::ActRider* fc_rider;
+  int act_region;
   float* dl_buf;
   float* ppo_rows;
   float* vclip_rows;
@@ -133,6 +141,7 @@
   void* fc_pack;
   int tower_on;
   int heads_ntiles;
+  float* heads_partial;
   int no_quarter_tiles;
   int tower2_on;
   int managed_weights;
@@ -210,6 +219,11 @@
   const float *ba, *bc;
   float* values_out;
 };
+inline size_t act_region_floats(const paac_ctx* c) { return (size_t)c->fc_splits_max * c->max_batch * c->spec.fc / 2; }
+int launch_fc_heads_rider(bool nature, bool quarter, bool packed, unsigned fc_wgs, const float* act, const void* wfp,
+                          const float* bf, const float* wa, const float* wc, int A, int batch, float* partial, float* h_out,
+                          const ActRider& r, hipStream_t s);
+int launch_act_sample_flush(const ActSample& owed, hipStream_t s);
 size_t mt_ahead_bytes();
 bool sampler_folds_heads(int N, int A, const void* walk_scratch);
 bool tower2_available();
diff --git a/paac_amd/csrc/fc_heads.h b/paac_amd/csrc/fc_heads.h
--- a/paac_amd/csrc/fc_heads.h
+++ b/paac_amd/csrc/fc_heads.h
@@ -28,24 +28,36 @@
   out[i] = v;
 }
 
-template <int K, int H, int NW, bool A_PACKED>
+struct NoRider {};
+constexpr int kRiderLdsVecs = kFcHeadsMaxRows * 33 / 4;
+
+template <int K, int H, int NW, bool A_PACKED, class RIDER = NoRider>
 __global__ __launch_bounds__(64 * NW) void fc_heads_kernel(const float* __restrict__ act, const f32x4* __restrict__ wfp,
                                                            const float* __restrict__ bf, const float* __restrict__ Wa,
                                                            const float* __restrict__ Wc, const int A, const int B,
                                                            float* __restrict__ partial, float* __restrict__ h_out,
-                                                           const MtAheadArgs ahead) {
+                                                           const MtAheadArgs ahead, const RIDER rider) {
   constexpr int NTILES = H / 16, G = K / 16, GPW = G / NW, PF = 8;
+  constexpr bool RIDDEN = !__is_same(RIDER, NoRider);
   static_assert(K % 16 == 0 && H % 16 == 0 && G % NW == 0 && GPW > PF, "fc geometry");
-  if (ahead.out != nullptr && blockIdx.x == gridDim.x - 1) {
-    __shared__ uint32_t ahead_blocks[MT_AHEAD_BLK * 624];
-    mt_produce_ahead<64 * NW>(ahead, ahead_blocks);
-    return;
-  }
-  __shared__ f32x4 red[NW * 64];
+  if constexpr (!RIDDEN) {
+    if (ahead.out != nullptr && blockIdx.x == gridDim.x - 1) {
+      __shared__ uint32_t ahead_blocks[MT_AHEAD_BLK * 624];
+      mt_produce_ahead<64 * NW>(ahead, ahead_blocks);
+      return;
+    }
+  }
+  __shared__ f32x4 red[RIDDEN && kRiderLdsVecs > NW * 64 ? kRiderLdsVecs : NW * 64];
+  int bid = blockIdx.x, nfc = gridDim.x;
+  uint4 shift_old = make_uint4(0u, 0u, 0u, 0u);
+  if constexpr (RIDDEN) {
+    if (rider.front(bid, nfc, reinterpret_cast<float*>(red))) return;
+    shift_old = rider.shift_load(bid);
+  }
   const int tid = threadIdx.x, lane = tid & 63;
   const int wave = __builtin_amdgcn_readfirstlane(tid >> 6);
   const int li = lane & 15, kq = lane >> 4;
-  const int nt = blockIdx.x % NTILES, mt = blockIdx.x / NTILES;
+  const int nt = bid % NTILES, mt = bid / NTILES;
   const int row_a = mt * 16 + li;
   const bool row_ok = row_a < B;
   const int col = nt * 16 + li;
@@ -83,6 +95,7 @@
       acc = __builtin_amdgcn_mfma_f32_16x16x4f32(row_ok ? fa[i % RING][e] : 0.f, fb[i % RING][e], acc, 0, 0, 0);
     __builtin_amdgcn_sched_barrier(0);
   }
+  if constexpr (RIDDEN) rider.shift_store(bid, nfc, shift_old);
   red[wave * 64 + lane] = acc;
   __syncthreads();
   f32x4 h = red[lane];
@@ -121,19 +134,27 @@
   }
 }
 
-template <int K, int H, int NW, bool A_PACKED>
+template <int K, int H, int NW, bool A_PACKED, class RIDER = NoRider>
 __global__ __launch_bounds__(64 * NW) void fc_heads_q_kernel(const float* __restrict__ act, const f32x4* __restrict__ wfp,
                                                              const float* __restrict__ bf, const float* __restrict__ Wa,
                                                              const float* __restrict__ Wc, const int A, const int B,
-                                                             float* __restrict__ partial, float* __restrict__ h_out) {
+                                                             float* __restrict__ partial, float* __restrict__ h_out,
+                                                             const RIDER rider) {
   constexpr int NTILES = H / 8, G = K / 16, GPW = G / NW, NS = GPW / 2, PF = 6;
+  constexpr bool RIDDEN = !__is_same(RIDER, NoRider);
   static_assert(K % 16 == 0 && H % 16 == 0 && G % NW == 0 && GPW % 2 == 0 && NS > PF, "fc geometry");
-  __shared__ f32x4 red[NW * 64];
+  __shared__ f32x4 red[RIDDEN && kRiderLdsVecs > NW * 64 ? kRiderLdsVecs : NW * 64];
+  int bid = blockIdx.x, nfc = gridDim.x;
+  uint4 shift_old = make_uint4(0u, 0u, 0u, 0u);
+  if constexpr (RIDDEN) {
+    if (rider.front(bid, nfc, reinterpret_cast<float*>(red))) return;
+    shift_old = rider.shift_load(bid);
+  }
   const int tid = threadIdx.x, lane = tid & 63;
   const int wave = __builtin_amdgcn_readfirstlane(tid >> 6);
   const int li = lane & 15, kq = lane >> 4;
   const int l8 = li & 7, odd = li >> 3;
-  const int nt = blockIdx.x % NTILES, mt = blockIdx.x / NTILES;
+  const int nt = bid % NTILES, mt = bid / NTILES;
   const int row_a = mt * 8 + l8;
   const bool row_ok = row_a < B;
   const int col = nt * 8 + l8;
@@ -172,6 +193,7 @@
       acc = __builtin_amdgcn_mfma_f32_16x16x4f32(row_ok ? fa[i % RING][e] : 0.f, fb[i % RING][e], acc, 0, 0, 0);
     __builtin_amdgcn_sched_barrier(0);
   }
+  if constexpr (RIDDEN) rider.shift_store(bid, nfc, shift_old);
   red[wave * 64 + lane] = acc;
   __syncthreads();
   const bool own = li < 8 && kq < 2;
diff --git a/paac_amd/csrc/misc.hip b/paac_amd/csrc/misc.hip
--- a/paac_amd/csrc/misc.hip
+++ b/paac_amd/csrc/misc.hip
@@ -1,5 +1,6 @@
 #include "common.h"
 #include "synth_dev.h"
+#include "net_common.h"
 #include "fc_heads.h"
 #include "heads.h"
 
@@ -618,9 +619,25 @@
     }
   }
 };
+template <int LDSC>
+struct MtLds {
+  double pj[mt_lds_d(LDSC)];
+  double u[mt_lds_d(LDSC)];
+  uint32_t blocks[mt_lds_blk(LDSC) * 624];
+  __attribute__((aligned(16))) unsigned char jh_tab[mt_tab_max(LDSC)];
+  unsigned short skip_tab[mt_skip_max(LDSC)];
+  int entry[33];
+  uint32_t pos;
+  int any_zero;
+};
+template <int LDSC, int SET>
+__device__ __forceinline__ MtLds<LDSC>& mt_lds() {
+  __shared__ MtLds<LDSC> lds;
+  return lds;
+}
 template <class H> struct HookFused { static constexpr bool value = false; };
 template <> struct HookFused<FusedHeadsHook> { static constexpr bool value = true; };
-template <int LDSC, class HOOK = NoProbsHook>
+template <int LDSC, class HOOK = NoProbsHook, int SET = 0>
 __device__ __forceinline__ bool sample_mt_body(const float* __restrict__ probs, int N, int A,
                                                uint32_t* __restrict__ mt_state, double* __restrict__ pj_g,
                                                double* __restrict__ u_g, uint32_t* __restrict__ blocks_g,
@@ -634,9 +651,10 @@
   MISC_STAMP(0);
   constexpr bool LDSPATH = LDSC > 0;
   constexpr int PRW = LDSC == 2 ? 18 : 8;
-  __shared__ double pj_s[mt_lds_d(LDSC)];
-  __shared__ double u_s[mt_lds_d(LDSC)];
-  __shared__ uint32_t blocks_s[mt_lds_blk(LDSC) * 624];
+  MtLds<LDSC>& lds = mt_lds<LDSC, SET>();
+  double* const pj_s = lds.pj;
+  double* const u_s = lds.u;
+  uint32_t* const blocks_s = lds.blocks;
   double* pj_buf = LDSPATH ? pj_s : pj_g;
   double* u_buf = LDSPATH ? u_s : u_g;
   uint32_t* blocks = LDSPATH ? blocks_s : blocks_g;
@@ -644,8 +662,8 @@
   const int J = A - 1;
   const int D = N * J;
   __shared__ float probs_s[LDSPATH ? 2 * mt_lds_d(LDSC) : 1];
-  __shared__ uint32_t pos_s;
-  __shared__ int any_zero;
+  uint32_t& pos_s = lds.pos;
+  int& any_zero = lds.any_zero;
   uint32_t pos;
   constexpr int AHW = LDSC == 2 ? (MT_LDS_D2 + 255) / 256 : (LDSC == 1 ? MT_LDS_D / 256 : 1);
   double ahu[AHW];
@@ -694,7 +712,7 @@
   MISC_STAMP(1);
   const float* pr = LDSPATH ? (probs_lds ? probs_lds : probs_s) : probs;
   const int nblk = (int)((pos + 2u * (uint32_t)D) / 624u) + 1;
-  __shared__ __attribute__((aligned(16))) unsigned char jh_tab[mt_tab_max(LDSC)];
+  unsigned char* const jh_tab = lds.jh_tab;
   const bool multi = LDSC == 2 && mw.W > 0;
   const bool walk_ok = (LDSC == 1 && N <= 32 && 4 + 48 * (J - 1) <= 256) || multi;
   double* thr_s = reinterpret_cast<double*>(jh_tab);
@@ -780,8 +798,8 @@
     __syncthreads();
   }
   MISC_STAMP(4);
-  __shared__ unsigned short skip_tab[mt_skip_max(LDSC)];
-  __shared__ int entry_s[33];
+  unsigned short* const skip_tab = lds.skip_tab;
+  int* const entry_s = lds.entry;
   bool chased = false;
   if constexpr (LDSPATH) {
     const long tab_entries = (long)N + (long)(J - 1) * N * (N - 1) / 2;
@@ -1138,6 +1156,47 @@
   }
 }
 
+template <bool ONE_SET>
+__device__ __forceinline__ void act_sample_body(const float* __restrict__ partial, int ntiles, const float* __restrict__ ba,
+                                                const float* __restrict__ bc, float* __restrict__ probs_out,
+                                                float* __restrict__ values_out, int A, uint32_t* __restrict__ mt_state,
+                                                int32_t* __restrict__ actions, uint64_t seed, uint32_t env_offset, int N,
+                                                uint32_t thresh, uint64_t id, float* rewards_out, float* masks_out,
+                                                float* ep_reward, int32_t* ep_len, FinishedRing* fin,
+                                                const MtAhead* __restrict__ ahead, float* lg_s) {
+  __shared__ int16_t act_s[kFcHeadsMaxRows];
+  __shared__ float probs_sh[kFcHeadsMaxRows * 32];
+  uint32_t stw[3];
+#pragma unroll
+  for (int k = 0; k < 3; ++k) stw[k] = mt_state[min((int)threadIdx.x + k * 256, 624)];
+  const int e0 = threadIdx.x < N ? threadIdx.x : 0;
+  const bool env_step = rewards_out != nullptr;
+  const float ep_reward0 = env_step ? ep_reward[e0] : 0.f;
+  const int32_t ep_len0 = env_step ? ep_len[e0] : 0;
+  const uint32_t key0 = synth_key(seed, env_offset + (uint32_t)e0, id);
+  const uint32_t hr5 = synth_reward_slot(key0);
+  const bool term0 = synth_terminal(key0, thresh);
+  if (N <= 32 && A <= 7 && ntiles <= 64) {
+    float pv[64];
+    const int row = (int)threadIdx.x >> 3, a = (int)threadIdx.x & 7;
+    const int n = N * (A + 1);
+    const int idx = (row < N && a <= A) ? row * (A + 1) + a : 0;
+    const float bias = (a < A) ? ba[a] : bc[0];
+#pragma unroll
+    for (int t = 0; t < 64; ++t) pv[t] = partial[(size_t)(t < ntiles ? t : 0) * n + idx];
+    sample_mt_body<1, FusedHeadsHook, ONE_SET ? 0 : 1>(nullptr, N, A, mt_state, nullptr, nullptr, nullptr, actions, act_s, probs_sh, stw,
+                      FusedHeadsHook{pv, bias, ntiles, N, A, probs_sh, probs_out, values_out},
+                      MultiWalk{nullptr, nullptr, nullptr, 0}, ahead);
+  } else {
+    heads_from_partials(partial, ntiles, N, A, ba, bc, lg_s, probs_sh, nullptr, probs_out, values_out, nullptr, nullptr,
+                        nullptr);
+    sample_mt_body<1>(nullptr, N, A, mt_state, nullptr, nullptr, nullptr, actions, act_s, probs_sh, stw, NoProbsHook(),
+                      MultiWalk{nullptr, nullptr, nullptr, 0}, ahead);
+  }
+  if (env_step && (int)threadIdx.x < N)
+    synth_bookkeep_hashed(hr5, term0, e0, act_s[e0], ep_reward0, ep_len0, StepRecords{rewards_out, masks_out, ep_reward, ep_len, fin});
+}
+
 __global__ __launch_bounds__(256) void synth_step_a_mth_kernel(const float* __restrict__ partial, int ntiles,
                                                                const float* __restrict__ ba, const float* __restrict__ bc,
                                                                float* __restrict__ probs_out, float* __restrict__ values_out,
@@ -1153,42 +1212,53 @@
                                                                const MtAhead* __restrict__ ahead) {
   const uint64_t id = (step_base ? *step_base : 0ull) + step_off + 1ull;
   if (blockIdx.x == 0) {
-    __shared__ int16_t act_s[kFcHeadsMaxRows];
     __shared__ float lg_s[kFcHeadsMaxRows * 33];
-    __shared__ float probs_sh[kFcHeadsMaxRows * 32];
-    uint32_t stw[3];
-#pragma unroll
-    for (int k = 0; k < 3; ++k) stw[k] = mt_state[min((int)threadIdx.x + k * 256, 624)];
-    const int e0 = threadIdx.x < N ? threadIdx.x : 0;
-    const bool env_step = rewards_out != nullptr;
-    const float ep_reward0 = env_step ? ep_reward[e0] : 0.f;
-    const int32_t ep_len0 = env_step ? ep_len[e0] : 0;
-    const uint32_t key0 = synth_key(seed, env_offset + (uint32_t)e0, id);
-    const uint32_t hr5 = synth_reward_slot(key0);
-    const bool term0 = synth_terminal(key0, thresh);
-    if (N <= 32 && A <= 7 && ntiles <= 64) {
-      float pv[64];
-      const int row = (int)threadIdx.x >> 3, a = (int)threadIdx.x & 7;
-      const int n = N * (A + 1);
-      const int idx = (row < N && a <= A) ? row * (A + 1) + a : 0;
-      const float bias = (a < A) ? ba[a] : bc[0];
-#pragma unroll
-      for (int t = 0; t < 64; ++t) pv[t] = partial[(size_t)(t < ntiles ? t : 0) * n + idx];
-      sample_mt_body<1>(nullptr, N, A, mt_state, nullptr, nullptr, nullptr, actions, act_s, probs_sh, stw,
-                        FusedHeadsHook{pv, bias, ntiles, N, A, probs_sh, probs_out, values_out},
-                        MultiWalk{nullptr, nullptr, nullptr, 0}, ahead);
-    } else {
-      heads_from_partials(partial, ntiles, N, A, ba, bc, lg_s, probs_sh, nullptr, probs_out, values_out, nullptr, nullptr,
-                          nullptr);
-      sample_mt_body<1>(nullptr, N, A, mt_state, nullptr, nullptr, nullptr, actions, act_s, probs_sh, stw, NoProbsHook(),
-                        MultiWalk{nullptr, nullptr, nullptr, 0}, ahead);
-    }
-    if (env_step && (int)threadIdx.x < N)
-      synth_bookkeep_hashed(hr5, term0, e0, act_s[e0], ep_reward0, ep_len0, StepRecords{rewards_out, masks_out, ep_reward, ep_len, fin});
+    act_sample_body<false>(partial, ntiles, ba, bc, probs_out, values_out, A, mt_state, actions, seed, env_offset, N, thresh, id,
+                    rewards_out, masks_out, ep_reward, ep_len, fin, ahead, lg_s);
     return;
   }
   if (raw) synth_raw_unit(seed, env_offset, id, (int)blockIdx.x - 1, raw);
   else synth_shift_band(seed, env_offset, id, thresh, (int)blockIdx.x - 1, stack_in, stack_out, stack_out2);
+}
+
+struct ActRiderDev {
+  ActRider r;
+  __device__ __forceinline__ bool front(int& bid, int& nfc, float* lds) const {
+    const int ns = r.owed.partial ? 1 : 0;
+    if (bid < ns) {
+      if (threadIdx.x >= 256) return true;
+      const ActSample& o = r.owed;
+      const uint64_t id = (o.step_base ? *o.step_base : 0ull) + o.step_off + 1ull;
+      act_sample_body<true>(o.partial, o.ntiles, o.ba, o.bc, o.probs_out, o.values_out, o.A, o.mt_state, o.actions, o.seed,
+                      o.env_offset, o.N, o.thresh, id, o.rec.rewards, o.rec.masks, o.rec.ep_reward, o.rec.ep_len, o.rec.fin,
+                      nullptr, lds);
+      return true;
+    }
+    bid -= ns;
+    nfc -= ns;
+    return false;
+  }
+  __device__ __forceinline__ uint4 shift_load(const int bid) const {
+    const SynthStep& st = r.shift;
+    if (st.stack_in == nullptr || threadIdx.x >= 256 || bid >= st.N * PRE_BANDS) return make_uint4(0u, 0u, 0u, 0u);
+    return synth_shift_load(bid, st.stack_in);
+  }
+  __device__ __forceinline__ void shift_store(const int bid, const int nfc, const uint4 old) const {
+    const SynthStep& st = r.shift;
+    if (st.stack_in == nullptr || threadIdx.x >= 256) return;
+    const uint64_t id = st.id();
+    const int units = st.N * PRE_BANDS;
+    if (bid < units) synth_shift_store(st.seed, st.env_offset, id, st.thresh, bid, old, st.stack_out, st.stack_out2);
+    for (int u = bid + nfc; u < units; u += nfc)
+      synth_shift_band(st.seed, st.env_offset, id, st.thresh, u, st.stack_in, st.stack_out, st.stack_out2);
+  }
+};
+
+__global__ __launch_bounds__(256) void act_sample_flush_kernel(const ActSample o) {
+  __shared__ float lg_s[kFcHeadsMaxRows * 33];
+  const uint64_t id = (o.step_base ? *o.step_base : 0ull) + o.step_off + 1ull;
+  act_sample_body<true>(o.partial, o.ntiles, o.ba, o.bc, o.probs_out, o.values_out, o.A, o.mt_state, o.actions, o.seed, o.env_offset,
+                  o.N, o.thresh, id, o.rec.rewards, o.rec.masks, o.rec.ep_reward, o.rec.ep_len, o.rec.fin, nullptr, lg_s);
 }
 
 __global__ __launch_bounds__(256) void synth_raw_kernel(const SynthStep st, const int32_t* __restrict__ actions,
@@ -1237,6 +1307,49 @@
   }
   if (st.raw) launch_preprocess_after_step(st, s);
   return 0;
+}
+
+int launch_act_sample_flush(const ActSample& owed, hipStream_t s) {
+  ProfScope ps(g_prof_ctx, F_SAMPLE_ENV_STEP, owed.N, s);
+  launch_k(act_sample_flush_kernel, dim3(1), dim3(256), s, PROF_WHOLE, owed);
+  return 0;
+}
+
+template <class NT>
+static int launch_fc_rider_of(bool quarter, bool packed, unsigned fc_wgs, const float* act, const void* wfp, const float* bf,
+                              const float* wa, const float* wc, int A, int batch, float* partial, float* h_out,
+                              const ActRider& r, hipStream_t s) {
+  constexpr int NW = fc_heads_waves(NT::FLAT);
+  if constexpr (NW > 0) {
+    const ActRiderDev rd{r};
+    const dim3 grid(fc_wgs + (r.owed.partial ? 1u : 0u)), block(64 * NW);
+    const f32x4* w = reinterpret_cast<const f32x4*>(wfp);
+    if constexpr (fc_heads_quarter_ok(NT::FLAT)) if (quarter) {
+      if (packed) launch_k(fc_heads_q_kernel<NT::FLAT, NT::H, NW, true, ActRiderDev>, grid, block, s, PROF_WHOLE, act, w, bf, wa, wc,
+                           A, batch, partial, h_out, rd);
+      else launch_k(fc_heads_q_kernel<NT::FLAT, NT::H, NW, false, ActRiderDev>, grid, block, s, PROF_WHOLE, act, w, bf, wa, wc, A,
+                    batch, partial, h_out, rd);
+      return 0;
+    }
+    if (quarter) {
+      set_error("fc rider: no quarter-tile kernel for this geometry");
+      return -1;
+    }
+    const MtAheadArgs none{nullptr, nullptr, 0};
+    if (packed) launch_k(fc_heads_kernel<NT::FLAT, NT::H, NW, true, ActRiderDev>, grid, block, s, PROF_WHOLE, act, w, bf, wa, wc, A,
+                         batch, partial, h_out, none, rd);
+    else launch_k(fc_heads_kernel<NT::FLAT, NT::H, NW, false, ActRiderDev>, grid, block, s, PROF_WHOLE, act, w, bf, wa, wc, A, batch,
+                  partial, h_out, none, rd);
+    return 0;
+  }
+  set_error("fc rider: this geometry has no fc + head partials kernel");
+  return -1;
+}
+int launch_fc_heads_rider(bool nature, bool quarter, bool packed, unsigned fc_wgs, const float* act, const void* wfp,
+                          const float* bf, const float* wa, const float* wc, int A, int batch, float* partial, float* h_out,
+                          const ActRider& r, hipStream_t s) {
+  if (nature) return launch_fc_rider_of<NatureNet>(quarter, packed, fc_wgs, act, wfp, bf, wa, wc, A, batch, partial, h_out, r, s);
+  return launch_fc_rider_of<OtherNet>(quarter, packed, fc_wgs, act, wfp, bf, wa, wc, A, batch, partial, h_out, r, s);
 }
 
 int launch_returns_norm(const paac_returns* ret, const float* v_boot, float* adv_n, double* stats, hipStream_t s) {
diff --git a/paac_amd/csrc/net_fwd.hip b/paac_amd/csrc/net_fwd.hip
--- a/paac_amd/csrc/net_fwd.hip
+++ b/paac_amd/csrc/net_fwd.hip
@@ -243,6 +243,11 @@
                         bool defer_heads = false, bool trunk_only = false) {
   const paac_layout& L = ctx->layout;
   Workspace& W = ctx->ws[wsi];
+  if (wsi == 0 && ctx->act_owed->partial && !ctx->fc_rider) {
+    set_error("forward: the last paac_act_step_pipe's sample is still pending: pay it with paac_bootstrap_forward_trunk, another "
+              "paac_act_step_pipe or paac_act_step_flush before another acting forward (paac_act_step_mt, paac_forward*)");
+    return -1;
+  }
   ctx->last_ws = wsi;
   const int cls = batch_class(batch);
   const int A = ctx->cfg.num_actions;
@@ -281,6 +286,10 @@
   const bool small_tail = NW > 0 && batch <= kFcHeadsMaxRows && !ph.enabled && !st.active();
   const bool mid_tail = !small_tail && (tower || tower2) && !keep_acts && wsi == 0 && batch <= kFcHeadsMidRows && !ph.enabled &&
                         !st.active() && !trunk_only;
+  if (wsi == 0 && ctx->fc_rider && (!small_tail || ctx->ahead_state)) {
+    set_error("forward: the fc launch's riders need the small acting route without the spare MT19937 workgroup");
+    return -1;
+  }
   Workspace* keepW = nullptr;
   if (keep_row >= 0) {
     const bool generic_ok = !small_tail && !mid_tail && (ph.enabled || st.active()) && !defer_heads && !trunk_only;
@@ -338,6 +347,9 @@
     const int NTILES = quarter ? NT::H / 8 : NT::H / 16;
     ctx->heads_ntiles = NTILES;
     float* partial = W.fc_slab;
+    const ActRider* rider = wsi == 0 ? ctx->fc_rider : nullptr;
+    if (rider) partial += (size_t)ctx->act_region * act_region_floats(ctx);
+    ctx->heads_partial = partial;
     const bool keep_h = keep_acts;
     float* h_keep = keepW ? keepW->fc_slab + (size_t)keep_row * NT::H : nullptr;
     {
@@ -346,23 +358,32 @@
       MtAheadArgs ah{ctx->ahead_state, ctx->ahead_state ? reinterpret_cast<MtAhead*>(ctx->mt_ahead) : nullptr, ctx->ahead_D};
       ctx->ahead_state = nullptr;
       const unsigned grid = NTILES * ((batch + 15) / 16) + (ah.out ? 1 : 0);
+      if (rider) {
+        const unsigned fc_wgs = quarter ? NTILES * ((batch + 7) / 8) : NTILES * ((batch + 15) / 16);
+        if (launch_fc_heads_rider(ctx->cfg.arch == PAAC_ARCH_NATURE, quarter, packed3, fc_wgs, last,
+                                  ctx->fc_pack, bf, wa, wc, A, batch, partial, packed3 ? h_keep : (keep_h ? W.h : (float*)nullptr),
+                                  *rider, s))
+          return -1;
+        ctx->fc_rider = nullptr;
+        ctx->act_region ^= 1;
+      } else
       if constexpr (fc_heads_quarter_ok(NT::FLAT)) if (quarter) {
         if (packed3)
           launch_k(fc_heads_q_kernel<NT::FLAT, NT::H, NW, true>, dim3(NTILES * ((batch + 7) / 8)), dim3(64 * NW), s, PROF_WHOLE,
-                   last, reinterpret_cast<const f32x4*>(ctx->fc_pack), bf, wa, wc, A, batch, partial, h_keep);
+                   last, reinterpret_cast<const f32x4*>(ctx->fc_pack), bf, wa, wc, A, batch, partial, h_keep, NoRider{});
         else
           launch_k(fc_heads_q_kernel<NT::FLAT, NT::H, NW, false>, dim3(NTILES * ((batch + 7) / 8)), dim3(64 * NW), s, PROF_WHOLE,
                    last, reinterpret_cast<const f32x4*>(ctx->fc_pack), bf, wa, wc, A, batch, partial,
-                   keep_h ? W.h : (float*)nullptr);
+                   keep_h ? W.h : (float*)nullptr, NoRider{});
       }
-      if (quarter) {
+      if (quarter || rider) {
       } else if (packed3)
         launch_k(fc_heads_kernel<NT::FLAT, NT::H, NW, true>, dim3(grid), dim3(64 * NW), s, PROF_WHOLE,
-                 last, reinterpret_cast<const f32x4*>(ctx->fc_pack), bf, wa, wc, A, batch, partial, h_keep, ah);
+                 last, reinterpret_cast<const f32x4*>(ctx->fc_pack), bf, wa, wc, A, batch, partial, h_keep, ah, NoRider{});
       else
         launch_k(fc_heads_kernel<NT::FLAT, NT::H, NW, false>, dim3(grid), dim3(64 * NW), s, PROF_WHOLE,
                  last, reinterpret_cast<const f32x4*>(ctx->fc_pack), bf, wa, wc, A, batch, partial,
-                 keep_h ? W.h : (float*)nullptr, ah);
+                 keep_h ? W.h : (float*)nullptr, ah, NoRider{});
     }
     if (defer_heads) return 0;
     if (mid_tail) {
@@ -492,10 +513,10 @@
   const int nt = L.num_tensors;
   hp->ba = params + L.offset[nt - 3];
   hp->bc = params + L.offset[nt - 1];
-  hp->partial = ctx->ws[0].fc_slab;
   const int rc = (ctx->cfg.arch == PAAC_ARCH_NATURE)
                      ? forward_impl<NatureNet>(ctx, 0, params, states, batch, nullptr, nullptr, nullptr, ph, st, s, true)
                      : forward_impl<OtherNet>(ctx, 0, params, states, batch, nullptr, nullptr, nullptr, ph, st, s, true);
+  hp->partial = ctx->heads_partial;
   hp->ntiles = ctx->heads_ntiles;
   return rc;
 }
diff --git a/paac_amd/csrc/synth_dev.h b/paac_amd/csrc/synth_dev.h
--- a/paac_amd/csrc/synth_dev.h
+++ b/paac_amd/csrc/synth_dev.h
@@ -82,18 +82,22 @@
   return synth_bookkeep_with(key, e, actions ? actions[e] : 0, thresh, rec.ep_reward[e], rec.ep_len[e], rec);
 }
 
-__device__ __forceinline__ void synth_shift_band(uint64_t seed, uint32_t env_offset, uint64_t id, uint32_t thresh, int unit,
-                                                 const uint32_t* __restrict__ stack_in, uint32_t* __restrict__ stack_out,
-                                                 uint32_t* __restrict__ stack_out2 = nullptr,
-                                                 const bool force_reset = false) {
+constexpr int SHIFT_QUADS = OBS_PIX / PRE_BANDS / 4;
+__device__ __forceinline__ uint4 synth_shift_load(int unit, const uint32_t* __restrict__ stack_in) {
+  const int i = threadIdx.x;
+  if (i >= SHIFT_QUADS) return make_uint4(0u, 0u, 0u, 0u);
+  const long quad = (long)(unit / PRE_BANDS) * (OBS_PIX / 4) + (unit % PRE_BANDS) * SHIFT_QUADS + i;
+  return reinterpret_cast<const uint4*>(stack_in)[quad];
+}
+__device__ __forceinline__ void synth_shift_store(uint64_t seed, uint32_t env_offset, uint64_t id, uint32_t thresh, int unit,
+                                                  uint4 old, uint32_t* __restrict__ stack_out,
+                                                  uint32_t* __restrict__ stack_out2, const bool force_reset = false) {
   const int e = unit / PRE_BANDS;
   const int band = unit % PRE_BANDS;
-  constexpr int QUADS_PER_BAND = OBS_PIX / PRE_BANDS / 4;
   const int i = threadIdx.x;
-  if (i >= QUADS_PER_BAND) return;
-  const int q = band * QUADS_PER_BAND + i;
+  if (i >= SHIFT_QUADS) return;
+  const int q = band * SHIFT_QUADS + i;
   const long quad = (long)e * (OBS_PIX / 4) + q;
-  uint4 old = force_reset ? make_uint4(0u, 0u, 0u, 0u) : reinterpret_cast<const uint4*>(stack_in)[quad];
   const uint32_t key = synth_key(seed, env_offset + (uint32_t)e, id);
   const bool reset = force_reset || lowbias32(key ^ 0x3C6EF372u) < thresh;
   if (reset) old = make_uint4(0u, 0u, 0u, 0u);
@@ -103,6 +107,34 @@
   reinterpret_cast<uint4*>(stack_out)[quad] = outv;
   if (stack_out2) reinterpret_cast<uint4*>(stack_out2)[quad] = outv;
 }
+__device__ __forceinline__ void synth_shift_band(uint64_t seed, uint32_t env_offset, uint64_t id, uint32_t thresh, int unit,
+                                                 const uint32_t* __restrict__ stack_in, uint32_t* __restrict__ stack_out,
+                                                 uint32_t* __restrict__ stack_out2 = nullptr,
+                                                 const bool force_reset = false) {
+  const uint4 old = force_reset ? make_uint4(0u, 0u, 0u, 0u) : synth_shift_load(unit, stack_in);
+  synth_shift_store(seed, env_offset, id, thresh, unit, old, stack_out, stack_out2, force_reset);
+}
+
+struct ActSample {
+  const float* partial;
+  int ntiles;
+  const float *ba, *bc;
+  float *probs_out, *values_out;
+  int A;
+  uint32_t* mt_state;
+  int32_t* actions;
+  uint64_t seed;
+  uint32_t env_offset;
+  int N;
+  uint32_t thresh;
+  const uint64_t* step_base;
+  uint64_t step_off;
+  StepRecords rec;
+};
+struct ActRider {
+  ActSample owed;
+  SynthStep shift;
+};
 
 __device__ __forceinline__ void synth_raw_unit(uint64_t seed, uint32_t env_offset, uint64_t id, int unit,
                                                uint32_t* __restrict__ raw) {
diff --git a/paac_amd/hip_ops.py b/paac_amd/hip_ops.py
--- a/paac_amd/hip_ops.py
+++ b/paac_amd/hip_ops.py
@@ -349,21 +349,38 @@
         self._act(N, params, states, mt_state, actions, probs_out, values_out, step, env_seed, env_offset, terminal_threshold,
                   step_base_dev, step_offset, raw_scratch, walk_scratch)
 
+    def act_step_pipe(self, params, states, mt_state, actions, probs_out, values_out, env_seed, env_offset,
+                      terminal_threshold, step_base_dev, step_offset, stack_out, rewards_out, masks_out, ep_reward, ep_len,
+                      finished=None, stack_out2=None):
+        N = self._check_states(states)
+        if stack_out is None:
+            raise ValueError("stack_out is required")
+        step = _step_ptrs(N, stack_out, rewards_out, masks_out, ep_reward, ep_len, finished, stack_out2, states=states)
+        self._act(N, params, states, mt_state, actions, probs_out, values_out, step, env_seed, env_offset, terminal_threshold,
+                  step_base_dev, step_offset, entry="paac_act_step_pipe")
+
+    def act_step_flush(self):
+        _lib.check(self.lib.paac_act_step_flush(self.handle, _stream()), "paac_act_step_flush")
+
+    def act_step_pending(self):
+        return bool(self.lib.paac_act_step_pending(self.handle))
+
     def act_mt(self, params, states, mt_state, actions, probs_out, values_out):
         N = self._check_states(states)
         self._act(N, params, states, mt_state, actions, probs_out, values_out, _step_ptrs(N))
 
     def _act(self, N, params, states, mt_state, actions, probs_out, values_out, step, env_seed=0, env_offset=0,
-             terminal_threshold=0, step_base_dev=None, step_offset=0, raw_scratch=None, walk_scratch=None):
+             terminal_threshold=0, step_base_dev=None, step_offset=0, raw_scratch=None, walk_scratch=None,
+             entry="paac_act_step_mt"):
         A = self.num_actions
-        _lib.check(self.lib.paac_act_step_mt(
+        _lib.check(getattr(self.lib, entry)(
             self.handle, _ptr(params, torch.float32, self.layout["total"], "params"),
             _ptr(states, torch.uint8, N * 28224, "states"), N, _ptr(mt_state, torch.int32, 625, "mt_state"),
             _ptr(actions, torch.int32, N, "actions"), _ptr(probs_out, torch.float32, N * A, "probs_out"),
             _ptr(values_out, torch.float32, N, "values_out"), int(env_seed), int(env_offset), int(terminal_threshold),
             _ptr(step_base_dev, torch.int64, 1, "step_base", True), int(step_offset), *step,
             _ptr(raw_scratch, torch.uint8, N * 2 * RAW_H * RAW_W, "raw_scratch", True),
-            *_lent(walk_scratch), _stream()), "paac_act_step_mt")
+            *_lent(walk_scratch), _stream()), entry)
 
     def pack_weights(self, params):
         _lib.check(self.lib.paac_pack_weights(self.handle, _ptr(params, torch.float32, self.layout["total"], "params"),
@@ -846,6 +863,7 @@
 FUSED_SAMPLE_MAX_DRAWS = 2304
 ACT_STEP_MAX_DRAWS = 1024
 ACT_STEP_MAX_ENVS = 64
+ACT_PIPE_MAX_ACTIONS = 31
 ACT_STEP_MAX_ENVS_LARGE = 256
 KEEP_FORWARD_MAX_ROWS = 256
 
diff --git a/paac_amd/paac.py b/paac_amd/paac.py
--- a/paac_amd/paac.py
+++ b/paac_amd/paac.py
@@ -57,6 +57,7 @@
 class DeviceRollout(object):
     truncs = None
     pool = None
+    act_pipeline = False
 
     def __init__(self, learner, env_spec, sampler="philox", sampler_seed=42, env_offset=0, use_graph=True,
                  total_envs=None):
@@ -145,6 +146,9 @@
         self.act_step_large = os.environ.get("PAAC_MT_AHEAD", "1") != "0" and N <= hip_ops.ACT_STEP_MAX_ENVS_LARGE and towered
         self.reuse_acting = os.environ.get("PAAC_REUSE_ACTING", "1") != "0" and towered and N <= hip_ops.KEEP_FORWARD_MAX_ROWS
         self.route = self._route()
+        self.act_pipeline = (os.environ.get("PAAC_ACT_PIPELINE", "1") != "0" and self.route == "act_step" and self.raw is None
+                             and self.reuse_acting and N <= hip_ops.ACT_STEP_MAX_ENVS
+                             and N * (A - 1) <= hip_ops.ACT_STEP_MAX_DRAWS and A <= hip_ops.ACT_PIPE_MAX_ACTIONS)
         self.records = [(self.rewards[t], self.masks[t], self.ep_reward, self.ep_len, self.finished) for t in range(T)]
         if self.pool is not None:
             hip_ops.duel_ghost_reset(env_spec["seed"], self.env_offset, self.env_state[0], self.states[0], self.ghost_states[0])
@@ -181,7 +185,10 @@
         seed = self.env_spec["seed"]
         if self.reuse_acting:
             L.ctx.keep_next_forward(t * self.N)
-        if route == "act_step":
+        if route == "act_step" and self.act_pipeline:
+            L.ctx.act_step_pipe(params, obs, self.mt_state, self.actions[t], self.probs, self.values[t], seed, self.env_offset,
+                                self.env_spec["terminal_threshold"], self.tick, t, nxt, *records, stack_out2=wrap)
+        elif route == "act_step":
             L.ctx.act_step_mt(params, obs, self.mt_state, self.actions[t], self.probs, self.values[t], seed, self.env_offset,
                               self.env_spec["terminal_threshold"], self.tick, t, nxt, *records, stack_out2=wrap,
                               raw_scratch=self.raw, walk_scratch=self.walk_scratch)
```

Result: faster. 827,300 env-steps/s, median of 6 (+10.2%).
